# PeixinC/VoiceControlledRobot-VAR

Hardware: AMD Instinct MI355X
Metric: pretext triplets/sec (84x84 RGB + 16 kHz/1 s audio) (higher is better)
Workload: dtype f32; 1 GPU; Kuka+GoogleCommand pretext step, batch 256 per GPU on MI355X, fp32: u8 84x84 image + 2 int16 1 s clips per triplet resident in HBM -> MFCC -> fwd + triplet loss + bwd + Adam (BASELINE.json configs[1]); per_gpu_batch=256, global_batch=256, audio=16 kHz x 1 s int16 x 2, parallelism=dp1, launch=hip-graph replay, head=triplet

## Files before the change

include/var_hip.h:

```cpp
#ifndef VAR_HIP_H
#define VAR_HIP_H

#include <stdint.h>

#ifdef __cplusplus
extern "C" {
#endif

#define VAR_OK 0
#define VAR_ERR_ARG (-1)
#define VAR_ERR_HIP (-2)
#define VAR_ERR_PLAN (-3)
#define VAR_ERR_STATE (-4)

#define VAR_N_PARAMS 213478
#define VAR_EMB_DIM 3
#define VAR_MFCC_FRAMES 100
#define VAR_MFCC_COEFFS 40

typedef struct var_ctx var_ctx;


int var_init(int device_id, var_ctx** out);
int var_destroy(var_ctx* ctx);
const char* var_last_error(var_ctx* ctx);
int var_param_count(void);

int var_plan(var_ctx* ctx, int max_batch, int img_hw);

int var_plan_generation(var_ctx* ctx);
int var_saved_generation(var_ctx* ctx);

typedef struct var_weights var_weights;
int var_weights_create(var_ctx* ctx, var_weights** out);
int var_weights_destroy(var_ctx* ctx, var_weights* w);
int var_weights_bind(var_ctx* ctx, var_weights* w);
int var_pack_weights(var_ctx* ctx, void* stream, const float* params);

int var_arm_encoder_fwd(var_ctx* ctx, void* stream, const float* params,
                        const void* image, int image_is_u8, long image_bstride,
                        const float* mfcc_pos, const float* mfcc_neg, int B, int H,
                        float* image_feat, float* pos_feat, float* neg_feat,
                        float* image_raw, float* pos_raw, int save_for_bwd);

int var_row_dot(var_ctx* ctx, void* stream, const float* a, const float* b, int rows, int dim, float* out);
int var_set_reward_dot(var_ctx* ctx, const float* goal_feat, float* reward_out);

int var_arm_encoder_bwd(var_ctx* ctx, void* stream, const float* params,
                        const float* g_image_feat, const float* g_pos_feat, const float* g_neg_feat,
                        float* grads);

int var_triplet_fwd_bwd(var_ctx* ctx, void* stream, const float* a, const float* p, const float* n,
                        int B, float margin, float inv_count,
                        float* loss_out, float* ga, float* gp, float* gn);

int var_arm_loss_grad(var_ctx* ctx, void* stream, const float* params,
                      const void* image, int image_is_u8, long image_bstride,
                      const float* mfcc_pos, const float* mfcc_neg, int B, int H,
                      float margin, float inv_count,
                      float* grads, float* loss_out, float* feats_out);

int var_arm_loss_grad_pcm(var_ctx* ctx, void* stream, const float* params,
                          const void* image, int image_is_u8, long image_bstride, const int* image_index,
                          const int16_t* pcm, int pcm_stride, const int* clip_index, const int* lens,
                          int B, int H, float margin, float inv_count,
                          float* grads, float* loss_out, float* feats_out);

int var_arm_loss_grad_gather(var_ctx* ctx, void* stream, const float* params,
                             const void* image, int image_is_u8, long image_bstride, const int* image_index,
                             const float* mfcc_pos, const float* mfcc_neg, int B, int H,
                             float margin, float inv_count,
                             float* grads, float* loss_out, float* feats_out);

int var_adam_step(var_ctx* ctx, void* stream, float* params, const float* grads, float* exp_avg,
                  float* exp_avg_sq, long n, float lr, float beta1, float beta2, float eps,
                  float weight_decay, int step);

int var_adam_step_dev(var_ctx* ctx, void* stream, float* params, const float* grads, float* exp_avg,
                      float* exp_avg_sq, long n, const float* lr_dev, float beta1, float beta2, float eps,
                      float weight_decay, int* step_dev);

int var_adam_step_graph(var_ctx* ctx, void* stream, float* params, const float* grads, float* exp_avg,
                        float* exp_avg_sq, long n, const float* lr_dev, float beta1, float beta2, float eps,
                        float weight_decay, int* step_dev, const int* index_table, int row_ints, int n_rows,
                        int* cursor_dev, int* index_row, int ahead);

int var_mfcc(var_ctx* ctx, void* stream, const int16_t* pcm, const int* lens, const int* clip_index,
             int nclips, int pcm_stride, int out_frames, float* out);

int var_mfcc_ex(var_ctx* ctx, void* stream, const int16_t* pcm, const int* lens, const int* clip_index,
                int nclips, int pcm_stride, int out_frames, int n_fft, int win_length, int hop_length, float* out);

int var_ithor_param_count(void);
int var_ithor_plan(var_ctx* ctx, int max_batch, int img_hw);
int var_ithor_set_bf16(var_ctx* ctx, int on);
int var_ithor_set_gru_sequence(var_ctx* ctx, int on);
int var_ithor_gru_status(var_ctx* ctx, unsigned* word);
int var_ithor_guard_loss(var_ctx* ctx, const float* loss_dev);
int var_ithor_encoder_fwd(var_ctx* ctx, void* stream, const float* params,
                          const void* image, int image_is_u8, long image_bstride,
                          const float* snd_pos, const float* snd_neg, int B, int H,
                          float* image_feat, float* pos_feat, float* neg_feat,
                          float* image_raw, float* pos_raw, int save_for_bwd);
int var_ithor_saved_generation(var_ctx* ctx);
int var_ithor_encoder_bwd(var_ctx* ctx, void* stream, const float* params,
                          const float* g_image_feat, const float* g_pos_feat, const float* g_neg_feat,
                          float* grads);
int var_ithor_loss_grad(var_ctx* ctx, void* stream, const float* params,
                        const void* image, int image_is_u8, long image_bstride,
                        const float* snd_pos, const float* snd_neg, int B, int H,
                        float margin, float inv_count,
                        float* grads, float* loss_out, float* feats_out);

int var_inbatch_loss_fwd_bwd(var_ctx* ctx, void* stream, const float* anchor, const float* cand, const int* target,
                             int B, int M, float tau, float inv_count, float* scratch, float* loss_out,
                             float* g_anchor, float* g_cand);

int var_comm_unique_id(var_ctx* ctx, void* id128);
int var_comm_init(var_ctx* ctx, int rank, int nranks, const void* id128);
int var_comm_destroy(var_ctx* ctx);
int var_allreduce_grads(var_ctx* ctx, void* stream, float* flat_grad, long n);
int var_allgather_emb(var_ctx* ctx, void* stream, const float* local, float* global, long n_local);

int var_armnet_param_count(void);
int var_armnet_plan(var_ctx* ctx, int max_batch);
int var_armnet_forward(var_ctx* ctx, void* stream, const float* params, const void* image, int image_is_u8,
                       long image_bstride, const float* image_feat, const float* robot_pose,
                       const float* goal_sound_feat, const float* rnn_hxs, const float* masks, int B,
                       float* value, float* actor_features, float* action_mean, float* rnn_hxs_out);
int var_armnet_status(var_ctx* ctx, unsigned* word);
int var_armnet_clear_status(var_ctx* ctx);

int var_ithor_policy_param_count(int n_actions);
int var_ithor_policy_plan(var_ctx* ctx, int max_batch);
int var_ithor_policy_forward(var_ctx* ctx, void* stream, const float* params, int n_actions, const void* image, int image_is_u8,
                             long image_bstride, const void* occupancy, int occupancy_is_u8, const float* image_feat,
                             const float* goal_sound_feat, const float* rnn_hxs, const float* masks, int B,
                             float* value, float* actor_features, float* logits, float* rnn_hxs_out);
int var_ithor_policy_status(var_ctx* ctx, unsigned* word);
int var_ithor_policy_clear_status(var_ctx* ctx);

int var_ithor_reward_plan(var_ctx* ctx, int max_batch, int img_hw);
int var_ithor_reward_pack(var_ctx* ctx, void* stream, const float* params);
int var_ithor_reward_step(var_ctx* ctx, void* stream, const float* params,
                          const void* image, int image_is_u8, long image_bstride,
                          const float* goal_mfcc, int B,
                          float* image_feat, float* goal_feat, float* reward);

int var_mfcc_psf(var_ctx* ctx, void* stream, const int16_t* pcm, const int* lens, const int* clip_index,
                 int nclips, int pcm_stride, int out_frames, float* out);

int var_profile_tag_count(void);
const char* var_profile_tag_name(int tag);
int var_profile_select(var_ctx* ctx, int tag);
int var_profile_read(var_ctx* ctx, float* total_ms, int* count);
int var_set_streams(var_ctx* ctx, int mask);
int var_join_status(var_ctx* ctx, unsigned* timeouts);
int var_debug_buffer(var_ctx* ctx, const char* name, void** ptr, long* nfloats);
int var_debug_ithor_gru_drop_workgroup(var_ctx* ctx);
int var_debug_armnet_drop_workgroup(var_ctx* ctx);
int var_debug_ithor_dense(var_ctx* ctx, void* stream, int a_kfast, int b_kfast, const float* a, const float* b,
                          float* c, int M, int N, int K, int nsplit, int add);

#ifdef __cplusplus
}
#endif
#endif
```

voicecontrolledrobot-var_amd/_lib.py:

```python
import ctypes
import os
import subprocess
import threading

_HERE = os.path.dirname(os.path.abspath(__file__))
_LIB_PATH = os.environ.get("VAR_HIP_LIB") or os.path.join(_HERE, "libvar_hip.so")
_lib = None
_lock = threading.Lock()


class VarHipError(RuntimeError):
    pass


def library_path():
    return _LIB_PATH


def build_library(force=False):
    args = ["make", "-C", os.path.join(_HERE, "csrc"), "-j8", "-s"]
    if force:
        args.append("-B")
    subprocess.check_call(args)
    return _LIB_PATH


_vp, _i, _l, _f = ctypes.c_void_p, ctypes.c_int, ctypes.c_long, ctypes.c_float

_SIGNATURES = {
    "var_init": (_i, [_i, ctypes.POINTER(_vp)]),
    "var_destroy": (_i, [_vp]),
    "var_last_error": (ctypes.c_char_p, [_vp]),
    "var_param_count": (_i, []),
    "var_plan": (_i, [_vp, _i, _i]),
    "var_plan_generation": (_i, [_vp]),
    "var_saved_generation": (_i, [_vp]),
    "var_weights_create": (_i, [_vp, ctypes.POINTER(_vp)]),
    "var_weights_destroy": (_i, [_vp, _vp]),
    "var_weights_bind": (_i, [_vp, _vp]),
    "var_pack_weights": (_i, [_vp, _vp, _vp]),
    "var_arm_encoder_fwd": (_i, [_vp, _vp, _vp, _vp, _i, _l, _vp, _vp, _i, _i, _vp, _vp, _vp, _vp, _vp, _i]),
    "var_arm_encoder_bwd": (_i, [_vp, _vp, _vp, _vp, _vp, _vp, _vp]),
    "var_row_dot": (_i, [_vp, _vp, _vp, _vp, _i, _i, _vp]),
    "var_triplet_fwd_bwd": (_i, [_vp, _vp, _vp, _vp, _vp, _i, _f, _f, _vp, _vp, _vp, _vp]),
    "var_arm_loss_grad": (_i, [_vp, _vp, _vp, _vp, _i, _l, _vp, _vp, _i, _i, _f, _f, _vp, _vp, _vp]),
    "var_adam_step": (_i, [_vp, _vp, _vp, _vp, _vp, _vp, _l, _f, _f, _f, _f, _f, _i]),
    "var_adam_step_dev": (_i, [_vp, _vp, _vp, _vp, _vp, _vp, _l, _vp, _f, _f, _f, _f, _vp]),
    "var_adam_step_graph": (_i, [_vp, _vp, _vp, _vp, _vp, _vp, _l, _vp, _f, _f, _f, _f, _vp, _vp, _i, _i, _vp, _vp, _i]),
    "var_mfcc": (_i, [_vp, _vp, _vp, _vp, _vp, _i, _i, _i, _vp]),
    "var_mfcc_ex": (_i, [_vp, _vp, _vp, _vp, _vp, _i, _i, _i, _i, _i, _i, _vp]),
    "var_arm_loss_grad_pcm": (_i, [_vp, _vp, _vp, _vp, _i, _l, _vp, _vp, _i, _vp, _vp, _i, _i, _f, _f, _vp, _vp, _vp]),
    "var_arm_loss_grad_gather": (_i, [_vp, _vp, _vp, _vp, _i, _l, _vp, _vp, _vp, _i, _i, _f, _f, _vp, _vp, _vp]),
    "var_inbatch_loss_fwd_bwd": (_i, [_vp, _vp, _vp, _vp, _vp, _i, _i, _f, _f, _vp, _vp, _vp, _vp]),
    "var_comm_unique_id": (_i, [_vp, _vp]),
    "var_comm_init": (_i, [_vp, _i, _i, _vp]),
    "var_comm_destroy": (_i, [_vp]),
    "var_allreduce_grads": (_i, [_vp, _vp, _vp, _l]),
    "var_allgather_emb": (_i, [_vp, _vp, _vp, _vp, _l]),
    "var_armnet_param_count": (_i, []),
    "var_armnet_plan": (_i, [_vp, _i]),
    "var_armnet_forward": (_i, [_vp, _vp, _vp, _vp, _i, _l, _vp, _vp, _vp, _vp, _vp, _i, _vp, _vp, _vp, _vp]),
    "var_armnet_status": (_i, [_vp, _vp]),
    "var_join_status": (_i, [_vp, _vp]),
    "var_set_reward_dot": (_i, [_vp, _vp, _vp]),
    "var_armnet_clear_status": (_i, [_vp]),
    "var_debug_armnet_drop_workgroup": (_i, [_vp]),
    "var_ithor_policy_param_count": (_i, [_i]),
    "var_ithor_policy_plan": (_i, [_vp, _i]),
    "var_ithor_policy_forward": (_i, [_vp, _vp, _vp, _i, _vp, _i, _l, _vp, _i, _vp, _vp, _vp, _vp, _i, _vp, _vp, _vp, _vp]),
    "var_ithor_policy_status": (_i, [_vp, _vp]),
    "var_ithor_policy_clear_status": (_i, [_vp]),
    "var_ithor_reward_plan": (_i, [_vp, _i, _i]),
    "var_ithor_reward_pack": (_i, [_vp, _vp, _vp]),
    "var_ithor_reward_step": (_i, [_vp, _vp, _vp, _vp, _i, _l, _vp, _i, _vp, _vp, _vp]),
    "var_mfcc_psf": (_i, [_vp, _vp, _vp, _vp, _vp, _i, _i, _i, _vp]),
    "var_ithor_param_count": (_i, []),
    "var_ithor_plan": (_i, [_vp, _i, _i]),
    "var_ithor_set_bf16": (_i, [_vp, _i]),
    "var_ithor_set_gru_sequence": (_i, [_vp, _i]),
    "var_ithor_gru_status": (_i, [_vp, _vp]),
    "var_ithor_guard_loss": (_i, [_vp, _vp]),
    "var_debug_ithor_gru_drop_workgroup": (_i, [_vp]),
    "var_ithor_encoder_fwd": (_i, [_vp, _vp, _vp, _vp, _i, _l, _vp, _vp, _i, _i, _vp, _vp, _vp, _vp, _vp, _i]),
    "var_ithor_saved_generation": (_i, [_vp]),
    "var_ithor_encoder_bwd": (_i, [_vp, _vp, _vp, _vp, _vp, _vp, _vp]),
    "var_ithor_loss_grad": (_i, [_vp, _vp, _vp, _vp, _i, _l, _vp, _vp, _i, _i, _f, _f, _vp, _vp, _vp]),
    "var_profile_tag_count": (_i, []),
    "var_profile_tag_name": (ctypes.c_char_p, [_i]),
    "var_profile_select": (_i, [_vp, _i]),
    "var_set_streams": (_i, [_vp, _i]),
    "var_profile_read": (_i, [_vp, ctypes.POINTER(_f), ctypes.POINTER(_i)]),
    "var_debug_buffer": (_i, [_vp, ctypes.c_char_p, ctypes.POINTER(_vp), ctypes.POINTER(_l)]),
    "var_debug_ithor_dense": (_i, [_vp, _vp, _i, _i, _vp, _vp, _vp, _i, _i, _i, _i, _i]),
}

EXPORTED_SYMBOLS = tuple(_SIGNATURES.keys())


def load_library():
    global _lib
    with _lock:
        if _lib is None:
            if not os.path.exists(_LIB_PATH):
                raise VarHipError(
                    f"{_LIB_PATH} is missing: build it with `python __graft_entry__.py` "
                    "(there is no CPU/eager fallback for the VAR hot path)")
            lib = ctypes.CDLL(_LIB_PATH)
            for name, (res, args) in _SIGNATURES.items():
                fn = getattr(lib, name)
                fn.restype = res
                fn.argtypes = args
            _lib = lib
    return _lib


def new_graph():
    import torch
    return torch.cuda.CUDAGraph()


class Context:
    _by_device = {}

    def __init__(self, device_index):
        self.lib = load_library()
        self.device_index = int(device_index)
        h = _vp()
        rc = self.lib.var_init(self.device_index, ctypes.byref(h))
        if rc != 0:
            raise VarHipError(f"var_init({device_index}) failed ({rc}): {self.lib.var_last_error(None).decode()}")
        self.handle = h
        self.plan = (0, 0)

    @classmethod
    def get(cls, device_index):
        ctx = cls._by_device.get(device_index)
        if ctx is None:
            ctx = cls._by_device[device_index] = Context(device_index)
        return ctx

    def check(self, rc, what):
        if rc != 0:
            raise VarHipError(f"{what} failed ({rc}): {self.lib.var_last_error(self.handle).decode()}")

    def stream(self):
        return current_stream_handle()

    def new_weights(self):
        return Weights(self)

    def capture(self, groups):
        import torch
        dev = torch.device("cuda", self.device_index)
        side = torch.cuda.Stream(device=dev)
        side.wait_stream(torch.cuda.current_stream(dev))
        graphs = []
        with torch.cuda.stream(side):
            for bodies in groups:
                g = new_graph()
                with torch.cuda.graph(g, stream=side, capture_error_mode="thread_local"):
                    for body in bodies:
                        body()
                graphs.append(g)
        torch.cuda.current_stream(dev).wait_stream(side)
        return [g.replay for g in graphs]

    def ensure_plan(self, batch, hw):
        if self.plan[1] != hw or self.plan[0] < batch:
            self.check(self.lib.var_plan(self.handle, int(batch), int(hw)), "var_plan")
            self.plan = (int(batch), int(hw))

    def profile_select(self, tag):
        self.check(self.lib.var_profile_select(self.handle, int(tag)), "var_profile_select")

    def set_streams(self, mask):
        return self.lib.var_set_streams(self.handle, int(mask))

    def join_timeouts(self):
        n = ctypes.c_uint(0)
        self.check(self.lib.var_join_status(self.handle, ctypes.byref(n)), "var_join_status")
        return n.value

    def profile_read(self):
        ms, n = _f(), _i()
        self.check(self.lib.var_profile_read(self.handle, ctypes.byref(ms), ctypes.byref(n)), "var_profile_read")
        return ms.value, n.value

    def tag_names(self):
        return [self.lib.var_profile_tag_name(t).decode() for t in range(self.lib.var_profile_tag_count())]

    def debug_buffer(self, name):
        import torch
        p, n = _vp(), _l()
        self.check(self.lib.var_debug_buffer(self.handle, name.encode(), ctypes.byref(p), ctypes.byref(n)),
                   "var_debug_buffer")
        out = torch.empty(n.value, dtype=torch.float32, device=f"cuda:{self.device_index}")
        torch.cuda.synchronize()
        rt = ctypes.CDLL("libamdhip64.so")
        rt.hipMemcpy.argtypes = [_vp, _vp, ctypes.c_size_t, _i]
        rc = rt.hipMemcpy(out.data_ptr(), p, n.value * 4, 3)
        if rc != 0:
            raise VarHipError(f"hipMemcpy failed ({rc})")
        return out


class Weights:

    def __init__(self, ctx):
        self.ctx = ctx
        h = _vp()
        ctx.check(ctx.lib.var_weights_create(ctx.handle, ctypes.byref(h)), "var_weights_create")
        self.handle = h
        self.key = None

    def bind(self):
        c = self.ctx
        c.check(c.lib.var_weights_bind(c.handle, self.handle), "var_weights_bind")

    def pack(self, flat, key=None):
        c = self.ctx
        self.bind()
        c.check(c.lib.var_pack_weights(c.handle, c.stream(), flat.data_ptr()), "var_pack_weights")
        self.key = key

    def __del__(self):
        try:
            if self.handle and self.ctx.handle:
                self.ctx.lib.var_weights_destroy(self.ctx.handle, self.handle)
        except Exception:
            pass
        self.handle = None


def ptr(t):
    return None if t is None else t.data_ptr()


def current_stream_handle():
    import torch
    return torch.cuda.current_stream().cuda_stream
```

voicecontrolledrobot-var_amd/csrc/api.hip:

```cpp
#include <new>
#include <stdlib.h>
#include <string.h>

#include "var_common.h"

static char g_init_err[256] = "";

#define CHECK_CTX(ctx) do { if (!(ctx)) return VAR_ERR_ARG; } while (0)
#define SET_DEVICE(ctx) VAR_HIP_CHECK(ctx, hipSetDevice((ctx)->device))

extern "C" {

int var_param_count(void) { return VAR_N_PARAMS; }

const char* var_last_error(var_ctx* ctx) { return ctx ? ctx->err : g_init_err; }

static int default_streams();

int var_init(int device_id, var_ctx** out) {
    if (!out) return VAR_ERR_ARG;
    *out = nullptr;
    int n = 0;
    hipError_t e = hipGetDeviceCount(&n);
    if (e != hipSuccess || device_id < 0 || device_id >= n) {
        snprintf(g_init_err, sizeof(g_init_err), "var_init: device %d not available (%d HIP devices, %s)",
                 device_id, n, hipGetErrorString(e));
        return VAR_ERR_HIP;
    }
    var_ctx* c = new (std::nothrow) var_ctx();
    if (!c) return VAR_ERR_HIP;
    c->device = device_id;
    c->streams = default_streams();
    c->pl = make_param_layout();
    c->kl = make_pack_layout();
    if (c->pl.total != VAR_N_PARAMS) {
        snprintf(g_init_err, sizeof(g_init_err), "var_init: layout mismatch %d", c->pl.total);
        delete c;
        return VAR_ERR_ARG;
    }
    e = hipSetDevice(device_id);
    if (e == hipSuccess) e = hipMalloc((void**)&c->default_w.data, sizeof(float) * (size_t)c->kl.total);
    c->default_w.owner = c;
    c->bound = &c->default_w;
    c->wpack = c->default_w.data;
    if (e == hipSuccess) e = hipMalloc((void**)&c->loss_buf, sizeof(float) * 64);
    if (e == hipSuccess) e = hipMemset(c->loss_buf, 0, sizeof(float) * 64);
    c->done_ctr = (unsigned*)(c->loss_buf + 32);
    c->jsig = (unsigned*)(c->loss_buf + 40);
    if (e != hipSuccess) {
        snprintf(g_init_err, sizeof(g_init_err), "var_init: %s", hipGetErrorString(e));
        delete c;
        return VAR_ERR_HIP;
    }
    if (e == hipSuccess) e = hipStreamCreateWithFlags(&c->side, hipStreamNonBlocking);
    for (int i = 0; i < 2 && e == hipSuccess; i++) {
        e = hipEventCreateWithFlags(&c->ev_fork[i], hipEventDisableTiming);
        if (e == hipSuccess) e = hipEventCreateWithFlags(&c->ev_join[i], hipEventDisableTiming);
    }
    if (e != hipSuccess) {
        snprintf(g_init_err, sizeof(g_init_err), "var_init: %s", hipGetErrorString(e));
        delete c;
        return VAR_ERR_HIP;
    }
    if (mfcc_build_tables(c) != VAR_OK || pack_table_upload(c) != VAR_OK) {
        snprintf(g_init_err, sizeof(g_init_err), "var_init: %s", c->err);
        delete c;
        return VAR_ERR_HIP;
    }
    *out = c;
    return VAR_OK;
}

int var_destroy(var_ctx* c) {
    CHECK_CTX(c);
    (void)hipSetDevice(c->device);
    comm_free(c);
    mfcc_any_forget(c);
    ithor_free(c);
    armnet_free(c);
    ithor_policy_free(c);
    ithor_reward_free(c);
    for (auto& sl : c->ws_slot) if (sl.base) (void)hipFree(sl.base);
    for (int i = 0; i < c->n_retired; i++) (void)hipFree(c->retired[i]);
    free(c->retired);
    if (c->default_w.data) (void)hipFree(c->default_w.data);
    if (c->loss_buf) (void)hipFree(c->loss_buf);
    if (c->mfcc_tab) (void)hipFree(c->mfcc_tab);
    if (c->mfcc_psf_tab) (void)hipFree(c->mfcc_psf_tab);
    if (c->pack_segs_dev) (void)hipFree(c->pack_segs_dev);
    for (int i = 0; i < 2; i++) {
        if (c->ev_fork[i]) (void)hipEventDestroy(c->ev_fork[i]);
        if (c->ev_join[i]) (void)hipEventDestroy(c->ev_join[i]);
    }
    if (c->side) (void)hipStreamDestroy(c->side);
    if (c->prof_ev) {
        for (int i = 0; i < 2 * kProfMaxPairs; i++) (void)hipEventDestroy(c->prof_ev[i]);
        delete[] c->prof_ev;
    }
    delete c;
    return VAR_OK;
}

int retire_block(var_ctx* c, void* p) {
    if (c->n_retired == c->cap_retired) {
        const int cap = c->cap_retired ? 2 * c->cap_retired : 8;
        void** q = (void**)realloc(c->retired, sizeof(void*) * cap);
        if (!q) { VAR_SET_ERR(c, "var_plan: out of host memory"); return VAR_ERR_HIP; }
        c->retired = q; c->cap_retired = cap;
    }
    c->retired[c->n_retired++] = p;
    return VAR_OK;
}

int var_plan_generation(var_ctx* c) { return c ? c->plan_gen : VAR_ERR_ARG; }
int var_saved_generation(var_ctx* c) { return c ? (c->saved_B > 0 ? c->saved_gen : 0) : VAR_ERR_ARG; }

int var_weights_create(var_ctx* c, var_weights** out) {
    CHECK_CTX(c);
    if (!out) return VAR_ERR_ARG;
    *out = nullptr;
    SET_DEVICE(c);
    var_weights* w = new (std::nothrow) var_weights();
    if (!w) return VAR_ERR_HIP;
    w->owner = c;
    hipError_t e = hipMalloc((void**)&w->data, sizeof(float) * (size_t)c->kl.total);
    if (e != hipSuccess) { VAR_SET_ERR(c, "var_weights_create: %s", hipGetErrorString(e)); delete w; return VAR_ERR_HIP; }
    *out = w;
    return VAR_OK;
}

int var_weights_destroy(var_ctx* c, var_weights* w) {
    CHECK_CTX(c);
    if (!w || w->owner != c || w == &c->default_w) { VAR_SET_ERR(c, "var_weights_destroy: not a handle of this context"); return VAR_ERR_ARG; }
    SET_DEVICE(c);
    if (c->bound == w) { c->bound = &c->default_w; c->wpack = c->default_w.data; }
    int rc = retire_block(c, w->data);
    delete w;
    return rc;
}

int var_weights_bind(var_ctx* c, var_weights* w) {
    CHECK_CTX(c);
    if (!w) w = &c->default_w;
    if (w->owner != c) { VAR_SET_ERR(c, "var_weights_bind: handle belongs to another context"); return VAR_ERR_ARG; }
    c->bound = w;
    c->wpack = w->data;
    return VAR_OK;
}

static int check_weights(var_ctx* c, const float* params, const char* who) {
    if (c->bound->params != params) {
        VAR_SET_ERR(c, "%s: the bound weight image was %s -- var_weights_bind + var_pack_weights first", who,
                    c->bound->params ? "packed from another parameter arena" : "never packed");
        return VAR_ERR_STATE;
    }
    return VAR_OK;
}

static size_t plan_layout(var_ctx* c, char* base, int max_batch, int img_hw) {
    const size_t B = (size_t)max_batch;
    int hs[6];
    hs[0] = img_hw;
    for (int i = 0; i < 5; i++) hs[i + 1] = conv_out(hs[i]);
    size_t off = 0;
    auto carve = [&](size_t nfloats) { size_t o = off; off += (nfloats * 4 + 255) & ~(size_t)255; return o; };
    size_t o_act[6], o_gact[6], o_sact[5], o_gsact[5];
    for (int l = 1; l <= 5; l++) {
        size_t n = B * kImgCh[l] * hs[l] * hs[l];
        if (l == 1 && img_hw == 84) n = B * kAct1TiledFloats;
        o_act[l] = carve(n);
        o_gact[l] = carve(n);
    }
    for (int l = 1; l <= 4; l++) {
        const size_t n = 2 * B * 32 * kSndT[l];
        o_sact[l] = carve(n);
        o_gsact[l] = carve(n);
    }
    const size_t o_hid_i = carve(B * kHid), o_hid_s = carve(2 * B * kHid);
    const size_t o_emb = carve(9 * B), o_emb_raw = carve(9 * B), o_gemb = carve(24 * B), o_hpart = carve(48 * B);
    const size_t o_ghid = carve(6 * B * kHid);
    const size_t n_img_slab = img_slab_floats(), n_snd_slab = snd_slab_floats();
    const size_t o_slab = carve(n_img_slab + n_snd_slab);
    const size_t o_mfcc = carve(2 * B * VAR_MFCC_FRAMES * VAR_MFCC_COEFFS);
    if (!base) return off;
    c->ws = base;
    c->ws_bytes = off;
    auto P = [&](size_t o) { return (float*)(c->ws + o); };
    for (int l = 1; l <= 5; l++) { c->act[l] = P(o_act[l]); c->gact[l] = P(o_gact[l]); }
    for (int l = 1; l <= 4; l++) { c->sact[l] = P(o_sact[l]); c->gsact[l] = P(o_gsact[l]); }
    c->hid_i = P(o_hid_i); c->hid_s = P(o_hid_s);
    c->head_part = P(o_hpart);
    c->emb = P(o_emb); c->emb_raw = P(o_emb_raw); c->gemb = P(o_gemb); c->ghid = P(o_ghid);
    c->slabs = P(o_slab);
    c->mfcc_buf = P(o_mfcc);
    c->slab_floats = n_img_slab + n_snd_slab;
    c->snd_slab_off = n_img_slab;
    c->maxB = max_batch;
    c->H = img_hw;
    for (int i = 0; i < 6; i++) c->hs[i] = hs[i];
    c->saved_B = 0;
    return off;
}

int var_plan(var_ctx* c, int max_batch, int img_hw) {
    CHECK_CTX(c);
    if (max_batch <= 0 || (img_hw != 84 && img_hw != 96)) {
        VAR_SET_ERR(c, "var_plan: batch %d / image size %d unsupported (size must be 84 or 96)", max_batch, img_hw);
        return VAR_ERR_ARG;
    }
    SET_DEVICE(c);
    if (c->ws && c->maxB >= max_batch && c->H == img_hw) return VAR_OK;
    var_ctx::WsSlot& slot = c->ws_slot[img_hw == 84 ? 0 : 1];
    if (!slot.base || slot.maxB < max_batch) {
        if (slot.base) { int rc = retire_block(c, slot.base); if (rc != VAR_OK) return rc; slot.base = nullptr; }
        if (c->ws && c->H == img_hw) c->ws = nullptr;
        const int Bn = slot.maxB > max_batch ? slot.maxB : max_batch;
        const size_t bytes = plan_layout(c, nullptr, Bn, img_hw);
        char* blk = nullptr;
        VAR_HIP_CHECK(c, hipMalloc((void**)&blk, bytes));
        VAR_HIP_CHECK(c, hipMemset(blk, 0, bytes));
        slot.base = blk; slot.maxB = Bn;
    }
    c->plan_gen++;
    plan_layout(c, slot.base, slot.maxB, img_hw);
    return VAR_OK;
}

int var_pack_weights(var_ctx* c, void* stream, const float* params) {
    CHECK_CTX(c);
    if (!params) { VAR_SET_ERR(c, "var_pack_weights: null params"); return VAR_ERR_ARG; }
    SET_DEVICE(c);
    c->bound->params = params;
    return launch_pack_weights(c, (hipStream_t)stream, params);
}

static int check_plan(var_ctx* c, int B, int H, const char* who) {
    if (!c->ws) { VAR_SET_ERR(c, "%s: var_plan() has not been called", who); return VAR_ERR_PLAN; }
    if (B <= 0) { VAR_SET_ERR(c, "%s: batch %d", who, B); return VAR_ERR_ARG; }
    if (B > c->maxB || H != c->H) {
        VAR_SET_ERR(c, "%s: batch %d / size %d exceeds the plan (%d / %d)", who, B, H, c->maxB, c->H);
        return VAR_ERR_PLAN;
    }
    return VAR_OK;
}


struct AudioIn {
    const int16_t* pcm = nullptr; const int* lens = nullptr; const int* clip_index = nullptr; int pcm_stride = 0;
};

static int fork_side(var_ctx* c, hipStream_t s, int i) {
    if (!(c->streams & (1 << i))) return VAR_OK;
    VAR_HIP_CHECK(c, hipEventRecord(c->ev_fork[i], s));
    VAR_HIP_CHECK(c, hipStreamWaitEvent(c->side, c->ev_fork[i], 0));
    return VAR_OK;
}
static int join_side(var_ctx* c, hipStream_t s, int i) {
    if (!(c->streams & (1 << i))) return VAR_OK;
    VAR_HIP_CHECK(c, hipEventRecord(c->ev_join[i], c->side));
    VAR_HIP_CHECK(c, hipStreamWaitEvent(s, c->ev_join[i], 0));
    return VAR_OK;
}

struct CopySegs { float* dst[5]; const float* src[5]; int n[5]; int count; };
__global__ void __launch_bounds__(256) copy_out_kernel(CopySegs S) {
    for (int k = 0; k < S.count; ++k)
        for (int e = blockIdx.x * 256 + threadIdx.x; e < S.n[k]; e += gridDim.x * 256) S.dst[k][e] = S.src[k][e];
}

__global__ void __launch_bounds__(256) gemb_in_kernel(const float* __restrict__ g0, const float* __restrict__ g1, const float* __restrict__ g2,
                                                      float* __restrict__ gemb, int n) {
    const int e = blockIdx.x * 256 + threadIdx.x;
    if (e >= n) return;
    gemb[e] = g0 ? g0[e] : 0.f;
    gemb[n + e] = g1 ? g1[e] : 0.f;
    gemb[2 * n + e] = g2 ? g2[e] : 0.f;
}

__global__ void __launch_bounds__(256) row_dot_kernel(const float* __restrict__ a, const float* __restrict__ b, int rows, int dim,
                                                      float* __restrict__ out) {
    const int r = blockIdx.x * 256 + threadIdx.x;
    if (r >= rows) return;
    float s = 0.f;
    for (int k = 0; k < dim; ++k) s += a[(size_t)r * dim + k] * b[(size_t)r * dim + k];
    out[r] = s;
}

static constexpr int kHead1MaxB = 64;
static constexpr int kSmallMidB = 16;

static FwdPlan plan_encoder_fwd(int H, int B, int save_for_bwd, bool image, bool pos, bool neg, bool finish, bool join_requested,
                                bool capturing, int streams, bool dot_armed) {
    FwdPlan p;
    const bool fwd_only = save_for_bwd == 2;
    const bool snd = pos || neg;
    const bool head2 = !(fwd_only && B <= kHead1MaxB);
    if (head2 && H == 84 && B <= kHead2G && !snd) p.img = ImgPath::All;
    else if (fwd_only && B <= kSmallMidB && H == 84) p.img = ImgPath::Head1Small;
    else p.img = head2 ? ImgPath::Head2Mid3 : ImgPath::Head1Mid3;
    p.act1_tiled = head2 && H == 84;
    p.head_in_conv = p.img != ImgPath::Head1Small;
    p.conv_finish = p.head_in_conv && finish;
    p.fork_ok = (streams & 1) && B > 32;
    p.mfcc_main = !p.fork_ok;
    p.dev_join = join_requested && capturing && p.fork_ok && (streams & 2) && !(streams & 64) && image && pos && neg;
    if (dot_armed && image && finish) p.dot = p.img == ImgPath::Head1Small ? RewardDot::InHead : RewardDot::RowDot;
    return p;
}

static int encoder_fwd(var_ctx* c, hipStream_t s, const float* params, const void* image, int is_u8,
                       long bstride, const int* image_index, const float* pos, const float* neg,
                       const AudioIn* audio, int B, int save_for_bwd, bool finish, bool join_requested, bool dot_armed) {
    int rc;
    if (audio && audio->pcm) {
        pos = c->mfcc_buf;
        neg = c->mfcc_buf + (size_t)B * VAR_MFCC_FRAMES * VAR_MFCC_COEFFS;
    }
    const bool snd = pos || neg;
    hipStreamCaptureStatus cap = hipStreamCaptureStatusNone;
    if (join_requested && hipStreamIsCapturing(s, &cap) != hipSuccess) cap = hipStreamCaptureStatusNone;
    const FwdPlan p = plan_encoder_fwd(c->H, B, save_for_bwd, image, pos, neg, finish, join_requested,
                                       cap == hipStreamCaptureStatusActive, c->streams, dot_armed);
    c->fwd_plan = p;
    hipStream_t ss = p.fork_ok ? c->side : s;
    bool forked = false;
    if (snd && audio && audio->pcm) {
        if (!p.mfcc_main) { if ((rc = fork_side(c, s, 0)) != VAR_OK) return rc; forked = true; }
        if ((rc = launch_mfcc(c, p.mfcc_main ? s : ss, audio->pcm, audio->lens, audio->clip_index, 2 * B, audio->pcm_stride,
                              VAR_MFCC_FRAMES, c->mfcc_buf)) != VAR_OK) return rc;
    }
    if (snd && p.fork_ok && !forked && (rc = fork_side(c, s, 0)) != VAR_OK) return rc;
    if (image) {
        if ((rc = launch_img_fwd(c, s, p, params, image, is_u8, bstride, image_index, B)) != VAR_OK) return rc;
        if ((rc = launch_heads_fwd(c, s, s, p, params, B, true, false, false, finish)) != VAR_OK) return rc;
        if (p.dot == RewardDot::RowDot) {
            hipLaunchKernelGGL(row_dot_kernel, dim3((B + 255) / 256), dim3(256), 0, s, (const float*)c->emb, c->dot_with, B, kEmb, c->dot_out);
            VAR_HIP_CHECK(c, hipGetLastError());
        }
    }
    if (snd) {
        if ((rc = launch_snd_fwd(c, ss, params, pos, neg, B)) != VAR_OK) return rc;
        if ((rc = launch_heads_fwd(c, ss, ss, p, params, B, false, pos != nullptr, neg != nullptr, finish)) != VAR_OK) return rc;
        if (p.fork_ok && !p.dev_join && (rc = join_side(c, s, 0)) != VAR_OK) return rc;
    }
    c->saved_B = B;
    c->saved_gen = ++c->fwd_gen;
    c->saved_image = image;
    c->saved_u8 = is_u8;
    c->saved_bstride = bstride;
    c->saved_index = image_index;
    c->saved_pos = pos;
    c->saved_neg = neg;
    return VAR_OK;
}

int var_arm_encoder_fwd(var_ctx* c, void* stream, const float* params, const void* image, int image_is_u8,
                        long image_bstride, const float* mfcc_pos, const float* mfcc_neg, int B, int H,
                        float* image_feat, float* pos_feat, float* neg_feat, float* image_raw, float* pos_raw,
                        int save_for_bwd) {
    CHECK_CTX(c);
    if (!params) { VAR_SET_ERR(c, "var_arm_encoder_fwd: null params"); return VAR_ERR_ARG; }
    if (image && image_bstride < 3L * H * H) { VAR_SET_ERR(c, "var_arm_encoder_fwd: image stride %ld < 3*H*H", image_bstride); return VAR_ERR_ARG; }
    int rc = check_plan(c, B, H, "var_arm_encoder_fwd");
    if (rc != VAR_OK) return rc;
    if ((rc = check_weights(c, params, "var_arm_encoder_fwd")) != VAR_OK) return rc;
    SET_DEVICE(c);
    hipStream_t s = (hipStream_t)stream;
    c->out_img = image ? image_feat : nullptr; c->out_pos = mfcc_pos ? pos_feat : nullptr; c->out_neg = mfcc_neg ? neg_feat : nullptr;
    rc = encoder_fwd(c, s, params, image, image_is_u8, image_bstride, nullptr, mfcc_pos, mfcc_neg, nullptr, B, save_for_bwd, true,
                     false, c->dot_out != nullptr);
    c->out_img = c->out_pos = c->out_neg = nullptr;
    c->dot_with = nullptr; c->dot_out = nullptr;
    if (rc != VAR_OK) return rc;
    if (save_for_bwd != 1) c->saved_B = 0;
    CopySegs S{};
    auto seg = [&](float* dst, const float* src, int n) { S.dst[S.count] = dst; S.src[S.count] = src; S.n[S.count] = n; S.count++; };
    if (image && image_raw) seg(image_raw, c->act[5], kImgFeat * B);
    if (mfcc_pos && pos_raw) seg(pos_raw, c->sact[4], kSndFeat * B);
    if (S.count) {
        const int grid = (kImgFeat * B + 255) / 256;
        hipLaunchKernelGGL(copy_out_kernel, dim3(grid < 1024 ? grid : 1024), dim3(256), 0, s, S);
        VAR_HIP_CHECK(c, hipGetLastError());
    }
    return VAR_OK;
}

int var_row_dot(var_ctx* c, void* stream, const float* a, const float* b, int rows, int dim, float* out) {
    CHECK_CTX(c);
    if (!a || !b || !out || rows < 1 || dim < 1 || dim > 64) { VAR_SET_ERR(c, "var_row_dot: bad argument (rows %d, dim %d)", rows, dim); return VAR_ERR_ARG; }
    SET_DEVICE(c);
    hipLaunchKernelGGL(row_dot_kernel, dim3((rows + 255) / 256), dim3(256), 0, (hipStream_t)stream, a, b, rows, dim, out);
    VAR_HIP_CHECK(c, hipGetLastError());
    return VAR_OK;
}

int var_set_reward_dot(var_ctx* c, const float* goal_feat, float* reward_out) {
    CHECK_CTX(c);
    if ((goal_feat == nullptr) != (reward_out == nullptr)) { VAR_SET_ERR(c, "var_set_reward_dot: both pointers or neither"); return VAR_ERR_ARG; }
    c->dot_with = goal_feat;
    c->dot_out = reward_out;
    return VAR_OK;
}

static int encoder_bwd(var_ctx* c, hipStream_t s, const float* params, float* grads, bool fused = false,
                       float margin = 0.f, float inv_count = 0.f, float* loss_out = nullptr) {
    const int B = c->saved_B;
    int rc;
    if (!c->saved_image || !c->saved_pos || !c->saved_neg) {
        if ((rc = var_zero_async(c, s, grads, sizeof(float) * VAR_N_PARAMS)) != VAR_OK) return rc;
    }
    const int snd_lo = c->saved_pos ? 0 : B, snd_hi = c->saved_neg ? 2 * B : B;
    hipStream_t ss = (c->streams & 2) ? c->side : s;
    const bool dev_join = c->fwd_plan.dev_join;
    if (!dev_join && (rc = fork_side(c, s, 1)) != VAR_OK) return rc;
    if (c->saved_image) {
        if ((rc = launch_heads_bwd(c, s, s, params, grads, B, true, 0, 0, dev_join, fused, margin, inv_count, fused ? loss_out : nullptr)) != VAR_OK) return rc;
        if ((rc = launch_img_bwd(c, s, params, grads, B)) != VAR_OK) return rc;
    }
    if ((rc = launch_heads_bwd(c, ss, ss, params, grads, B, false, snd_lo, snd_hi, dev_join, fused, margin, inv_count)) != VAR_OK) return rc;
    if ((rc = launch_snd_bwd(c, ss, params, grads, B)) != VAR_OK) return rc;
    return join_side(c, s, 1);
}

int var_arm_encoder_bwd(var_ctx* c, void* stream, const float* params, const float* g_image_feat,
                        const float* g_pos_feat, const float* g_neg_feat, float* grads) {
    CHECK_CTX(c);
    if (!params || !grads) { VAR_SET_ERR(c, "var_arm_encoder_bwd: null params/grads"); return VAR_ERR_ARG; }
    if (c->saved_B <= 0) { VAR_SET_ERR(c, "var_arm_encoder_bwd: no forward saved (save_for_bwd=1 required)"); return VAR_ERR_STATE; }
    { int rc = check_weights(c, params, "var_arm_encoder_bwd"); if (rc != VAR_OK) return rc; }
    SET_DEVICE(c);
    hipStream_t s = (hipStream_t)stream;
    const int B = c->saved_B;
    hipLaunchKernelGGL(gemb_in_kernel, dim3((3 * B + 255) / 256), dim3(256), 0, s, g_image_feat, g_pos_feat, g_neg_feat, c->gemb, 3 * B);
    VAR_HIP_CHECK(c, hipGetLastError());
    return encoder_bwd(c, s, params, grads);
}

int var_triplet_fwd_bwd(var_ctx* c, void* stream, const float* a, const float* p, const float* n, int B,
                        float margin, float inv_count, float* loss_out, float* ga, float* gp, float* gn) {
    CHECK_CTX(c);
    if (!a || !p || !n || !loss_out || B <= 0) { VAR_SET_ERR(c, "var_triplet_fwd_bwd: bad argument"); return VAR_ERR_ARG; }
    SET_DEVICE(c);
    return launch_triplet(c, (hipStream_t)stream, a, p, n, B, margin, inv_count, loss_out, ga, gp, gn);
}

static int loss_grad_impl(var_ctx* c, hipStream_t s, const float* params, const void* image, int image_is_u8,
                          long image_bstride, const int* image_index, const float* mfcc_pos, const float* mfcc_neg,
                          const AudioIn* audio, int B, int H, float margin, float inv_count, float* grads,
                          float* loss_out, float* feats_out, const char* who) {
    if (image_bstride < 3L * H * H) { VAR_SET_ERR(c, "%s: image stride %ld < 3*H*H", who, image_bstride); return VAR_ERR_ARG; }
    int rc = check_plan(c, B, H, who);
    if (rc != VAR_OK) return rc;
    if ((rc = check_weights(c, params, who)) != VAR_OK) return rc;
    SET_DEVICE(c);
    const bool fused = !feats_out && image && (mfcc_pos || (audio && audio->pcm)) && (mfcc_neg || (audio && audio->pcm));
    if ((rc = encoder_fwd(c, s, params, image, image_is_u8, image_bstride, image_index, mfcc_pos, mfcc_neg, audio, B, 1,
                          !fused, fused, false)) != VAR_OK) return rc;
    if (fused) {
        rc = encoder_bwd(c, s, params, grads, true, margin, inv_count, loss_out);
        c->fwd_plan.dev_join = false;
        return rc;
    }
    if ((rc = launch_triplet(c, s, c->emb, c->emb + 3 * B, c->emb + 6 * B, B, margin, inv_count, loss_out,
                             c->gemb, c->gemb + 3 * B, c->gemb + 6 * B)) != VAR_OK) return rc;
    if (feats_out)
        if ((rc = var_copy_async(c, s, feats_out, c->emb, sizeof(float) * 9 * (size_t)B)) != VAR_OK) return rc;
    return encoder_bwd(c, s, params, grads);
}

int var_arm_loss_grad(var_ctx* c, void* stream, const float* params, const void* image, int image_is_u8,
                      long image_bstride, const float* mfcc_pos, const float* mfcc_neg, int B, int H,
                      float margin, float inv_count, float* grads, float* loss_out, float* feats_out) {
    CHECK_CTX(c);
    if (!params || !image || !mfcc_pos || !mfcc_neg || !grads || !loss_out) {
        VAR_SET_ERR(c, "var_arm_loss_grad: null argument");
        return VAR_ERR_ARG;
    }
    return loss_grad_impl(c, (hipStream_t)stream, params, image, image_is_u8, image_bstride, nullptr, mfcc_pos,
                          mfcc_neg, nullptr, B, H, margin, inv_count, grads, loss_out, feats_out, "var_arm_loss_grad");
}

int var_arm_loss_grad_gather(var_ctx* c, void* stream, const float* params, const void* image, int image_is_u8,
                             long image_bstride, const int* image_index, const float* mfcc_pos, const float* mfcc_neg,
                             int B, int H, float margin, float inv_count, float* grads, float* loss_out,
                             float* feats_out) {
    CHECK_CTX(c);
    if (!params || !image || !mfcc_pos || !mfcc_neg || !grads || !loss_out) {
        VAR_SET_ERR(c, "var_arm_loss_grad_gather: null argument");
        return VAR_ERR_ARG;
    }
    return loss_grad_impl(c, (hipStream_t)stream, params, image, image_is_u8, image_bstride, image_index, mfcc_pos,
                          mfcc_neg, nullptr, B, H, margin, inv_count, grads, loss_out, feats_out,
                          "var_arm_loss_grad_gather");
}

int var_arm_loss_grad_pcm(var_ctx* c, void* stream, const float* params, const void* image, int image_is_u8,
                          long image_bstride, const int* image_index, const int16_t* pcm, int pcm_stride,
                          const int* clip_index, const int* lens, int B, int H, float margin, float inv_count,
                          float* grads, float* loss_out, float* feats_out) {
    CHECK_CTX(c);
    if (!params || !image || !pcm || !lens || !grads || !loss_out || pcm_stride <= 0) {
        VAR_SET_ERR(c, "var_arm_loss_grad_pcm: null argument");
        return VAR_ERR_ARG;
    }
    AudioIn a;
    a.pcm = pcm; a.lens = lens; a.clip_index = clip_index; a.pcm_stride = pcm_stride;
    return loss_grad_impl(c, (hipStream_t)stream, params, image, image_is_u8, image_bstride, image_index, nullptr,
                          nullptr, &a, B, H, margin, inv_count, grads, loss_out, feats_out, "var_arm_loss_grad_pcm");
}

int var_adam_step(var_ctx* c, void* stream, float* params, const float* grads, float* exp_avg, float* exp_avg_sq,
                  long n, float lr, float beta1, float beta2, float eps, float weight_decay, int step) {
    CHECK_CTX(c);
    if (!params || !grads || !exp_avg || !exp_avg_sq || n <= 0 || step < 1) {
        VAR_SET_ERR(c, "var_adam_step: bad argument");
        return VAR_ERR_ARG;
    }
    SET_DEVICE(c);
    hipStream_t s = (hipStream_t)stream;
    int rc = launch_adam(c, s, params, grads, exp_avg, exp_avg_sq, n, lr, beta1, beta2, eps, weight_decay, step);
    if (rc != VAR_OK) return rc;
    if (n == VAR_N_PARAMS && c->bound->params == params) return launch_pack_weights(c, s, params);
    return VAR_OK;
}

int var_adam_step_dev(var_ctx* c, void* stream, float* params, const float* grads, float* exp_avg, float* exp_avg_sq,
                      long n, const float* lr_dev, float beta1, float beta2, float eps, float weight_decay,
                      int* step_dev) {
    return var_adam_step_graph(c, stream, params, grads, exp_avg, exp_avg_sq, n, lr_dev, beta1, beta2, eps,
                               weight_decay, step_dev, nullptr, 0, 0, nullptr, nullptr, 0);
}

int var_adam_step_graph(var_ctx* c, void* stream, float* params, const float* grads, float* exp_avg,
                        float* exp_avg_sq, long n, const float* lr_dev, float beta1, float beta2, float eps,
                        float weight_decay, int* step_dev, const int* index_table, int row_ints, int n_rows,
                        int* cursor_dev, int* index_row, int ahead_from) {
    CHECK_CTX(c);
    if (!params || !grads || !exp_avg || !exp_avg_sq || !lr_dev || !step_dev || n <= 0) {
        VAR_SET_ERR(c, "var_adam_step_dev: bad argument");
        return VAR_ERR_ARG;
    }
    if (index_table && (!cursor_dev || !index_row || row_ints <= 0 || n_rows <= 0)) {
        VAR_SET_ERR(c, "var_adam_step_graph: index table without cursor / row buffer / sizes");
        return VAR_ERR_ARG;
    }
    SET_DEVICE(c);
    return launch_adam_dev(c, (hipStream_t)stream, params, grads, exp_avg, exp_avg_sq, n, lr_dev, beta1, beta2, eps,
                           weight_decay, step_dev, n == VAR_N_PARAMS && c->bound->params == params, index_table, row_ints, n_rows, cursor_dev, index_row,
                           ahead_from);
}

int var_mfcc(var_ctx* c, void* stream, const int16_t* pcm, const int* lens, const int* clip_index, int nclips,
             int pcm_stride, int out_frames, float* out) {
    CHECK_CTX(c);
    if (!pcm || !lens || !out || nclips <= 0 || pcm_stride <= 0 || out_frames <= 0) {
        VAR_SET_ERR(c, "var_mfcc: bad argument");
        return VAR_ERR_ARG;
    }
    SET_DEVICE(c);
    return launch_mfcc(c, (hipStream_t)stream, pcm, lens, clip_index, nclips, pcm_stride, out_frames, out);
}

int var_mfcc_ex(var_ctx* c, void* stream, const int16_t* pcm, const int* lens, const int* clip_index, int nclips,
                int pcm_stride, int out_frames, int n_fft, int win_length, int hop_length, float* out) {
    CHECK_CTX(c);
    if (!pcm || !lens || !out || nclips <= 0 || pcm_stride <= 0 || out_frames <= 0) {
        VAR_SET_ERR(c, "var_mfcc_ex: bad argument");
        return VAR_ERR_ARG;
    }
    SET_DEVICE(c);
    if (n_fft == 512 && win_length == 400 && hop_length == 160)
        return launch_mfcc(c, (hipStream_t)stream, pcm, lens, clip_index, nclips, pcm_stride, out_frames, out);
    return launch_mfcc_any(c, (hipStream_t)stream, pcm, lens, clip_index, nclips, pcm_stride, out_frames, n_fft, win_length,
                           hop_length, out);
}

static const char* kTagNames[TAG_COUNT] = {
    "(unused)", "img conv1+conv2 forward", "img conv3+4+5 forward + image head", "(unused)",
    "(unused)", "(unused)", "(unused)", "img conv3+4+5 weight gradients",
    "(unused)", "(unused)", "(unused)",
    "img conv2 data gradient + conv2, conv1 weight gradients",
    "img conv5-4-3 data gradient chain", "(unused)", "(unused)", "img weight-gradient slab fold",
    "snd_fwd_kernel", "snd_dgrad_kernel", "snd_wgrad_kernel", "snd_reduce_kernel", "heads_fwd_kernel",
    "heads_bwd_rows_kernel", "heads_bwd_gemm_kernel", "triplet_kernel", "adam_kernel", "pack_weights_kernel",
    "mfcc_kernel", "ithor conv 11x5 s2 forward", "ithor conv 11x5 s2 data gradient", "ithor conv 11x5 s2 weight gradient"};

int var_profile_tag_count(void) { return TAG_COUNT; }
const char* var_profile_tag_name(int tag) { return (tag >= 0 && tag < TAG_COUNT) ? kTagNames[tag] : ""; }

static int default_streams() { return kDefaultStreams; }

int var_set_streams(var_ctx* c, int mask) {
    if (!c) return -1;
    const int old = c->streams;
    c->streams = mask < 0 ? default_streams() : (mask & (3 | 64));
    return old;
}

int var_join_status(var_ctx* c, unsigned* timeouts) {
    CHECK_CTX(c);
    if (!timeouts) { VAR_SET_ERR(c, "var_join_status: null argument"); return VAR_ERR_ARG; }
    SET_DEVICE(c);
    unsigned w[8];
    VAR_HIP_CHECK(c, hipMemcpy(w, c->jsig, sizeof(w), hipMemcpyDeviceToHost));
    *timeouts = w[3] + w[7];
    return VAR_OK;
}

int var_profile_select(var_ctx* c, int tag) {
    CHECK_CTX(c);
    SET_DEVICE(c);
    if (tag >= TAG_COUNT) { VAR_SET_ERR(c, "var_profile_select: bad tag %d", tag); return VAR_ERR_ARG; }
    if (tag >= 0 && !c->prof_ev) {
        c->prof_ev = new hipEvent_t[2 * kProfMaxPairs];
        for (int i = 0; i < 2 * kProfMaxPairs; i++) VAR_HIP_CHECK(c, hipEventCreate(&c->prof_ev[i]));
    }
    c->prof_tag = tag;
    c->prof_n = 0;
    return VAR_OK;
}

int var_profile_read(var_ctx* c, float* total_ms, int* count) {
    CHECK_CTX(c);
    if (!total_ms || !count) return VAR_ERR_ARG;
    SET_DEVICE(c);
    float tot = 0.f;
    for (int i = 0; i < c->prof_n; i++) {
        float ms = 0.f;
        VAR_HIP_CHECK(c, hipEventSynchronize(c->prof_ev[2 * i + 1]));
        VAR_HIP_CHECK(c, hipEventElapsedTime(&ms, c->prof_ev[2 * i], c->prof_ev[2 * i + 1]));
        tot += ms;
    }
    *total_ms = tot;
    *count = c->prof_n;
    return VAR_OK;
}

int var_debug_buffer(var_ctx* c, const char* name, void** ptr, long* nfloats) {
    CHECK_CTX(c);
    if (!name || !ptr || !nfloats) return VAR_ERR_ARG;
    const size_t B = c->maxB;
    *ptr = nullptr; *nfloats = 0;
    if (!strcmp(name, "wpack")) { *ptr = c->wpack; *nfloats = c->kl.total; return VAR_OK; }
    if (!strncmp(name, "ithor_", 6)) return ithor_debug_buffer(c, name + 6, ptr, nfloats);
    if (!c->ws) { VAR_SET_ERR(c, "var_debug_buffer: no plan"); return VAR_ERR_PLAN; }
    for (int l = 1; l <= 5; l++) {
        char a[16], g[16];
        snprintf(a, sizeof a, "act%d", l); snprintf(g, sizeof g, "gact%d", l);
        const long n = (long)(B * kImgCh[l] * c->hs[l] * c->hs[l]);
        if (!strcmp(name, a)) {
            *ptr = c->act[l]; *nfloats = n;
            if (l == 1 && c->fwd_plan.act1_tiled) {
                int rc = launch_act1_untile(c, nullptr, (int)B);
                if (rc != VAR_OK) return rc;
                VAR_HIP_CHECK(c, hipStreamSynchronize(nullptr));
                *ptr = c->gact[1];
            }
            return VAR_OK;
        }
        if (!strcmp(name, g)) { *ptr = c->gact[l]; *nfloats = n; return VAR_OK; }
    }
    for (int l = 1; l <= 4; l++) {
        char a[16], g[16];
        snprintf(a, sizeof a, "sact%d", l); snprintf(g, sizeof g, "gsact%d", l);
        const long n = (long)(2 * B * 32 * kSndT[l]);
        if (!strcmp(name, a)) { *ptr = c->sact[l]; *nfloats = n; return VAR_OK; }
        if (!strcmp(name, g)) { *ptr = c->gsact[l]; *nfloats = n; return VAR_OK; }
    }
    if (!strcmp(name, "hid_i")) { *ptr = c->hid_i; *nfloats = (long)B * kHid; return VAR_OK; }
    if (!strcmp(name, "hid_s")) { *ptr = c->hid_s; *nfloats = 2 * (long)B * kHid; return VAR_OK; }
    if (!strcmp(name, "emb")) { *ptr = c->emb; *nfloats = 9 * (long)B; return VAR_OK; }
    if (!strcmp(name, "mfcc")) { *ptr = c->mfcc_buf; *nfloats = 2 * (long)B * VAR_MFCC_FRAMES * VAR_MFCC_COEFFS; return VAR_OK; }
    if (!strcmp(name, "slabs")) { *ptr = c->slabs; *nfloats = (long)c->slab_floats; return VAR_OK; }
    if (!strcmp(name, "gemb")) { *ptr = c->gemb; *nfloats = 9 * (long)B; return VAR_OK; }
    VAR_SET_ERR(c, "var_debug_buffer: unknown buffer '%s'", name);
    return VAR_ERR_ARG;
}

}
```

voicecontrolledrobot-var_amd/csrc/img_conv_bwd.hip:

```cpp
#include <stdio.h>
#include <stdlib.h>

#include "img_stage.h"
#define VAR_WGRAD_DEVICE_ONLY
#include "img_wgrad.hip"
#undef VAR_WGRAD_DEVICE_ONLY

template <class W2, class W3, class W4>
__global__ void __launch_bounds__(768)
img_wgrad345_kernel(const float* __restrict__ x2, const float* __restrict__ x3, const float* __restrict__ x4,
                    const float* __restrict__ gy3, const float* __restrict__ gy4, const float* __restrict__ gy5,
                    float* __restrict__ slabs2, float* __restrict__ slabs3, float* __restrict__ slabs4, int G2, int G3, int G4, int B) {
    static_assert(W2::NW * 64 == 768 && W3::NW * 64 == 768 && W4::NW * 64 == 768, "12 waves each");
    int id = blockIdx.x;
    const int n2 = G2 * W2::NCOMBO, n3 = G3 * W3::NCOMBO;
    if (id < n2) { img_wgrad_body<W2>(x2, (long)W2::CIN * W2::H * W2::W, nullptr, gy3, slabs2, B, id % G2, id / G2, G2); return; }
    id -= n2;
    if (id < n3) { img_wgrad_body<W3>(x3, (long)W3::CIN * W3::H * W3::W, nullptr, gy4, slabs3, B, id % G3, id / G3, G3); return; }
    id -= n3;
    img_wgrad_body<W4>(x4, (long)W4::CIN * W4::H * W4::W, nullptr, gy5, slabs4, B, id % G4, id / G4, G4);
}

template <class W2, class W3, class W4>
static int launch_wgrad345(var_ctx* c, hipStream_t s, int B) {
    ProfScope prof(c, s, TAG_IMG_WGRAD0 + 2);
    constexpr int LDS_BYTES = W2::LDS_BYTES > W3::LDS_BYTES ? (W2::LDS_BYTES > W4::LDS_BYTES ? W2::LDS_BYTES : W4::LDS_BYTES)
                                                           : (W3::LDS_BYTES > W4::LDS_BYTES ? W3::LDS_BYTES : W4::LDS_BYTES);
    static unsigned attr_set = 0;
    if (!(attr_set & var_dev_bit(c))) {
        VAR_HIP_CHECK(c, hipFuncSetAttribute((const void*)img_wgrad345_kernel<W2, W3, W4>,
                                             hipFuncAttributeMaxDynamicSharedMemorySize, LDS_BYTES));
        attr_set |= var_dev_bit(c);
    }
    auto groups = [&](int layer, int nb, int nu) {
        const int need = (B * nb + nu - 1) / nu, gmax = img_wgrad_groups(layer);
        return need < gmax ? need : gmax;
    };
    const int G2 = groups(2, W2::NB, W2::NU), G3 = groups(3, W3::NB, W3::NU), G4 = groups(4, W4::NB, W4::NU);
    c->wg_groups[2] = G2; c->wg_groups[3] = G3; c->wg_groups[4] = G4;
    hipLaunchKernelGGL((img_wgrad345_kernel<W2, W3, W4>), dim3(G2 * W2::NCOMBO + G3 * W3::NCOMBO + G4 * W4::NCOMBO), dim3(768),
                       LDS_BYTES, s, c->act[2], c->act[3], c->act[4], c->gact[3], c->gact[4], c->gact[5],
                       c->slabs + img_slab_offset(2), c->slabs + img_slab_offset(3), c->slabs + img_slab_offset(4), G2, G3, G4, B);
    VAR_HIP_CHECK(c, hipGetLastError());
    return VAR_OK;
}

int launch_img_bwd(var_ctx* c, hipStream_t s, const float* params, float* grads, int B) {
    int rc;
    const int H = c->H;
    if (H != 84 && H != 96) { VAR_SET_ERR(c, "unsupported image size %d (84 or 96)", H); return VAR_ERR_ARG; }
    if ((rc = launch_img_bwd_chain(c, s, B)) != VAR_OK) return rc;
    rc = H == 84 ? launch_wgrad345<W84_2, W84_3, W84_4>(c, s, B) : launch_wgrad345<W96_2, W96_3, W96_4>(c, s, B);
    if (rc != VAR_OK) return rc;
    rc = launch_img_bwd_tail2(c, s, B);
    if (rc != VAR_OK) return rc;
    (void)params;
    return launch_img_wgrad_reduce(c, s, grads, 0, 4);
}
```

voicecontrolledrobot-var_amd/csrc/img_wgrad.hip:

```cpp
#include <stdlib.h>

#include <type_traits>

#include "img_stage.h"

template <int CIN_, int COUT_, int H_, bool U8_, int R_, int NU_, int KS_, bool DB_ = false>
struct WgCfg {
    static constexpr bool DB = DB_;
    static constexpr int CIN = CIN_, COUT = COUT_, H = H_, W = H_, R = R_, NU = NU_;
    static constexpr bool U8 = U8_;
    static constexpr bool SMALLC = (CIN < 32);
    static constexpr int HO = (H - 1) / 2 + 1, WO = HO;
    static constexpr int IR = 2 * R + 1;
    static constexpr int PW = 2 * WO + 3;
    static constexpr int XC = SMALLC ? CIN : 32;
    static constexpr int PLANE_X = (IR * PW) | 1;
    static constexpr int UNIT_X = XC * PLANE_X;
    static constexpr int POW = WO + 1;
    static constexpr int PLANE_Y = (R * POW) | 1;
    static constexpr int UNIT_Y = 32 * PLANE_Y;
    static constexpr int NB = (HO + R - 1) / R;
    static constexpr int NBLK = COUT / 32;
    static constexpr int CBLK = SMALLC ? 1 : CIN / 32;
    static constexpr int NCOMBO = NBLK * CBLK;
    static constexpr int KS = KS_;
    static constexpr int NW = SMALLC ? KS : 3 * KS;
    static constexpr int NT = NW * 64;
    static constexpr int XS = (NU * UNIT_X + 3) & ~3, YS = NU * UNIT_Y;
    static constexpr int ZPAD = (XS + YS + 3) & ~3;
    static constexpr int STAGE = ZPAD + 4;
    static constexpr int FOLD = SMALLC ? NW * 1024 : NW * 3 * 1024;
    static constexpr int LDS_FLOATS = ((DB ? 2 : 1) * STAGE > FOLD ? (DB ? 2 : 1) * STAGE : FOLD);
    static_assert(LDS_FLOATS * 4 <= 160 * 1024, "LDS");
    static constexpr int LDS_BYTES = LDS_FLOATS * 4;
    static constexpr int SLAB = SMALLC ? (32 * 32 + 32) : (32 * 9 * 32 + 32);
    static constexpr int HSTEPS = (WO + 1) / 2;
    static constexpr int TS = NU * R * HSTEPS;
    static constexpr int NSTEP = (TS + KS - 1) / KS;
};

#ifndef VAR_WG_PH
#define VAR_WG_PH
namespace { PH_DECL(); }
#if defined(VAR_PHASES) && defined(VAR_WGRAD_DEVICE_ONLY)
extern "C" int var_debug_phases_wgrad(unsigned long long* out) {
    unsigned long long z[32] = {0};
    if (hipMemcpyFromSymbol(out, HIP_SYMBOL(g_phase), sizeof(z)) != hipSuccess) return -1;
    return hipMemcpyToSymbol(HIP_SYMBOL(g_phase), z, sizeof(z)) == hipSuccess ? 0 : -1;
}
#endif
#endif
#ifndef VAR_WG_PH_BLOCK
#define VAR_WG_PH_BLOCK 0
#endif
template <class C>
__device__ __forceinline__ void img_wgrad_body(const void* __restrict__ xin, long bstride, const int* __restrict__ bidx,
                                               const float* __restrict__ gy, float* __restrict__ slabs, int B,
                                               int bx, int by, int G) {
    extern __shared__ __attribute__((aligned(16))) float lds[];
    float* xs = lds;
    float* ys = lds + C::XS;
    constexpr int NT = C::NT;
    using XT = typename std::conditional<C::U8, uint8_t, float>::type;
    const int tid = threadIdx.x, lane = tid & 63, wave = tid >> 6;
    const int half = lane >> 5, l31 = lane & 31;
    const int total_units = B * C::NB;
    const int combo = by;
    const int nb = combo / C::CBLK, cb = combo - nb * C::CBLK;
    const int ky = C::SMALLC ? 0 : wave % 3, ks = C::SMALLC ? wave : wave / 3;

    constexpr bool FLATX = !C::U8 && !C::SMALLC && C::NB == 1 && (C::W & 1) && C::R == C::HO;
    constexpr bool FLATY = !C::SMALLC && C::NB == 1 && (C::WO & 1) && C::R == C::HO;
    typename std::conditional<FLATX, FlatStager<C::XC, C::H, C::W, C::PW, C::PLANE_X, 1, 1, NT, C::NU>,
                              ColStager<C::XC, C::H, C::W, C::IR, C::PW, C::PLANE_X, 1, C::U8, NT, C::NU>>::type sx;
    typename std::conditional<FLATY, FlatStager<32, C::HO, C::WO, C::POW, C::PLANE_Y, 0, 0, NT, C::NU>,
                              ColStager<32, C::HO, C::WO, C::R, C::POW, C::PLANE_Y, 0, false, NT, C::NU>>::type sy;
    sx.init(tid);
    sy.init(tid);

    static_assert(C::NU == 1 || C::NB == 1, "multi-unit stages need whole-image units (consecutive images)");
    struct Stage { const XT* bx; const float* by; int row0x, row0y, nvalid; };
    auto make_stage = [&](int unit0) {
        Stage st;
        const int bo = unit0 / C::NB, band = unit0 - bo * C::NB;
        const int b = bidx ? bidx[bo] : bo;
        st.bx = (const XT*)xin + (size_t)b * bstride + (size_t)(cb * C::XC) * C::H * C::W;
        st.by = gy + ((size_t)bo * C::COUT + nb * 32) * C::HO * C::WO;
        st.row0x = 2 * band * C::R - 1;
        st.row0y = band * C::R;
        st.nvalid = total_units - unit0 < C::NU ? total_units - unit0 : C::NU;
        return st;
    };
    constexpr long YSTRIDE = (long)C::COUT * C::HO * C::WO;

    const int aoff = l31 * C::PLANE_Y + half;
    int boff;
    if constexpr (C::SMALLC) {
        const int col = l31 < C::CIN * 9 ? l31 : 0;
        const int tap = col / C::CIN, c = col - tap * C::CIN;
        boff = c * C::PLANE_X + (tap / 3) * C::PW + (tap % 3) + 2 * half;
    } else {
        boff = l31 * C::PLANE_X + ky * C::PW + 2 * half;
    }
    const int t0 = (ks * C::TS) / C::KS, t1 = ((ks + 1) * C::TS) / C::KS;
    int aos[C::NSTEP], bos[C::NSTEP];
#pragma unroll
    for (int i = 0; i < C::NSTEP; ++i) {
        const int t = t0 + i;
        const bool live = t < t1;
        const int tt = live ? t : t0;
        const int u = tt / (C::R * C::HSTEPS), rem = tt - u * (C::R * C::HSTEPS);
        const int oyl = rem / C::HSTEPS, sstep = rem - oyl * C::HSTEPS;
        aos[i] = live ? C::XS + aoff + u * C::UNIT_Y + oyl * C::POW + 2 * sstep : C::ZPAD;
        bos[i] = boff + u * C::UNIT_X + 2 * oyl * C::PW + 4 * sstep;
    }
    f32x16 acc[3];
#pragma unroll
    for (int t = 0; t < 3; ++t)
#pragma unroll
        for (int r = 0; r < 16; ++r) acc[t][r] = 0.f;
    float bsum = 0.f;

    PHR_INIT(VAR_WG_PH_BLOCK, VAR_PH_THREAD);
    lds_zero<NT>(lds, C::LDS_FLOATS, tid);
    const int first = bx * C::NU;
    if (first < total_units) {
        const Stage st = make_stage(first);
        sx.issue(st.bx, bstride, st.row0x, st.nvalid);
        sy.issue(st.by, YSTRIDE, st.row0y, st.nvalid);
    }
    auto multiply = [&](const float* stage) {
#pragma unroll
        for (int i = 0; i < C::NSTEP; ++i) {
            const float a = stage[aos[i]];
            bsum += a;
            if constexpr (C::SMALLC) {
                acc[0] = __builtin_amdgcn_mfma_f32_32x32x2f32(a, stage[bos[i]], acc[0], 0, 0, 0);
            } else {
                const float b0 = stage[bos[i]], b1 = stage[bos[i] + 1], b2 = stage[bos[i] + 2];
                acc[0] = __builtin_amdgcn_mfma_f32_32x32x2f32(a, b0, acc[0], 0, 0, 0);
                acc[1] = __builtin_amdgcn_mfma_f32_32x32x2f32(a, b1, acc[1], 0, 0, 0);
                acc[2] = __builtin_amdgcn_mfma_f32_32x32x2f32(a, b2, acc[2], 0, 0, 0);
            }
        }
    };
    if constexpr (C::DB) {
        __syncthreads();
        if (first < total_units) {
            const Stage st = make_stage(first);
            sx.store(lds, st.row0x, st.nvalid);
            sy.store(lds + C::XS, st.row0y, st.nvalid);
        }
        __syncthreads();
        int it = 0;
#pragma unroll 1
        for (int unit0 = first; unit0 < total_units; unit0 += G * C::NU, ++it) {
            const int next = unit0 + G * C::NU;
            const bool more = next < total_units;
            const Stage sn = make_stage(more ? next : unit0);
            if (more) {
                sx.issue(sn.bx, bstride, sn.row0x, sn.nvalid);
                sy.issue(sn.by, YSTRIDE, sn.row0y, sn.nvalid);
            }
            __builtin_amdgcn_sched_barrier(0);
            multiply(lds + (it & 1) * C::STAGE);
            __builtin_amdgcn_sched_barrier(0);
            if (more) {
                float* nst = lds + ((it + 1) & 1) * C::STAGE;
                sx.store(nst, sn.row0x, sn.nvalid);
                sy.store(nst + C::XS, sn.row0y, sn.nvalid);
            }
            __syncthreads();
        }
    } else {
        PHR(0);
#pragma unroll 1
        for (int unit0 = first; unit0 < total_units; unit0 += G * C::NU) {
            __syncthreads();
            PHR(1);
            {
                const Stage st = make_stage(unit0);
                sx.store(xs, st.row0x, st.nvalid);
                sy.store(ys, st.row0y, st.nvalid);
            }
            PHR(2);
            __syncthreads();
            PHR(3);
            if (unit0 + G * C::NU < total_units) {
                const Stage st = make_stage(unit0 + G * C::NU);
                sx.issue(st.bx, bstride, st.row0x, st.nvalid);
                sy.issue(st.by, YSTRIDE, st.row0y, st.nvalid);
            }
            PHR(4);
            __builtin_amdgcn_sched_barrier(0);
            multiply(lds);
            __builtin_amdgcn_sched_barrier(0);
            PHR(5);
        }
    }

    float* slab = slabs + ((size_t)bx * C::NCOMBO + combo) * C::SLAB;
    bsum += __shfl_down(bsum, 32, 64);
    if constexpr (C::SMALLC) {
        __syncthreads();
#pragma unroll
        for (int r = 0; r < 16; ++r) {
            const int n = (r & 3) + 8 * (r >> 2) + 4 * half;
            lds[wave * 1024 + n * 32 + l31] = acc[0][r];
        }
        __syncthreads();
        for (int e = tid; e < 1024; e += NT) {
            float sum = 0.f;
#pragma unroll
            for (int q = 0; q < C::KS; ++q) sum += lds[q * 1024 + e];
            slab[e] = sum;
        }
    } else {
        __syncthreads();
#pragma unroll
        for (int kx = 0; kx < 3; ++kx)
#pragma unroll
            for (int r = 0; r < 16; ++r) {
                const int n = (r & 3) + 8 * (r >> 2) + 4 * half;
                lds[(wave * 3 + kx) * 1024 + n * 32 + l31] = acc[kx][r];
            }
        __syncthreads();
        for (int e = tid; e < 9 * 256; e += NT) {
            const int tap = e >> 8, kyy = tap / 3, kx = tap - 3 * kyy, i = (e & 255) * 4;
            f32x4 sum = {0.f, 0.f, 0.f, 0.f};
#pragma unroll
            for (int q = 0; q < C::KS; ++q) sum += *(const f32x4*)(lds + ((q * 3 + kyy) * 3 + kx) * 1024 + i);
            *(f32x4*)(slab + ((i >> 5) * 9 + tap) * 32 + (i & 31)) = sum;
        }
    }
    __syncthreads();
    if (ky == 0 && half == 0) lds[ks * 32 + l31] = bsum;
    __syncthreads();
    if (tid < 32) {
        float sum = 0.f;
#pragma unroll
        for (int q = 0; q < C::KS; ++q) sum += lds[q * 32 + tid];
        slab[(C::SMALLC ? 1024 : 9216) + tid] = sum;
    }
    PHR(6);
    PHR_FLUSH();
}

using W84_2 = WgCfg<32, 64, 21, false, 11, 1, 4>;
using W84_3 = WgCfg<64, 64, 11, false, 6, 4, 4>;
using W84_4 = WgCfg<64, 64, 6, false, 3, 4, 4>;
using W96_2 = WgCfg<32, 64, 24, false, 6, 1, 4>;
using W96_3 = WgCfg<64, 64, 12, false, 6, 1, 4>;
using W96_4 = WgCfg<64, 64, 6, false, 3, 4, 4>;

#ifndef VAR_WGRAD_DEVICE_ONLY
struct RedSeg { int slab_off; int slab_sz; int G; int ncombo; int cblk; int cin; int smallc; int gw; int gb; };
struct RedTable { RedSeg seg[5]; int start[6]; };

__global__ void __launch_bounds__(256)
img_wgrad_reduce_kernel(RedTable T, const float* __restrict__ slabs, float* __restrict__ grads) {
    __shared__ float part[8][33];
    const int lane32 = threadIdx.x & 31, gs = threadIdx.x >> 5;
    const int j = blockIdx.x * 32 + lane32;
    const bool live = j < T.start[5];
    int l = 0;
#pragma unroll
    for (int i = 1; i < 5; ++i) if (j >= T.start[i] && T.start[i + 1] > T.start[i]) l = i;
    const RedSeg S = T.seg[l];
    const int e = live ? j - T.start[l] : 0;
    const float* p = slabs + S.slab_off + e;
    const size_t gstride = (size_t)S.ncombo * S.slab_sz;
    float s = 0.f;
    if (live) {
#pragma unroll 8
        for (int g = gs; g < S.G; g += 8) s += p[(size_t)g * gstride];
    }
    part[gs][lane32] = s;
    __syncthreads();
    if (gs != 0 || !live) return;
    s = ((part[0][lane32] + part[1][lane32]) + (part[2][lane32] + part[3][lane32])) +
        ((part[4][lane32] + part[5][lane32]) + (part[6][lane32] + part[7][lane32]));
    const int combo = e / S.slab_sz, i = e - combo * S.slab_sz;
    if (S.smallc) {
        if (i >= 1024) { grads[S.gb + (i - 1024)] = s; return; }
        const int n = i / 32, col = i % 32;
        if (col < S.cin * 9) {
            const int tap = col / S.cin, c = col - tap * S.cin;
            grads[S.gw + (n * S.cin + c) * 9 + tap] = s;
        }
        return;
    }
    const int nb = combo / S.cblk, cb = combo - nb * S.cblk;
    if (i >= 9216) {
        if (cb == 0) grads[S.gb + nb * 32 + (i - 9216)] = s;
        return;
    }
    const int c = i % 32, tap = (i / 32) % 9, n = i / 288;
    grads[S.gw + ((nb * 32 + n) * S.cin + cb * 32 + c) * 9 + tap] = s;
}

static const int kWgG[5] = {512, 256, 64, 32, 32};
static const int kCombo[5] = {1, 1, 2, 4, 4};
static const int kSlabSz[5] = {32 * 32 + 32, 9248, 9248, 9248, 9248};

size_t img_slab_floats() {
    size_t t = 0;
    for (int i = 0; i < 5; i++) t += (size_t)kWgG[i] * kCombo[i] * kSlabSz[i];
    return t;
}

static size_t slab_offset(int layer) {
    size_t o = 0;
    for (int i = 0; i < layer; i++) o += (size_t)kWgG[i] * kCombo[i] * kSlabSz[i];
    return o;
}

int launch_img_wgrad_reduce(var_ctx* c, hipStream_t s, float* grads, int lo, int hi) {
    const ParamLayout& L = c->pl;
    RedTable T{};
    int st = 0;
    for (int i = 0; i < 5; i++) {
        T.seg[i] = RedSeg{(int)slab_offset(i), kSlabSz[i], c->wg_groups[i], kCombo[i], i < 3 ? 1 : 2, kImgCh[i],
                          i == 0 ? 1 : 0, L.img_w[i], L.img_b[i]};
        T.start[i] = st;
        if (i >= lo && i <= hi) st += kCombo[i] * kSlabSz[i];
    }
    T.start[5] = st;
    ProfScope prof(c, s, TAG_IMG_WREDUCE);
    hipLaunchKernelGGL(img_wgrad_reduce_kernel, dim3((st + 31) / 32), dim3(256), 0, s, T, c->slabs, grads);
    VAR_HIP_CHECK(c, hipGetLastError());
    return VAR_OK;
}

int img_wgrad_groups(int layer) { return kWgG[layer]; }
size_t img_slab_offset(int layer) { return slab_offset(layer); }
#endif
```

voicecontrolledrobot-var_amd/csrc/pack_adam.hip:

```cpp
#include <stdlib.h>

#include "var_common.h"

__global__ void __launch_bounds__(256) zero_words_kernel(unsigned* __restrict__ p, size_t n) {
    for (size_t i = (size_t)blockIdx.x * 256 + threadIdx.x; i < n; i += (size_t)gridDim.x * 256) p[i] = 0u;
}
__global__ void __launch_bounds__(256) copy_words_kernel(unsigned* __restrict__ d, const unsigned* __restrict__ s, size_t n) {
    for (size_t i = (size_t)blockIdx.x * 256 + threadIdx.x; i < n; i += (size_t)gridDim.x * 256) d[i] = s[i];
}
static inline int words_grid(size_t n) { const size_t g = (n + 255) / 256; return (int)(g < 1 ? 1 : (g > 2048 ? 2048 : g)); }
int var_zero_async(var_ctx* c, hipStream_t s, void* p, size_t bytes) {
    if (!bytes) return VAR_OK;
    if ((bytes & 3) || ((uintptr_t)p & 3)) { VAR_SET_ERR(c, "var_zero_async: %zu bytes at %p are not whole aligned words", bytes, p); return VAR_ERR_ARG; }
    hipLaunchKernelGGL(zero_words_kernel, dim3(words_grid(bytes / 4)), dim3(256), 0, s, (unsigned*)p, bytes / 4);
    VAR_HIP_CHECK(c, hipGetLastError());
    return VAR_OK;
}
int var_copy_async(var_ctx* c, hipStream_t s, void* dst, const void* src, size_t bytes) {
    if (!bytes) return VAR_OK;
    if ((bytes & 3) || ((uintptr_t)dst & 3) || ((uintptr_t)src & 3)) { VAR_SET_ERR(c, "var_copy_async: not whole aligned words"); return VAR_ERR_ARG; }
    hipLaunchKernelGGL(copy_words_kernel, dim3(words_grid(bytes / 4)), dim3(256), 0, s, (unsigned*)dst, (const unsigned*)src, bytes / 4);
    VAR_HIP_CHECK(c, hipGetLastError());
    return VAR_OK;
}

struct PackSeg {
    int dst;
    int count;
    int src;
    int cin, cout, taps;
    int kvalid;
    int type;
};
struct PackTable { PackSeg seg[24]; int nseg; };

__global__ void __launch_bounds__(256) pack_weights_kernel(PackTable T, const float* __restrict__ params,
                                                            float* __restrict__ wpack, int total) {
    for (int j = blockIdx.x * 256 + threadIdx.x; j < total; j += gridDim.x * 256) {
        int si = 0;
#pragma unroll
        for (int i = 1; i < 24; ++i) if (i < T.nseg && j >= T.seg[i].dst) si = i;
        const PackSeg S = T.seg[si];
        const int e = j - S.dst;
        float v = 0.f;
        if (S.type == 1) {
            const int c = e % S.cin, n = (e / S.cin) % S.cout, tap = e / (S.cin * S.cout);
            v = params[S.src + (n * S.cin + c) * S.taps + tap];
        } else if (S.type == 3) {
            const int jj = e & 3, ln = (e >> 2) & 63, grp = e >> 8;
            const int nsg = S.cout / 16, nct = S.cin / 16;
            const int sg = grp % nsg, ct = (grp / nsg) % nct, tap = grp / (nsg * nct);
            const int n = 16 * sg + 4 * jj + (ln >> 4), c = 16 * ct + (ln & 15);
            v = params[S.src + (n * S.cin + c) * S.taps + tap];
        } else if (S.type >= 4) {
            const int jj = e & 3, ln = (e >> 2) & 63, grp = e >> 8;
            const int nnt = S.cout / 16, ncg = S.cin / 16;
            const int nt = grp % nnt, G = grp / nnt;
            const int cg = S.type == 4 ? G % ncg : G / 9, tap = S.type == 4 ? G / ncg : G % 9;
            const int n = 16 * nt + (ln & 15), c = 16 * cg + 4 * jj + (ln >> 4);
            v = params[S.src + (n * S.cin + c) * S.taps + tap];
        } else {
            const int n = e % S.cout, k = e / S.cout;
            if (k < S.kvalid) {
                const int tap = k / S.cin, c = k - tap * S.cin;
                v = (S.type == 0) ? params[S.src + (n * S.cin + c) * S.taps + tap]
                                  : params[S.src + (n * S.taps + tap) * S.cin + c];
            }
        }
        wpack[j] = v;
    }
}

static PackTable make_pack_table(var_ctx* c) {
    const ParamLayout& L = c->pl;
    const PackLayout& K = c->kl;
    PackTable T{};
    int n = 0;
    auto add = [&](int dst, int count, int src, int cin, int cout, int taps, int type) {
        T.seg[n++] = PackSeg{dst, count, src, cin, cout, taps, cin * taps, type};
    };
    for (int i = 0; i < 5; i++) {
        int Kp = kImgCh[i] * 9; if (Kp & 1) Kp++;
        add(K.img_f[i], Kp * kImgCh[i + 1], L.img_w[i], kImgCh[i], kImgCh[i + 1], 9, i < 2 ? 0 : (i == 2 ? 5 : 4));
    }
    add(K.img_d[1], 9 * kImgCh[2] * kImgCh[1], L.img_w[1], kImgCh[1], kImgCh[2], 9, 1);
    add(K.snd_f[0], 200 * 32, L.snd_w[0], 40, 32, 5, 2);
    for (int i = 1; i < 4; i++) add(K.snd_f[i], 96 * 32, L.snd_w[i], 32, 32, 3, 0);
    for (int i = 1; i < 4; i++) add(K.snd_d[i], 96 * 32, L.snd_w[i], 32, 32, 3, 1);
    for (int i = 2; i < 5; i++) add(K.img_a[i], 9 * kImgCh[i + 1] * kImgCh[i], L.img_w[i], kImgCh[i], kImgCh[i + 1], 9, 3);
    add(K.ih_w0t, kImgFeat * kHid, L.ih_w0, kImgFeat, kHid, 1, 0);
    add(K.sh_w0t, kSndFeat * kHid, L.sh_w0, kSndFeat, kHid, 1, 0);
    T.nseg = n;
    return T;
}

int launch_pack_weights(var_ctx* c, hipStream_t s, const float* params) {
    const PackLayout& K = c->kl;
    const PackTable T = make_pack_table(c);
    ProfScope prof(c, s, TAG_PACK);
    hipLaunchKernelGGL(pack_weights_kernel, dim3(256), dim3(256), 0, s, T, params, c->wpack, K.total);
    VAR_HIP_CHECK(c, hipGetLastError());
    return VAR_OK;
}

__global__ void __launch_bounds__(256) adam_kernel(float* __restrict__ p, const float* __restrict__ g,
                                                    float* __restrict__ m, float* __restrict__ v, long n,
                                                    float b1, float b2, float eps, float wd,
                                                    float step_size, float bc2_sqrt, const unsigned* __restrict__ guard,
                                                    const float* __restrict__ gloss) {
    if (guard && *guard) return;
    if (gloss && !(fabsf(*gloss) <= 3.4e38f)) return;
    for (long i = (long)blockIdx.x * 256 + threadIdx.x; i < n; i += (long)gridDim.x * 256) {
        const float pi = p[i];
        const float gi = g[i] + wd * pi;
        const float mi = m[i] + (gi - m[i]) * (1.f - b1);
        const float vi = v[i] * b2 + (1.f - b2) * gi * gi;
        m[i] = mi;
        v[i] = vi;
        const float denom = sqrtf(vi) / bc2_sqrt + eps;
        p[i] = pi - step_size * (mi / denom);
    }
}

constexpr int kAdamT = 1024;
__global__ void __launch_bounds__(kAdamT)
adam_pack_dev_kernel(const PackSeg* __restrict__ segs, int nseg, float* __restrict__ p, const float* __restrict__ g, float* __restrict__ m,
                     float* __restrict__ v, long n, const float* __restrict__ lr_dev, float b1, float b2, float eps,
                     float wd, int* __restrict__ step_dev, unsigned* __restrict__ done_ctr, float* __restrict__ wpack,
                     const int* __restrict__ idx_table, int row_ints, int n_rows, int* __restrict__ cursor,
                     int* __restrict__ idx_row, int ahead_from, const unsigned* __restrict__ guard, const float* __restrict__ gloss) {
    if (guard && *guard) return;
    if (gloss && !(fabsf(*gloss) <= 3.4e38f)) return;
    __shared__ float sh_step[2];
    const int t = step_dev[0] + 1;
    if (threadIdx.x == 0) {
        auto ipow = [](double b, int e) { double r = 1.0; while (e > 0) { if (e & 1) r *= b; b *= b; e >>= 1; } return r; };
        const double bc1 = 1.0 - ipow((double)b1, t);
        const double bc2 = 1.0 - ipow((double)b2, t);
        sh_step[0] = (float)((double)lr_dev[0] / bc1);
        sh_step[1] = (float)sqrt(bc2);
    }
    __syncthreads();
    const float step_size = sh_step[0], bc2_sqrt = sh_step[1];
    if (blockIdx.x == 0 && idx_table) {
        int next = cursor[0] + 1;
        if (next >= n_rows) next = 0;
        int next2 = next + 1;
        if (next2 >= n_rows) next2 = 0;
        for (int e = threadIdx.x; e < row_ints; e += kAdamT) {
            idx_row[e] = idx_table[(size_t)next * row_ints + e];
            if (ahead_from > 0) idx_row[row_ints + e] = idx_table[(size_t)next2 * row_ints + e];
        }
        __syncthreads();
        if (threadIdx.x == 0) cursor[0] = next;
    }
    __shared__ PackSeg ssegs[24];
    if (wpack) {
        for (int e = threadIdx.x; e < nseg * (int)(sizeof(PackSeg) / 4); e += kAdamT) ((int*)ssegs)[e] = ((const int*)segs)[e];
        __syncthreads();
    }
    const int lane = threadIdx.x & 63;
    for (long w0 = (long)blockIdx.x * kAdamT + (threadIdx.x - lane); w0 < n; w0 += (long)gridDim.x * kAdamT) {
        const long i = w0 + lane;
        float pn = 0.f;
        if (i < n) {
            const float pi = p[i];
            const float gi = g[i] + wd * pi;
            const float mi = m[i] + (gi - m[i]) * (1.f - b1);
            const float vi = v[i] * b2 + (1.f - b2) * gi * gi;
            m[i] = mi;
            v[i] = vi;
            const float denom = sqrtf(vi) / bc2_sqrt + eps;
            pn = pi - step_size * (mi / denom);
            p[i] = pn;
        }
        if (wpack) {
            bool hit = false;
            if (lane < nseg) {
                const int src = ssegs[lane].src, cnt = ssegs[lane].cin * ssegs[lane].cout * ssegs[lane].taps;
                hit = src < w0 + 64 && src + cnt > w0;
            }
            unsigned long long mask = __ballot(hit);
            while (mask) {
                const int q = __ffsll((long long)mask) - 1;
                mask &= mask - 1;
                const PackSeg S = ssegs[q];
                const int e = (int)i - S.src;
                if (i >= n || e < 0 || e >= S.cin * S.cout * S.taps) continue;
                auto divmod = [](int a, int d, int& qq, int& r) {
                    qq = (int)((float)a * __frcp_rn((float)d));
                    r = a - qq * d;
                    if (r < 0) { --qq; r += d; } else if (r >= d) { ++qq; r -= d; }
                };
                int c, tap, nn, rest;
                if (S.type == 2) { divmod(e, S.cin, rest, c); divmod(rest, S.taps, nn, tap); }
                else { divmod(e, S.taps, rest, tap); divmod(rest, S.cin, nn, c); }
                int d;
                if (S.type == 3)
                    d = ((((tap * (S.cin / 16) + (c >> 4)) * (S.cout / 16) + (nn >> 4)) * 64 + 16 * (nn & 3) + (c & 15)) << 2) + ((nn >> 2) & 3);
                else if (S.type >= 4) {
                    const int G = S.type == 4 ? tap * (S.cin / 16) + (c >> 4) : (c >> 4) * 9 + tap;
                    d = (((G * (S.cout / 16) + (nn >> 4)) * 64 + 16 * (c & 3) + (nn & 15)) << 2) + ((c >> 2) & 3);
                } else d = S.type == 1 ? (tap * S.cout + nn) * S.cin + c : (tap * S.cin + c) * S.cout + nn;
                wpack[S.dst + d] = pn;
            }
        }
    }
    if (threadIdx.x == 0) {
        if (atomicAdd(done_ctr, (unsigned)(t != (int)0x80000000)) == gridDim.x - 1) { step_dev[0] = t; done_ctr[0] = 0; }
    }
}

int pack_table_upload(var_ctx* c) {
    const PackTable T = make_pack_table(c);
    VAR_HIP_CHECK(c, hipMalloc((void**)&c->pack_segs_dev, sizeof(T.seg)));
    VAR_HIP_CHECK(c, hipMemcpy(c->pack_segs_dev, T.seg, sizeof(T.seg), hipMemcpyHostToDevice));
    c->pack_nseg = T.nseg;
    return VAR_OK;
}

int launch_adam_dev(var_ctx* c, hipStream_t s, float* p, const float* g, float* m, float* v, long n,
                    const float* lr_dev, float b1, float b2, float eps, float wd, int* step_dev, bool repack,
                    const int* idx_table, int row_ints, int n_rows, int* cursor, int* idx_row, int ahead_from) {
    ProfScope prof(c, s, TAG_ADAM);
    int grid = (int)((n + kAdamT - 1) / kAdamT);
    if (grid > 256) grid = 256;
    hipLaunchKernelGGL(adam_pack_dev_kernel, dim3(grid), dim3(kAdamT), 0, s, (const PackSeg*)c->pack_segs_dev, c->pack_nseg, p, g, m, v, n, lr_dev,
                       b1, b2, eps, wd, step_dev, c->done_ctr, repack ? c->wpack : nullptr, idx_table, row_ints, n_rows,
                       cursor, idx_row, ahead_from, (c->adam_guard && n == c->adam_guard_n) ? c->adam_guard : nullptr,
                       n == c->adam_guard_n ? c->adam_guard_loss : nullptr);
    VAR_HIP_CHECK(c, hipGetLastError());
    return VAR_OK;
}

int launch_adam(var_ctx* c, hipStream_t s, float* p, const float* g, float* m, float* v, long n,
                float lr, float b1, float b2, float eps, float wd, int step) {
    const double bc1 = 1.0 - pow((double)b1, (double)step);
    const double bc2 = 1.0 - pow((double)b2, (double)step);
    const float step_size = (float)((double)lr / bc1);
    const float bc2_sqrt = (float)sqrt(bc2);
    int grid = (int)((n + 255) / 256);
    if (grid > 2048) grid = 2048;
    ProfScope prof(c, s, TAG_ADAM);
    hipLaunchKernelGGL(adam_kernel, dim3(grid), dim3(256), 0, s, p, g, m, v, n, b1, b2, eps, wd, step_size, bc2_sqrt,
                       (c->adam_guard && n == c->adam_guard_n) ? c->adam_guard : nullptr, n == c->adam_guard_n ? c->adam_guard_loss : nullptr);
    VAR_HIP_CHECK(c, hipGetLastError());
    return VAR_OK;
}
```

voicecontrolledrobot-var_amd/csrc/snd_mfma.hip:

```cpp
#include "var_common.h"

namespace {
constexpr int T0 = 100, F = 40, T1 = 48, T2 = 23, T3 = 11, T4 = 5;
constexpr int XROW = 41;
constexpr int XCLIP = T0 * XROW;
constexpr int SND_SLICE = 32 * 200 + 32 + 3 * (32 * 96 + 32);

template <int NT>
__device__ __forceinline__ void zero_lds(float* p, int n, int tid) {
    for (int e = tid; e < n; e += NT) p[e] = 0.f;
}

template <int NT>
__device__ __forceinline__ void stage_clip(float* dst, const float* __restrict__ src, bool valid, int tid) {
    constexpr int TOT = T0 * F / 4;
#pragma unroll 1
    for (int e0 = tid; e0 < TOT; e0 += NT * 4) {
        float4 v[4];
#pragma unroll
        for (int u = 0; u < 4; ++u) {
            const int e = e0 + u * NT;
            v[u] = (valid && e < TOT) ? ((const float4*)src)[e] : float4{0.f, 0.f, 0.f, 0.f};
        }
#pragma unroll
        for (int u = 0; u < 4; ++u) {
            const int e = e0 + u * NT;
            if (e < TOT) {
                const int r = e / 10, f4 = e - r * 10;
                float* d = dst + r * XROW + f4 * 4;
                d[0] = v[u].x; d[1] = v[u].y; d[2] = v[u].z; d[3] = v[u].w;
            }
        }
    }
}

constexpr int FNC = 4, FNW = 6, FNT = FNW * 64;
static_assert(FNC * 48 == FNW * 32, "layer 0: one 32-pixel block of the FNC x 48 (clip, t) pixels per wave");
constexpr int P1 = 49, P2 = 23, P3 = 11;
constexpr int F_XS = 0, F_Y1 = FNC * XCLIP, F_Y2 = F_Y1 + FNC * 32 * P1, F_Y3 = F_Y2 + FNC * 32 * P2,
              F_END = F_Y3 + FNC * 32 * P3;

template <int TIN, int TOUT, int PIN, int POUT, bool LAST>
__device__ __forceinline__ void snd_layer(const float* __restrict__ in, float* __restrict__ out,
                                          const float* __restrict__ w , const float* __restrict__ bias,
                                          float* __restrict__ gout, int clip0, int nclips, int wave, int lane) {
    constexpr int NPIX = FNC * TOUT, NPB = (NPIX + 31) / 32;
    if (wave >= NPB) return;
    const int half = lane >> 5, l31 = lane & 31;
    int p = wave * 32 + l31;
    const bool pv = p < NPIX;
    if (!pv) p = 0;
    const int cl = p / TOUT, t = p - cl * TOUT;
    const float* bp = in + cl * 32 * PIN + half * PIN + 2 * t;
    const float* wl = w + half * 32 + l31;
    f32x16 acc;
#pragma unroll
    for (int r = 0; r < 16; ++r) acc[r] = 0.f;
    float wb[3][16];
#pragma unroll
    for (int kt = 0; kt < 3; ++kt)
#pragma unroll
        for (int u = 0; u < 16; ++u) wb[kt][u] = wl[(kt * 32 + 2 * u) * 32];
    __builtin_amdgcn_sched_barrier(0);
#pragma unroll
    for (int kt = 0; kt < 3; ++kt)
#pragma unroll
        for (int u = 0; u < 16; ++u)
            acc = __builtin_amdgcn_mfma_f32_32x32x2f32(wb[kt][u], bp[2 * u * PIN + kt], acc, 0, 0, 0);
    if (pv && cl < nclips) {
#pragma unroll
        for (int r = 0; r < 16; ++r) {
            const int n = (r & 3) + 8 * (r >> 2) + 4 * half;
            float v = acc[r] + bias[n];
            v = v > 0.f ? v : 0.f;
            if constexpr (!LAST) out[cl * 32 * POUT + n * POUT + t] = v;
            gout[(size_t)(clip0 + cl) * 32 * TOUT + n * TOUT + t] = v;
        }
    }
}

__global__ void __launch_bounds__(FNT)
snd_fwd_kernel(const float* __restrict__ pos, const float* __restrict__ neg, int B, int clip_lo, int clip_hi,
               const float* __restrict__ w0, const float* __restrict__ w1, const float* __restrict__ w2,
               const float* __restrict__ w3, const float* __restrict__ b0, const float* __restrict__ b1,
               const float* __restrict__ b2, const float* __restrict__ b3,
               float* __restrict__ a1, float* __restrict__ a2, float* __restrict__ a3, float* __restrict__ a4) {
    extern __shared__ __attribute__((aligned(16))) float lds[];
    const int tid = threadIdx.x, lane = tid & 63, wave = tid >> 6;
    const int half = lane >> 5, l31 = lane & 31;
    const int clip0 = clip_lo + blockIdx.x * FNC;
    const int nclips = (clip_hi - clip0) < FNC ? (clip_hi - clip0) : FNC;
#pragma unroll 1
    for (int c = 0; c < FNC; ++c) {
        const int clip = clip0 + c;
        const bool valid = c < nclips;
        const float* src = clip < B ? pos + (size_t)clip * T0 * F : neg + (size_t)(clip - B) * T0 * F;
        stage_clip<FNT>(lds + F_XS + c * XCLIP, valid ? src : pos, valid, tid);
    }
    __syncthreads();
    {
        const int p = wave * 32 + l31;
        const int cl = p / T1, t = p - cl * T1;
        const float* bp = lds + F_XS + cl * XCLIP + 2 * t * XROW + half;
        const float* wl = w0 + half * 32 + l31;
        f32x16 acc;
#pragma unroll
        for (int r = 0; r < 16; ++r) acc[r] = 0.f;
        float wb[2][20];
#pragma unroll
        for (int u = 0; u < 20; ++u) wb[0][u] = wl[(2 * u) * 32];
#pragma unroll
        for (int kt = 0; kt < 5; ++kt) {
            if (kt + 1 < 5) {
#pragma unroll
                for (int u = 0; u < 20; ++u) wb[(kt + 1) & 1][u] = wl[((kt + 1) * 40 + 2 * u) * 32];
            }
            __builtin_amdgcn_sched_barrier(0);
#pragma unroll
            for (int u = 0; u < 20; ++u)
                acc = __builtin_amdgcn_mfma_f32_32x32x2f32(wb[kt & 1][u], bp[kt * XROW + 2 * u], acc, 0, 0, 0);
            __builtin_amdgcn_sched_barrier(0);
        }
        if (cl < nclips) {
#pragma unroll
            for (int r = 0; r < 16; ++r) {
                const int n = (r & 3) + 8 * (r >> 2) + 4 * half;
                float v = acc[r] + b0[n];
                v = v > 0.f ? v : 0.f;
                lds[F_Y1 + cl * 32 * P1 + n * P1 + t] = v;
                a1[(size_t)(clip0 + cl) * 32 * T1 + n * T1 + t] = v;
            }
        }
    }
    __syncthreads();
    snd_layer<T1, T2, P1, P2, false>(lds + F_Y1, lds + F_Y2, w1, b1, a2, clip0, nclips, wave, lane);
    __syncthreads();
    snd_layer<T2, T3, P2, P3, false>(lds + F_Y2, lds + F_Y3, w2, b2, a3, clip0, nclips, wave, lane);
    __syncthreads();
    snd_layer<T3, T4, P3, 1, true>(lds + F_Y3, nullptr, w3, b3, a4, clip0, nclips, wave, lane);
}

constexpr int DNC = 4, DNW = 4, DNT = DNW * 64;
constexpr int G4S = T4 + 2, G3S = T3 + 2, G2S = T2 + 2;
constexpr int D_G4 = 0, D_G3 = D_G4 + DNC * 32 * G4S, D_G2 = D_G3 + DNC * 32 * G3S, D_END = D_G2 + DNC * 32 * G2S;

template <int TIN, int TOUT, int GS, int GXS, bool TO_LDS>
__device__ __forceinline__ void snd_dgrad_layer(const float* __restrict__ g , float* __restrict__ gx_lds,
                                                const float* __restrict__ wd ,
                                                const float* __restrict__ yin, float* __restrict__ gout,
                                                int clip0, int nclips, int wave, int lane) {
    const int half = lane >> 5, l31 = lane & 31;
    constexpr int NE = (TIN + 1) / 2, NO = TIN / 2;
    constexpr int PBE = (DNC * NE + 31) / 32, PBO = (DNC * NO + 31) / 32;
#pragma unroll 1
    for (int it = wave; it < PBE + PBO; it += DNW) {
        const bool odd = it >= PBE;
        const int pb = odd ? it - PBE : it;
        const int per = odd ? NO : NE;
        int p = pb * 32 + l31;
        const bool pv = p < DNC * per;
        if (!pv) p = 0;
        const int cl = p / per, j = p - cl * per;
        const int tin = 2 * j + (odd ? 1 : 0);
        const float* gp = g + cl * 32 * GS + half * GS + j + 1;
        const float* wl = wd + half * 32 + l31;
        f32x16 acc;
#pragma unroll
        for (int r = 0; r < 16; ++r) acc[r] = 0.f;
        if (odd) {
            float wb[16];
#pragma unroll
            for (int u = 0; u < 16; ++u) wb[u] = wl[(1 * 32 + 2 * u) * 32];
#pragma unroll
            for (int u = 0; u < 16; ++u)
                acc = __builtin_amdgcn_mfma_f32_32x32x2f32(wb[u], gp[2 * u * GS], acc, 0, 0, 0);
        } else {
            float wa[16], wc[16];
#pragma unroll
            for (int u = 0; u < 16; ++u) { wa[u] = wl[(0 * 32 + 2 * u) * 32]; wc[u] = wl[(2 * 32 + 2 * u) * 32]; }
#pragma unroll
            for (int u = 0; u < 16; ++u) {
                acc = __builtin_amdgcn_mfma_f32_32x32x2f32(wa[u], gp[2 * u * GS], acc, 0, 0, 0);
                acc = __builtin_amdgcn_mfma_f32_32x32x2f32(wc[u], gp[2 * u * GS - 1], acc, 0, 0, 0);
            }
        }
        if (pv && cl < nclips) {
            const size_t go = (size_t)(clip0 + cl) * 32 * TIN + tin;
#pragma unroll
            for (int r = 0; r < 16; ++r) {
                const int c = (r & 3) + 8 * (r >> 2) + 4 * half;
                const float v = yin[go + c * TIN] > 0.f ? acc[r] : 0.f;
                gout[go + c * TIN] = v;
                if constexpr (TO_LDS) gx_lds[cl * 32 * GXS + c * GXS + tin + 1] = v;
            }
        }
    }
}

__global__ void __launch_bounds__(DNT)
snd_dgrad_kernel(int clip_lo, int clip_hi, const float* __restrict__ wd1, const float* __restrict__ wd2,
                 const float* __restrict__ wd3, const float* __restrict__ a1, const float* __restrict__ a2,
                 const float* __restrict__ a3, const float* __restrict__ g4, float* __restrict__ g3,
                 float* __restrict__ g2, float* __restrict__ g1) {
    __shared__ float lds[D_END];
    const int tid = threadIdx.x, lane = tid & 63, wave = tid >> 6;
    const int clip0 = clip_lo + blockIdx.x * DNC;
    const int nclips = (clip_hi - clip0) < DNC ? (clip_hi - clip0) : DNC;
    zero_lds<DNT>(lds, D_END, tid);
    __syncthreads();
    for (int e = tid; e < DNC * 32 * T4; e += DNT) {
        const int cl = e / (32 * T4), rem = e - cl * 32 * T4, n = rem / T4, t = rem - n * T4;
        if (cl < nclips) lds[D_G4 + cl * 32 * G4S + n * G4S + t + 1] = g4[(size_t)(clip0 + cl) * 32 * T4 + rem];
    }
    __syncthreads();
    snd_dgrad_layer<T3, T4, G4S, G3S, true>(lds + D_G4, lds + D_G3, wd3, a3, g3, clip0, nclips, wave, lane);
    __syncthreads();
    snd_dgrad_layer<T2, T3, G3S, G2S, true>(lds + D_G3, lds + D_G2, wd2, a2, g2, clip0, nclips, wave, lane);
    __syncthreads();
    snd_dgrad_layer<T1, T2, G2S, 1, false>(lds + D_G2, nullptr, wd1, a1, g1, clip0, nclips, wave, lane);
}

constexpr int WNW = 9, WNT = WNW * 64;
constexpr int WY1S = 49, WY2S = 23, WY3S = 11;
constexpr int WG1S = 49, WG2S = 25, WG3S = 13, WG4S = 7;
constexpr int W_X = 0, W_Y1 = W_X + XCLIP, W_Y2 = W_Y1 + 32 * WY1S, W_Y3 = W_Y2 + 32 * WY2S,
              W_G1 = W_Y3 + 32 * WY3S, W_G2 = W_G1 + 32 * WG1S, W_G3 = W_G2 + 32 * WG2S, W_G4 = W_G3 + 32 * WG3S,
              W_END = W_G4 + 32 * WG4S;

template <int TT, int NT>
struct RowRegs {
    static constexpr int N = (32 * TT + NT - 1) / NT;
    float v[N];
    __device__ __forceinline__ void load(const float* __restrict__ src, int tid) {
#pragma unroll
        for (int i = 0; i < N; ++i) {
            const int e = tid + i * NT;
            v[i] = e < 32 * TT ? src[e] : 0.f;
        }
    }
    template <int S>
    __device__ __forceinline__ void store(float* dst, int tid) const {
#pragma unroll
        for (int i = 0; i < N; ++i) {
            const int e = tid + i * NT;
            if (e < 32 * TT) dst[(e / TT) * S + (e % TT)] = v[i];
        }
    }
};

template <int NT>
struct ClipRegs {
    static constexpr int N = (T0 * F / 4 + NT - 1) / NT;
    float4 v[N];
    __device__ __forceinline__ void load(const float* __restrict__ src, int tid) {
#pragma unroll
        for (int i = 0; i < N; ++i) {
            const int e = tid + i * NT;
            v[i] = e < T0 * F / 4 ? ((const float4*)src)[e] : float4{0.f, 0.f, 0.f, 0.f};
        }
    }
    __device__ __forceinline__ void store(float* dst, int tid) const {
#pragma unroll
        for (int i = 0; i < N; ++i) {
            const int e = tid + i * NT;
            if (e < T0 * F / 4) {
                const int r = e / 10, f4 = e - r * 10;
                float* d = dst + r * XROW + f4 * 4;
                d[0] = v[i].x; d[1] = v[i].y; d[2] = v[i].z; d[3] = v[i].w;
            }
        }
    }
};

template <int TOUT, int GS, int YS>
__device__ __forceinline__ void wgrad_taps(f32x16 (&acc)[3], float& bsum, const float* __restrict__ g,
                                           const float* __restrict__ yin, int lane) {
    const int half = lane >> 5, l31 = lane & 31;
    const float* ap = g + l31 * GS + half;
    const float* bp = yin + l31 * YS + 2 * half;
#pragma unroll
    for (int s = 0; s < (TOUT + 1) / 2; ++s) {
        const float a = ap[2 * s];
        bsum += a;
#pragma unroll
        for (int kt = 0; kt < 3; ++kt)
            acc[kt] = __builtin_amdgcn_mfma_f32_32x32x2f32(a, bp[4 * s + kt], acc[kt], 0, 0, 0);
    }
}

__global__ void __launch_bounds__(WNT)
snd_wgrad_kernel(int clip_lo, int clip_hi, int B, const float* __restrict__ pos, const float* __restrict__ neg,
                 const float* __restrict__ a1, const float* __restrict__ a2, const float* __restrict__ a3,
                 const float* __restrict__ g1, const float* __restrict__ g2, const float* __restrict__ g3,
                 const float* __restrict__ g4, float* __restrict__ slabs) {
    __shared__ float lds[W_END];
    const int tid = threadIdx.x, lane = tid & 63, wave = tid >> 6;
    const int half = lane >> 5, l31 = lane & 31;
    f32x16 acc[3], acc2[3];
#pragma unroll
    for (int i = 0; i < 3; ++i)
#pragma unroll
        for (int r = 0; r < 16; ++r) { acc[i][r] = 0.f; acc2[i][r] = 0.f; }
    float bsum = 0.f, bsum2 = 0.f;
    int k0 = wave * 32 + l31;
    if (k0 >= 200) k0 = 0;
    const int xoff = (k0 / 40) * XROW + (k0 % 40) + 2 * half * XROW;
    zero_lds<WNT>(lds, W_END, tid);
    ClipRegs<WNT> rx;
    RowRegs<T1, WNT> ry1, rg1;
    RowRegs<T2, WNT> ry2, rg2;
    RowRegs<T3, WNT> ry3, rg3;
    RowRegs<T4, WNT> rg4;
    auto load_clip = [&](int clip) {
        const float* src = clip < B ? pos + (size_t)clip * T0 * F : neg + (size_t)(clip - B) * T0 * F;
        rx.load(src, tid);
        ry1.load(a1 + (size_t)clip * 32 * T1, tid);
        ry2.load(a2 + (size_t)clip * 32 * T2, tid);
        ry3.load(a3 + (size_t)clip * 32 * T3, tid);
        rg1.load(g1 + (size_t)clip * 32 * T1, tid);
        rg2.load(g2 + (size_t)clip * 32 * T2, tid);
        rg3.load(g3 + (size_t)clip * 32 * T3, tid);
        rg4.load(g4 + (size_t)clip * 32 * T4, tid);
    };
    if (clip_lo + (int)blockIdx.x < clip_hi) load_clip(clip_lo + blockIdx.x);
#pragma unroll 1
    for (int clip = clip_lo + blockIdx.x; clip < clip_hi; clip += gridDim.x) {
        __syncthreads();
        rx.store(lds + W_X, tid);
        ry1.store<WY1S>(lds + W_Y1, tid);
        ry2.store<WY2S>(lds + W_Y2, tid);
        ry3.store<WY3S>(lds + W_Y3, tid);
        rg1.store<WG1S>(lds + W_G1, tid);
        rg2.store<WG2S>(lds + W_G2, tid);
        rg3.store<WG3S>(lds + W_G3, tid);
        rg4.store<WG4S>(lds + W_G4, tid);
        __syncthreads();
        if (clip + (int)gridDim.x < clip_hi) load_clip(clip + gridDim.x);
        __builtin_amdgcn_sched_barrier(0);
        if (wave < 7) {
            const float* ap = lds + W_G1 + l31 * WG1S + half;
            const float* bp = lds + W_X + xoff;
#pragma unroll 8
            for (int s = 0; s < T1 / 2; ++s) {
                const float a = ap[2 * s];
                bsum += a;
                acc[0] = __builtin_amdgcn_mfma_f32_32x32x2f32(a, bp[4 * s * XROW], acc[0], 0, 0, 0);
            }
        } else if (wave == 7) {
            wgrad_taps<T2, WG2S, WY1S>(acc, bsum, lds + W_G2, lds + W_Y1, lane);
        } else {
            wgrad_taps<T3, WG3S, WY2S>(acc, bsum, lds + W_G3, lds + W_Y2, lane);
            wgrad_taps<T4, WG4S, WY3S>(acc2, bsum2, lds + W_G4, lds + W_Y3, lane);
        }
    }
    float* slab = slabs + (size_t)blockIdx.x * SND_SLICE;
    bsum += __shfl_down(bsum, 32, 64);
    bsum2 += __shfl_down(bsum2, 32, 64);
    if (wave < 7) {
        const int k = wave * 32 + l31;
        if (k < 200) {
#pragma unroll
            for (int r = 0; r < 16; ++r) {
                const int n = (r & 3) + 8 * (r >> 2) + 4 * half;
                slab[n * 200 + k] = acc[0][r];
            }
        }
        if (wave == 0 && half == 0) slab[6400 + l31] = bsum;
    } else {
        float* sl = slab + 6432 + (wave == 7 ? 0 : 3104);
#pragma unroll
        for (int kt = 0; kt < 3; ++kt)
#pragma unroll
            for (int r = 0; r < 16; ++r) {
                const int n = (r & 3) + 8 * (r >> 2) + 4 * half;
                sl[(n * 32 + l31) * 3 + kt] = acc[kt][r];
                if (wave == 8) sl[3104 + (n * 32 + l31) * 3 + kt] = acc2[kt][r];
            }
        if (half == 0) {
            sl[3072 + l31] = bsum;
            if (wave == 8) sl[3104 + 3072 + l31] = bsum2;
        }
    }
}

__global__ void __launch_bounds__(256)
snd_reduce_kernel(const float* __restrict__ slabs, int G, float* __restrict__ out) {
    __shared__ float part[8][33];
    const int l32 = threadIdx.x & 31, gs = threadIdx.x >> 5;
    const int e = blockIdx.x * 32 + l32;
    const bool live = e < SND_SLICE;
    float s = 0.f;
    if (live) {
#pragma unroll 16
        for (int g = gs; g < G; g += 8) s += slabs[(size_t)g * SND_SLICE + e];
    }
    part[gs][l32] = s;
    __syncthreads();
    if (gs == 0 && live)
        out[e] = ((part[0][l32] + part[1][l32]) + (part[2][l32] + part[3][l32])) +
                 ((part[4][l32] + part[5][l32]) + (part[6][l32] + part[7][l32]));
}
}

static const int kSndG = 128;
size_t snd_slab_floats() { return (size_t)kSndG * SND_SLICE; }

int launch_snd_fwd(var_ctx* c, hipStream_t s, const float* params, const float* pos, const float* neg, int B) {
    const ParamLayout& L = c->pl;
    const PackLayout& K = c->kl;
    const int lo = pos ? 0 : B, hi = neg ? 2 * B : B;
    if (hi <= lo) return VAR_OK;
    static unsigned attr_set = 0;
    if (!(attr_set & var_dev_bit(c))) {
        VAR_HIP_CHECK(c, hipFuncSetAttribute((const void*)snd_fwd_kernel, hipFuncAttributeMaxDynamicSharedMemorySize,
                                             F_END * 4));
        attr_set |= var_dev_bit(c);
    }
    ProfScope prof(c, s, TAG_SND_FWD);
    hipLaunchKernelGGL(snd_fwd_kernel, dim3((hi - lo + FNC - 1) / FNC), dim3(FNT), F_END * 4, s, pos, neg, B, lo, hi,
                       c->wpack + K.snd_f[0], c->wpack + K.snd_f[1], c->wpack + K.snd_f[2], c->wpack + K.snd_f[3],
                       params + L.snd_b[0], params + L.snd_b[1], params + L.snd_b[2], params + L.snd_b[3],
                       c->sact[1], c->sact[2], c->sact[3], c->sact[4]);
    VAR_HIP_CHECK(c, hipGetLastError());
    return VAR_OK;
}

int launch_snd_bwd(var_ctx* c, hipStream_t s, const float* params, float* grads, int B) {
    const ParamLayout& L = c->pl;
    const PackLayout& K = c->kl;
    const int lo = c->saved_pos ? 0 : B, hi = c->saved_neg ? 2 * B : B;
    if (hi <= lo) {
        { const int rz = var_zero_async(c, s, grads + L.snd_w[0], sizeof(float) * SND_SLICE); if (rz != VAR_OK) return rz; }
        return VAR_OK;
    }
    {
        ProfScope prof(c, s, TAG_SND_DGRAD);
        hipLaunchKernelGGL(snd_dgrad_kernel, dim3((hi - lo + DNC - 1) / DNC), dim3(DNT), 0, s, lo, hi,
                           c->wpack + K.snd_d[1], c->wpack + K.snd_d[2], c->wpack + K.snd_d[3],
                           c->sact[1], c->sact[2], c->sact[3], c->gsact[4], c->gsact[3], c->gsact[2], c->gsact[1]);
    }
    const int G = hi - lo < kSndG ? hi - lo : kSndG;
    float* slabs = c->slabs + c->snd_slab_off;
    {
        ProfScope prof(c, s, TAG_SND_WGRAD);
        hipLaunchKernelGGL(snd_wgrad_kernel, dim3(G), dim3(WNT), 0, s, lo, hi, B, c->saved_pos, c->saved_neg,
                           c->sact[1], c->sact[2], c->sact[3], c->gsact[1], c->gsact[2], c->gsact[3], c->gsact[4], slabs);
    }
    ProfScope prof(c, s, TAG_SND_REDUCE);
    hipLaunchKernelGGL(snd_reduce_kernel, dim3((SND_SLICE + 31) / 32), dim3(256), 0, s, slabs, G,
                       grads + L.snd_w[0]);
    VAR_HIP_CHECK(c, hipGetLastError());
    (void)params;
    return VAR_OK;
}
```

voicecontrolledrobot-var_amd/csrc/var_common.h:

```cpp
#pragma once
#include <hip/hip_runtime.h>
#include <stdint.h>
#include <stdio.h>

#include "../../include/var_hip.h"

typedef float f32x16 __attribute__((ext_vector_type(16)));
typedef float f32x4 __attribute__((ext_vector_type(4)));

static constexpr int kImgCh[6] = {3, 32, 32, 64, 64, 64};
static constexpr int kHid = 128;
static constexpr int kEmb = 3;
static constexpr int kImgFeat = 576;
static constexpr int kSndFeat = 160;
static constexpr int kSndT[5] = {100, 48, 23, 11, 5};

struct ParamLayout {
    int img_w[5], img_b[5];
    int snd_w[4], snd_b[4];
    int ih_w0, ih_b0, ih_w1, ih_b1;
    int sh_w0, sh_b0, sh_w1, sh_b1;
    int total;
};

inline ParamLayout make_param_layout() {
    ParamLayout L{};
    int o = 0;
    for (int i = 0; i < 5; i++) {
        L.img_w[i] = o; o += kImgCh[i + 1] * kImgCh[i] * 9;
        L.img_b[i] = o; o += kImgCh[i + 1];
    }
    const int snd_k[4] = {200, 96, 96, 96};
    for (int i = 0; i < 4; i++) {
        L.snd_w[i] = o; o += 32 * snd_k[i];
        L.snd_b[i] = o; o += 32;
    }
    L.ih_w0 = o; o += kHid * kImgFeat; L.ih_b0 = o; o += kHid;
    L.ih_w1 = o; o += kEmb * kHid;     L.ih_b1 = o; o += kEmb;
    L.sh_w0 = o; o += kHid * kSndFeat; L.sh_b0 = o; o += kHid;
    L.sh_w1 = o; o += kEmb * kHid;     L.sh_b1 = o; o += kEmb;
    L.total = o;
    return L;
}

struct PackLayout {
    int img_f[5];
    int img_d[5];
    int img_a[5];
    int snd_f[4];
    int snd_d[4];
    int ih_w0t;
    int sh_w0t;
    int total;
};

inline PackLayout make_pack_layout() {
    PackLayout P{};
    int o = 0;
    for (int i = 0; i < 5; i++) {
        int K = kImgCh[i] * 9; if (K & 1) K++;
        P.img_f[i] = o; o += K * kImgCh[i + 1];
    }
    P.img_d[0] = P.img_d[2] = P.img_d[3] = P.img_d[4] = -1;
    P.img_d[1] = o; o += 9 * kImgCh[2] * kImgCh[1];
    const int snd_k[4] = {200, 96, 96, 96};
    for (int i = 0; i < 4; i++) { P.snd_f[i] = o; o += snd_k[i] * 32; }
    P.snd_d[0] = -1;
    for (int i = 1; i < 4; i++) { P.snd_d[i] = o; o += 96 * 32; }
    P.img_a[0] = P.img_a[1] = -1;
    for (int i = 2; i < 5; i++) { P.img_a[i] = o; o += 9 * kImgCh[i + 1] * kImgCh[i]; }
    P.ih_w0t = o; o += kImgFeat * kHid;
    P.sh_w0t = o; o += kSndFeat * kHid;
    P.total = o;
    return P;
}

enum VarTag {
    TAG_IMG_FWD0 = 0,
    TAG_IMG_WGRAD0 = 5,
    TAG_IMG_DGRAD0 = 10,
    TAG_IMG_WREDUCE = 15,
    TAG_SND_FWD = 16, TAG_SND_DGRAD = 17, TAG_SND_WGRAD = 18, TAG_SND_REDUCE = 19,
    TAG_HEADS_FWD = 20, TAG_HEADS_BWD_ROWS = 21, TAG_HEADS_BWD_W = 22, TAG_TRIPLET = 23,
    TAG_ADAM = 24, TAG_PACK = 25, TAG_MFCC = 26,
    TAG_ITHOR_S2_FWD = 27, TAG_ITHOR_S2_DGRAD = 28, TAG_ITHOR_S2_WGRAD = 29,
    TAG_COUNT = 30
};
constexpr int kProfMaxPairs = 4096;

struct var_weights {
    float* data = nullptr;
    const float* params = nullptr;
    var_ctx* owner = nullptr;
};

enum class ImgPath {
    All,
    Head2Mid3,
    Head1Mid3,
    Head1Small,
};
enum class RewardDot {
    None,
    InHead,
    RowDot,
};
struct FwdPlan {
    ImgPath img = ImgPath::Head2Mid3;
    bool act1_tiled = false;
    bool head_in_conv = false;
    bool conv_finish = false;
    bool fork_ok = false;
    bool mfcc_main = true;
    bool dev_join = false;
    RewardDot dot = RewardDot::None;
};

struct var_ctx {
    int device = 0;
    char err[512] = {0};
    ParamLayout pl;
    PackLayout kl;
    int maxB = 0, H = 0;
    int hs[6] = {0};
    char* ws = nullptr;
    struct WsSlot { char* base = nullptr; int maxB = 0; } ws_slot[2];
    size_t ws_bytes = 0;
    float* wpack = nullptr;
    var_weights default_w;
    var_weights* bound = nullptr;
    void** retired = nullptr; int n_retired = 0, cap_retired = 0;
    int plan_gen = 0;
    int fwd_gen = 0, saved_gen = 0;
    float* act[6] = {nullptr};
    float* gact[6] = {nullptr};
    float* sact[5] = {nullptr};
    float* gsact[5] = {nullptr};
    float* hid_i = nullptr;
    float* hid_s = nullptr;
    float* emb = nullptr;
    float* emb_raw = nullptr;
    float* head_part = nullptr;
    float* gemb = nullptr;
    float* ghid = nullptr;
    void* pack_segs_dev = nullptr; int pack_nseg = 0;
    unsigned* done_ctr = nullptr;
    unsigned* jsig = nullptr;
    const float* dot_with = nullptr;
    float* dot_out = nullptr;
    FwdPlan fwd_plan;
    float* slabs = nullptr;
    size_t slab_floats = 0;
    size_t snd_slab_off = 0;
    int wg_groups[5] = {0};
    float* loss_buf = nullptr;
    float* mfcc_tab = nullptr;
    int prof_tag = -1;
    int prof_n = 0;
    hipEvent_t* prof_ev = nullptr;
    float *out_img = nullptr, *out_pos = nullptr, *out_neg = nullptr;
    int saved_B = 0;
    const void* saved_image = nullptr;
    int saved_u8 = 0;
    long saved_bstride = 0;
    const float* saved_pos = nullptr;
    const float* saved_neg = nullptr;
    const int* saved_index = nullptr;
    int streams = 0;
    hipStream_t side = nullptr;
    hipEvent_t ev_fork[2] = {nullptr, nullptr}, ev_join[2] = {nullptr, nullptr};
    float* mfcc_buf = nullptr;
    float* mfcc_psf_tab = nullptr;
    void* comm = nullptr; int comm_rank = 0, comm_size = 1;
    void* arm = nullptr;
    void* ith = nullptr;
    void* ipol = nullptr;
    void* irew = nullptr;
    const unsigned* adam_guard = nullptr;
    long adam_guard_n = 0;
    const float* adam_guard_loss = nullptr;
};

static inline unsigned var_dev_bit(const var_ctx* c) { return 1u << (c->device & 31); }

#define VAR_SET_ERR(ctx, ...) do { if (ctx) snprintf((ctx)->err, sizeof((ctx)->err), __VA_ARGS__); } while (0)

#define VAR_HIP_CHECK(ctx, expr)                                                              \
    do {                                                                                      \
        hipError_t e_ = (expr);                                                               \
        if (e_ != hipSuccess) {                                                               \
            VAR_SET_ERR(ctx, "%s failed: %s (%s:%d)", #expr, hipGetErrorString(e_), __FILE__, __LINE__); \
            return VAR_ERR_HIP;                                                               \
        }                                                                                     \
    } while (0)

struct ProfScope {
    var_ctx* c; hipStream_t s; bool on;
    ProfScope(var_ctx* c_, hipStream_t s_, int tag) : c(c_), s(s_), on(false) {
        if (c->prof_tag == tag && c->prof_ev && c->prof_n < kProfMaxPairs) {
            on = hipEventRecord(c->prof_ev[2 * c->prof_n], s) == hipSuccess;
        }
    }
    ~ProfScope() {
        if (on) { (void)hipEventRecord(c->prof_ev[2 * c->prof_n + 1], s); c->prof_n++; }
    }
};

#ifndef VAR_PH_THREAD
#define VAR_PH_THREAD 0
#endif
#ifdef VAR_PHASES
#define PH_DECL() static __device__ unsigned long long g_phase[32]
#define PH_INIT2(blk, thr) unsigned long long ph_t = clock64(); const bool ph_on = (int)blockIdx.x == (blk) && (int)threadIdx.x == (thr)
#define PH_INIT(blk) PH_INIT2(blk, 0)
#define PH(i) do { if (ph_on) { const unsigned long long t_ = clock64(); g_phase[i] += t_ - ph_t; ph_t = t_; } } while (0)
#define PHR_INIT(blk, thr) unsigned long long ph_t = clock64(), ph_a[16] = {0}; const unsigned long long ph_c0 = ph_t, ph_r0 = wall_clock64(); const bool ph_on = (int)blockIdx.x == (blk) && (int)threadIdx.x == (thr)
#define PHR(i) do { const unsigned long long t_ = clock64(); ph_a[i] += t_ - ph_t; ph_t = t_; } while (0)
#define PHR_FLUSH() do { if (ph_on) { for (int i_ = 0; i_ < 16; ++i_) g_phase[i_] += ph_a[i_]; g_phase[16] += wall_clock64() - ph_r0; g_phase[17] += clock64() - ph_c0; } } while (0)
#else
#define PH_DECL()
#define PH_INIT(blk)
#define PH_INIT2(blk, thr)
#define PH(i)
#define PHR_INIT(blk, thr)
#define PHR(i)
#define PHR_FLUSH()
#endif


typedef __attribute__((address_space(1))) unsigned gu32h;
__device__ __forceinline__ void join_store(float* p, float v) {
    __hip_atomic_store((gu32h*)p, __builtin_bit_cast(unsigned, v), __ATOMIC_RELAXED, __HIP_MEMORY_SCOPE_AGENT);
}
__device__ __forceinline__ float join_load(const float* p) {
    return __builtin_bit_cast(float, __hip_atomic_load((gu32h*)p, __ATOMIC_RELAXED, __HIP_MEMORY_SCOPE_AGENT));
}
__device__ __forceinline__ void join_signal(unsigned* sig, unsigned n_wg, unsigned* other) {
    __syncthreads();
    if (threadIdx.x == 0 && atomicAdd(sig, 1u) == n_wg - 1) {
        atomicExch(sig, 0u);
        atomicAdd(sig + 1, 1u);
        const unsigned want = __hip_atomic_load((gu32h*)(other + 2), __ATOMIC_RELAXED, __HIP_MEMORY_SCOPE_AGENT) + 1u;
        const unsigned long long t0 = wall_clock64();
        while ((int)(__hip_atomic_load((gu32h*)(other + 1), __ATOMIC_RELAXED, __HIP_MEMORY_SCOPE_AGENT) - want) < 0) {
            if (wall_clock64() - t0 > 500000ull) { atomicAdd(other + 3, 1u); break; }
            __builtin_amdgcn_s_sleep(8);
        }
        __hip_atomic_store((gu32h*)(other + 2), want, __ATOMIC_RELAXED, __HIP_MEMORY_SCOPE_AGENT);
    }
}

static inline int conv_out(int h) { return (h - 1) / 2 + 1; }

extern "C" int retire_block(var_ctx* c, void* p);
int mfcc_build_tables(var_ctx* c);
int launch_mfcc_any(var_ctx* c, hipStream_t s, const int16_t* pcm, const int* lens, const int* clip_index, int nclips,
                    int pcm_stride, int out_frames, int n_fft, int win, int hop, float* out);
int launch_mfcc_psf(var_ctx* c, hipStream_t s, const int16_t* pcm, const int* lens, const int* clip_index, int nclips,
                    int pcm_stride, int out_frames, float* out);
void mfcc_any_forget(var_ctx* c);
void ithor_free(var_ctx* c);
void armnet_free(var_ctx* c);
void ithor_policy_free(var_ctx* c);
void ithor_reward_free(var_ctx* c);
void comm_free(var_ctx* c);
int pack_table_upload(var_ctx* c);
size_t img_slab_floats();
int img_wgrad_groups(int layer);
size_t img_slab_offset(int layer);
int launch_img_wgrad_reduce(var_ctx* c, hipStream_t s, float* grads, int lo, int hi);
size_t snd_slab_floats();

int launch_pack_weights(var_ctx* c, hipStream_t s, const float* params);
int launch_img_fwd(var_ctx* c, hipStream_t s, const FwdPlan& p, const float* params, const void* image, int is_u8,
                   long bstride, const int* image_index, int B);
int launch_img_fwd_head(var_ctx* c, hipStream_t s, const float* params, const void* image, int is_u8, long bstride,
                        const int* image_index, int B);
int var_zero_async(var_ctx* c, hipStream_t s, void* p, size_t bytes);
int var_copy_async(var_ctx* c, hipStream_t s, void* dst, const void* src, size_t bytes);
int launch_img_fwd_head2(var_ctx* c, hipStream_t s, const float* params, const void* image, int is_u8, long bstride,
                         const int* image_index, int B);
#ifndef VAR_HEAD2_G
#define VAR_HEAD2_G 256
#endif
static constexpr int kHead2G = VAR_HEAD2_G;
int launch_img_fwd_mid(var_ctx* c, hipStream_t s, const float* params, int B, unsigned* sig, const float* fin_b1);
int launch_img_fwd_all(var_ctx* c, hipStream_t s, const float* params, const void* image, int is_u8, long bstride,
                       const int* image_index, int B, unsigned* sig,
                       const float* fin_b1);
static constexpr int kDefaultStreams = 3;
static constexpr int kTailG = 256;
static constexpr long kAct1TiledFloats = 7L * 32 * 300 + 128;
int launch_act1_untile(var_ctx* c, hipStream_t s, int B);
int launch_img_bwd_chain(var_ctx* c, hipStream_t s, int B);
static constexpr int kTail2G = 256;
int launch_img_bwd_tail2(var_ctx* c, hipStream_t s, int B);
int launch_img_bwd(var_ctx* c, hipStream_t s, const float* params, float* grads, int B);
int launch_snd_fwd(var_ctx* c, hipStream_t s, const float* params, const float* pos, const float* neg, int B);
int launch_snd_bwd(var_ctx* c, hipStream_t s, const float* params, float* grads, int B);
int launch_heads_fwd(var_ctx* c, hipStream_t s, hipStream_t ss, const FwdPlan& p, const float* params, int B, bool has_img,
                     bool has_pos, bool has_neg, bool finish);
int launch_heads_bwd(var_ctx* c, hipStream_t s, hipStream_t ss, const float* params, float* grads, int B, bool has_img,
                     int snd_lo, int snd_hi, bool dev_join, bool fused = false, float margin = 0.f, float inv_count = 0.f,
                     float* loss_out = nullptr);
int launch_triplet_loss(var_ctx* c, hipStream_t s, const float* params, int B, float margin, float inv_count,
                        float* loss_out);
int launch_triplet(var_ctx* c, hipStream_t s, const float* a, const float* p, const float* n, int B,
                   float margin, float inv_count, float* loss_out, float* ga, float* gp, float* gn);
int launch_adam(var_ctx* c, hipStream_t s, float* p, const float* g, float* m, float* v, long n,
                float lr, float b1, float b2, float eps, float wd, int step);
int launch_adam_dev(var_ctx* c, hipStream_t s, float* p, const float* g, float* m, float* v, long n,
                    const float* lr_dev, float b1, float b2, float eps, float wd, int* step_dev, bool repack,
                    const int* idx_table, int row_ints, int n_rows, int* cursor, int* idx_row, int ahead_from);
int launch_mfcc(var_ctx* c, hipStream_t s, const int16_t* pcm, const int* lens, const int* clip_index, int nclips,
                int pcm_stride, int out_frames, float* out);

long snd_bf16_workspace_bytes(int nclips);
int snd2_bf16_fwd(var_ctx* c, hipStream_t s, const float* x, const float* w, const float* bias, float* y, int nclips,
                  int maxclips, void* ws);
int snd1_bf16_fwd(var_ctx* c, hipStream_t s, const float* x0, int n0, const float* x1, int n1, const float* w, const float* bias,
                  float* y, int maxclips, void* ws);
int snd1_bf16_wgrad(var_ctx* c, hipStream_t s, const float* x0, int n0, const float* x1, int n1, float* dw, float* slab, int maxclips,
                    void* ws);
int snd3_bf16_fwd(var_ctx* c, hipStream_t s, const float* w, const float* bias, float* y, int nclips, int maxclips, void* ws);
int snd3_bf16_dgrad(var_ctx* c, hipStream_t s, const float* gy_seq, const float* w, float* dx, float* bias_part, int* nparts,
                    int nclips, int maxclips, void* ws);
int snd2_bf16_prepare_gy(var_ctx* c, hipStream_t s, const float* gy, int nclips, int maxclips, void* ws);
int snd2_bf16_dgrad(var_ctx* c, hipStream_t s, const float* w, float* dx, float* bias_part, int* nparts, int nclips, int maxclips,
                    void* ws);
int snd2_bf16_wgrad(var_ctx* c, hipStream_t s, float* dw, float* slab, int nclips, int maxclips, void* ws);
int snd3_bf16_wgrad(var_ctx* c, hipStream_t s, float* dw, float* slab, int nclips, int maxclips, void* ws);
int ithor_debug_buffer(var_ctx* c, const char* name, void** ptr, long* nfloats);

long gru_bf16_workspace_bytes(int maxclips);
void* gru_bf16_h16(void* ws);
void* gru_bf16_dgh16(void* ws, int maxclips);
void* gru_bf16_dgi16(void* ws, int maxclips);
void* gru_bf16_x16(void* ws, int maxclips);
int gru_bf16_to_bf16(var_ctx* c, hipStream_t s, const float* x, void* y, long n);
int gru_bf16_convert_x(var_ctx* c, hipStream_t s, const float* x, long n, int maxclips, void* ws);
void* gru_bf16_wih16(void* ws, int maxclips);
float* gru_bf16_bias_part(void* ws, int maxclips);
int gru_bf16_pack(var_ctx* c, hipStream_t s, const float* w_hh, const float* w_ih, long dirP, int nclips, int maxclips, float* Hb,
                  long dirH, void* ws);
int gru_bf16_step_fwd(var_ctx* c, hipStream_t s, const float* GI, float* Hb, const float* b_hh, long dirP, float* R, float* Z,
                      float* Nn, float* GHN, int nclips, int maxclips, int step, long dirGI, long dirH, long dirS, int save, void* ws);
int gru_bf16_step_bwd(var_ctx* c, hipStream_t s, float* DH, const float* Hb, const float* R, const float* Z, const float* Nn,
                      const float* GHN, float* DGI, float* DGH, int nclips, int maxclips, int step, int has_next, long dirGI,
                      long dirH, long dirS, long dirDGH, void* ws);
int gru_bf16_seq_fwd(var_ctx* c, hipStream_t s, const float* GI, float* Hb, const float* b_hh, long dirP, float* R, float* Z, float* Nn,
                     float* GHN, int nclips, int maxclips, long dirGI, long dirH, long dirS, int save, void* ws, int drop_one);
int gru_bf16_seq_bwd(var_ctx* c, hipStream_t s, float* DH, const float* Hb, const float* R, const float* Z, const float* Nn,
                     const float* GHN, float* DGI, float* DGH, int nclips, int maxclips, long dirGI, long dirH, long dirS, long dirDGH,
                     void* ws, int store32);
int gru_bf16_reset_timeout(var_ctx* c, hipStream_t s, int maxclips, void* ws);
int gru_bf16_step_begin(var_ctx* c, hipStream_t s, int maxclips, void* ws);
const unsigned* gru_bf16_timeout_ptr(int maxclips, void* ws);
int gru_bf16_poison_on_timeout(var_ctx* c, hipStream_t s, float* grads, int n, int maxclips, void* ws);
int gru_bf16_timeout_word(var_ctx* c, int maxclips, void* ws, unsigned* out);

long img_bf16_workspace_bytes();
int img_bf16_conv(var_ctx* c, hipStream_t s, int layer, int side, int dgrad, const float* x, const float* w, const float* bias,
                  const float* mask, float* y, float* csum, int* nparts, int B, void* ws, int prepacked);
int img_bf16_pack_all(var_ctx* c, hipStream_t s, const float* w2, const float* w3, const float* w4, const float* w5, void* ws);
int img_bf16_wgrad(var_ctx* c, hipStream_t s, int layer, int side, const float* x, const float* gy, float* dw, float* slab, int B);
int img_bf16_wgrad1(var_ctx* c, hipStream_t s, int side, const void* image, long bstride, const float* gy, float* dw, float* slab, int B);
```

voicecontrolledrobot-var_amd/trainer.py:

```python
import csv
import os

import torch

from ._lib import Context, VarHipError, ptr
from .layout import N_PARAMS
from .ops import mfcc as mfcc_op


def multistep_lr(base_lr, milestones, gamma, epoch):
    lr = base_lr
    for ms in sorted(milestones):
        if epoch >= ms:
            lr *= gamma
    return lr


def _dist_on(pg):
    return pg is not None or (torch.distributed.is_available() and torch.distributed.is_initialized())


class VARTrainer:

    def __init__(self, model, lr=1e-4, weight_decay=1e-6, betas=(0.9, 0.999), eps=1e-8, margin=1.0,
                 process_group=None, _ctx=None):
        flat = model.flat_parameters()
        if _ctx is None:
            if not flat.is_cuda:
                raise VarHipError("VARTrainer needs the model on a GPU (no CPU fallback)")
            _ctx = Context.get(flat.device.index)
        self.model = model
        self.dev = flat.device
        self.ctx = _ctx
        self.lr, self.wd, self.betas, self.eps, self.margin = lr, weight_decay, betas, eps, margin
        self.hw = model.config.img_dim[1]
        self.gbuf = torch.zeros(N_PARAMS + 1, dtype=torch.float32, device=self.dev)
        self.exp_avg = torch.zeros(N_PARAMS, dtype=torch.float32, device=self.dev)
        self.exp_avg_sq = torch.zeros(N_PARAMS, dtype=torch.float32, device=self.dev)
        self.step_count = 0
        self.pg = process_group
        self.world, self.rank = 1, 0
        self.rccl = None
        self.force_collective = os.environ.get("VAR_FORCE_ALLREDUCE") == "1"
        if _dist_on(process_group):
            self.world = torch.distributed.get_world_size(process_group)
            self.rank = torch.distributed.get_rank(process_group)
            if self.world > 1:
                src = torch.distributed.get_global_rank(process_group, 0) if process_group is not None else 0
                torch.distributed.broadcast(flat, src=src, group=process_group)
        self.pack()

    def pack(self):
        self.weights = self.model.hip_weights(self.ctx, force=True)

    def _bind(self):
        self.weights = self.model.hip_weights(self.ctx)

    @property
    def grads(self):
        return self.gbuf[:N_PARAMS]

    @property
    def loss(self):
        return self.gbuf[N_PARAMS:]

    def _loss_ptr(self):
        return self.gbuf.data_ptr() + 4 * N_PARAMS

    def sync_global_batch(self, local_batch):
        if self.rccl is not None and self.world > 1:
            t = torch.tensor([float(local_batch)], dtype=torch.float32, device=self.dev)
            self.rccl.allreduce(t)
            return int(round(float(t.item())))
        if self.world > 1:
            t = torch.tensor([int(local_batch)], dtype=torch.int64, device=self.dev)
            torch.distributed.all_reduce(t, op=torch.distributed.ReduceOp.SUM, group=self.pg)
            return int(t.item())
        return int(local_batch)

    def _gb(self, B, global_batch):
        return B * self.world if global_batch is None else int(global_batch)

    def loss_and_grads(self, image, pos, neg, global_batch=None):
        flat = self.model.flat_parameters()
        B = image.shape[0]
        c = self.ctx
        c.ensure_plan(B, self.hw)
        self._bind()
        c.check(c.lib.var_arm_loss_grad(c.handle, c.stream(), ptr(flat), ptr(image),
                                        int(image.dtype == torch.uint8), image.stride(0), ptr(pos), ptr(neg),
                                        B, self.hw, float(self.margin), 1.0 / self._gb(B, global_batch), ptr(self.gbuf),
                                        self._loss_ptr(), None), "var_arm_loss_grad")

    def use_rccl(self, comm):
        self.rccl = comm
        self.world, self.rank = comm.size, comm.rank
        return self

    def _collective(self):
        return self.rccl is not None or self.world > 1 or (self.force_collective and torch.distributed.is_initialized())

    def allreduce(self, async_op=False):
        if self.rccl is not None:
            self.rccl.allreduce(self.gbuf)
        elif self.world > 1 or (self.force_collective and torch.distributed.is_initialized()):
            return torch.distributed.all_reduce(self.gbuf, op=torch.distributed.ReduceOp.SUM, group=self.pg,
                                                async_op=async_op)
        return None

    def adam(self):
        self.step_count += 1
        flat = self.model.flat_parameters()
        c = self.ctx
        self._bind()
        c.check(c.lib.var_adam_step(c.handle, c.stream(), ptr(flat), ptr(self.gbuf),
                                    ptr(self.exp_avg), ptr(self.exp_avg_sq), N_PARAMS, float(self.lr),
                                    float(self.betas[0]), float(self.betas[1]), float(self.eps), float(self.wd),
                                    int(self.step_count)), "var_adam_step")

    def _device_scalars(self, B):
        dev = self.dev
        self._g_lr = torch.full((1,), float(self.lr), dtype=torch.float32, device=dev)
        self._g_step = torch.full((1,), int(self.step_count), dtype=torch.int32, device=dev)

    def sync_device_scalars(self):
        if getattr(self, "_g_step", None) is not None:
            self._g_step.fill_(int(self.step_count))
            self._g_lr.fill_(float(self.lr))

    def _body_grad_pcm(self, images, pcm, idx, Bs, gb):
        c, flat = self.ctx, self.model.flat_parameters()
        img_idx, clip_idx, lens = idx[:Bs], idx[Bs:3 * Bs], idx[3 * Bs:5 * Bs]

        def body():
            self._bind()
            c.check(c.lib.var_arm_loss_grad_pcm(c.handle, c.stream(), ptr(flat), ptr(images),
                                                int(images.dtype == torch.uint8), images.stride(0), ptr(img_idx),
                                                ptr(pcm), pcm.stride(0), ptr(clip_idx), ptr(lens), Bs, self.hw,
                                                float(self.margin), 1.0 / gb, ptr(self.gbuf),
                                                self._loss_ptr(), None), "var_arm_loss_grad_pcm")
        return body

    def _body_adam(self, table=None, rows=0, row_ints=0, ahead=0):
        c, flat = self.ctx, self.model.flat_parameters()

        def body():
            self._bind()
            c.check(c.lib.var_adam_step_graph(c.handle, c.stream(), ptr(flat), ptr(self.gbuf),
                                              ptr(self.exp_avg), ptr(self.exp_avg_sq), N_PARAMS, ptr(self._g_lr),
                                              float(self.betas[0]), float(self.betas[1]), float(self.eps),
                                              float(self.wd), ptr(self._g_step),
                                              ptr(table) if table is not None else None, row_ints, rows,
                                              ptr(self._g_cursor) if table is not None else None,
                                              ptr(self._g_idx) if table is not None else None, int(ahead)),
                    "var_adam_step_graph")
        return body

    def capture_dataset_step(self, images, pcm, batch, global_batch=None):
        B = batch
        self._g_idx = torch.zeros(5 * B, dtype=torch.int32, device=self.dev)
        self._device_scalars(B)
        self.ctx.ensure_plan(B, self.hw)
        grad = self._body_grad_pcm(images, pcm, self._g_idx, B, self._gb(B, global_batch))
        adam = self._body_adam()
        if self._collective():
            g_grad, g_adam = self.ctx.capture([[grad], [adam]])
        else:
            (g_grad,), g_adam = self.ctx.capture([[grad, adam]]), None

        def replay(idx_row):
            self._bind()
            self._g_idx.copy_(idx_row, non_blocking=True)
            g_grad()
            if g_adam is not None:
                self.allreduce()
                g_adam()
            self.step_count += 1
            return self.loss
        return replay

    def capture_epoch_steps(self, images, pcm, batch, table, global_batch=None, steps_per_epoch=None, tail_batch=0,
                            tail_global_batch=None):
        B = batch
        rows, row_ints = int(table.shape[0]), int(table.shape[1])
        if row_ints != 5 * B or table.dtype != torch.int32 or table.device != self.dev or not table.is_contiguous():
            raise VarHipError("index table must be a contiguous int32 (rows, 5*batch) tensor on the trainer's device")
        tail_batch = int(tail_batch)
        if tail_batch:
            if not (0 < tail_batch < B) or not steps_per_epoch or rows % steps_per_epoch:
                raise VarHipError("ragged table: need 0 < tail_batch < batch and rows a multiple of steps_per_epoch")
        self._g_table = torch.empty_like(table)
        self._g_cursor = torch.zeros(1, dtype=torch.int32, device=self.dev)
        self._device_scalars(B)
        c = self.ctx
        c.ensure_plan(B, self.hw)
        dp = self._collective()
        ahead = 1 if dp else 0
        self._g_idx = torch.zeros((2 if dp else 1) * row_ints, dtype=torch.int32, device=self.dev)
        adam = self._body_adam(self._g_table, rows, row_ints, ahead)
        sizes = [(B, self._gb(B, global_batch))]
        if tail_batch:
            sizes.append((tail_batch, self._gb(tail_batch, tail_global_batch)))
        state = {"row": 0}

        def is_tail(row):
            return bool(tail_batch) and row % steps_per_epoch == steps_per_epoch - 1

        if not dp:
            graphs = [c.capture([[self._body_grad_pcm(images, pcm, self._g_idx, Bs, gb), adam]])[0] for Bs, gb in sizes]

            def load_table(t):
                assert t.shape == self._g_table.shape
                self._g_table.copy_(t, non_blocking=True)
                self._g_idx.copy_(t[0], non_blocking=True)
                self._g_cursor.zero_()
                state["row"] = 0

            def replay():
                self._bind()
                graphs[1 if is_tail(state["row"]) else 0]()
                state["row"] = (state["row"] + 1) % rows
                self.step_count += 1
                return self.loss
            load_table(table)
            return replay, load_table

        flat = self.model.flat_parameters()
        self._g_mfcc = torch.zeros(2 * B, 1, 100, 40, dtype=torch.float32, device=self.dev)
        cur, nxt = self._g_idx[:row_ints], self._g_idx[row_ints:]

        def body_grad(Bs, gb):
            img_idx = cur[:Bs]

            def body():
                self._bind()
                c.check(c.lib.var_arm_loss_grad_gather(c.handle, c.stream(), ptr(flat), ptr(images),
                                                       int(images.dtype == torch.uint8), images.stride(0), ptr(img_idx),
                                                       ptr(self._g_mfcc), ptr(self._g_mfcc[Bs:]), Bs, self.hw,
                                                       float(self.margin), 1.0 / gb, ptr(self.gbuf),
                                                       self._loss_ptr(), None), "var_arm_loss_grad_gather")
            return body

        def body_front(Bs):
            clip_idx, lens = nxt[Bs:3 * Bs], nxt[3 * Bs:5 * Bs]

            def body():
                c.check(c.lib.var_mfcc(c.handle, c.stream(), ptr(pcm), ptr(lens), ptr(clip_idx), 2 * Bs,
                                       pcm.stride(0), 100, ptr(self._g_mfcc)), "var_mfcc")
            return body

        body_front(B)()
        g_front = [c.capture([[body_front(Bs)]])[0] for Bs, _ in sizes]

        def body_step(Bs, gb, Bn):
            grad, front = body_grad(Bs, gb), body_front(Bn)

            def body():
                grad()
                if self.dev.type == "cuda":
                    main = torch.cuda.current_stream(self.dev)
                    aux = self._aux_stream()
                    aux.wait_stream(main)
                    with torch.cuda.stream(aux):
                        front()
                    self.allreduce()
                    main.wait_stream(aux)
                else:
                    self.allreduce()
                    front()
                adam()
            return body

        def pairs():
            out = {(0, 0)}
            if tail_batch:
                out |= {(0, 1), (1, 0)} if steps_per_epoch > 1 else {(1, 1)}
            return sorted(out)
        one_graph = getattr(self, "dp_one_graph", True) and (
            self.dev.type != "cuda" or self.rccl is not None or
            (torch.distributed.is_initialized() and torch.distributed.get_backend(self.pg) == "nccl"))
        g_step = {}
        if one_graph:
            for a, b in pairs():
                (Bs, gb), (Bn, _) = sizes[a], sizes[b]
                g_step[(a, b)] = c.capture([[body_step(Bs, gb, Bn)]])[0]
        g_grad = g_adam = None
        if not one_graph:
            g_grad = [c.capture([[body_grad(Bs, gb)]])[0] for Bs, gb in sizes]
            g_adam = c.capture([[adam]])[0]
        self.dp_graphs_per_step = 1 if one_graph else 3

        def load_table(t):
            assert t.shape == self._g_table.shape
            self._g_table.copy_(t, non_blocking=True)
            nxt.copy_(t[0], non_blocking=True)
            g_front[1 if is_tail(0) else 0]()
            cur.copy_(t[0], non_blocking=True)
            nxt.copy_(t[1 % rows], non_blocking=True)
            self._g_cursor.zero_()
            state["row"] = 0

        def replay():
            row = state["row"]
            self._bind()
            a, b = (1 if is_tail(row) else 0), (1 if is_tail((row + 1) % rows) else 0)
            if one_graph:
                g_step[(a, b)]()
            else:
                g_grad[a]()
                work = self.allreduce(async_op=True)
                g_front[b]()
                if work is not None:
                    work.wait()
                g_adam()
            state["row"] = (row + 1) % rows
            self.step_count += 1
            return self.loss
        load_table(table)
        return replay, load_table

    def _aux_stream(self):
        if getattr(self, "_aux", None) is None:
            self._aux = torch.cuda.Stream(device=self.dev)
        return self._aux

    def set_lr(self, lr):
        self.lr = lr
        if getattr(self, "_g_lr", None) is not None:
            self._g_lr.fill_(float(lr))

    def step(self, image, pos, neg, global_batch=None):
        self._check(image, pos, neg)
        self.loss_and_grads(image, pos, neg, global_batch)
        self.allreduce()
        self.adam()
        return self.loss

    def step_from_dataset(self, images, image_index, pcm, clip_index, lens, global_batch=None):
        flat = self.model.flat_parameters()
        B = image_index.numel()
        for t in (image_index, clip_index, lens):
            if t.dtype != torch.int32 or t.device != self.dev or not t.is_contiguous():
                raise VarHipError("index / length tensors must be contiguous int32 tensors on the trainer's device")
        if pcm.dtype != torch.int16 or clip_index.numel() != 2 * B or lens.numel() != 2 * B:
            raise VarHipError("pcm must be int16 and clip_index / lens must hold 2*B entries")
        if pcm.stride(0) % 2 or (pcm.dim() == 2 and pcm.stride(1) != 1):
            raise VarHipError("pcm rows must be contiguous with an even stride (the front-end loads sample pairs)")
        c = self.ctx
        c.ensure_plan(B, self.hw)
        self._bind()
        c.check(c.lib.var_arm_loss_grad_pcm(c.handle, c.stream(), ptr(flat), ptr(images),
                                            int(images.dtype == torch.uint8), images.stride(0), ptr(image_index),
                                            ptr(pcm), pcm.stride(0), ptr(clip_index), ptr(lens), B, self.hw,
                                            float(self.margin), 1.0 / self._gb(B, global_batch), ptr(self.gbuf),
                                            self._loss_ptr(), None), "var_arm_loss_grad_pcm")
        self.allreduce()
        self.adam()
        return self.loss

    def _inbatch_head(self, anchor, cand, target, tau, inv_count):
        c = self.ctx
        B, M = anchor.shape[0], cand.shape[0]
        loss = torch.empty(1, dtype=torch.float32, device=self.dev)
        ga, gc = torch.empty_like(anchor), torch.empty_like(cand)
        scratch = torch.empty(2 * B, dtype=torch.float32, device=self.dev)
        c.check(c.lib.var_inbatch_loss_fwd_bwd(c.handle, c.stream(), ptr(anchor), ptr(cand), ptr(target), B, M, float(tau),
                                               float(inv_count), ptr(scratch), ptr(loss), ptr(ga), ptr(gc)),
                "var_inbatch_loss_fwd_bwd")
        return loss, ga, gc

    def step_inbatch(self, image, pos, neg, tau=0.1):
        self._check(image, pos, neg)
        c, m = self.ctx, self.model
        flat = m.flat_parameters()
        B = image.shape[0]
        c.ensure_plan(B, self.hw)
        dev = self.dev
        rccl, rank, world = self.rccl, self.rank, self.world
        stream = c.stream()
        self._bind()
        emb = torch.empty((3, B, 3), dtype=torch.float32, device=dev)
        c.check(c.lib.var_arm_encoder_fwd(c.handle, stream, ptr(flat), ptr(image), int(image.dtype == torch.uint8),
                                          image.stride(0), ptr(pos), ptr(neg), B, self.hw, ptr(emb[0]), ptr(emb[1]), ptr(emb[2]),
                                          None, None, 1), "var_arm_encoder_fwd")
        local = emb[1:].reshape(2 * B, 3)
        if rccl is not None and world > 1:
            cand = rccl.allgather(local.reshape(-1)).view(-1, 3)
        elif world > 1:
            cand = torch.empty((world * 2 * B, 3), dtype=torch.float32, device=dev)
            torch.distributed.all_gather_into_tensor(cand, local.contiguous(), group=self.pg)
        else:
            cand = local
        target = torch.arange(B, dtype=torch.int32, device=dev) + rank * 2 * B
        loss, ga, gc = self._inbatch_head(emb[0], cand.contiguous(), target, tau, 1.0 / (B * world))
        if rccl is not None and world > 1:
            rccl.allreduce(gc.view(-1))
        elif world > 1:
            torch.distributed.all_reduce(gc, op=torch.distributed.ReduceOp.SUM, group=self.pg)
        mine = gc[rank * 2 * B:(rank + 1) * 2 * B]
        c.check(c.lib.var_arm_encoder_bwd(c.handle, stream, ptr(flat), ptr(ga), ptr(mine[:B].contiguous()),
                                          ptr(mine[B:].contiguous()), ptr(self.gbuf)), "var_arm_encoder_bwd")
        self.gbuf[N_PARAMS:].copy_(loss)
        self.allreduce()
        self.adam()
        return self.loss

    def capture_inbatch_epoch_steps(self, images, pcm, batch, table, tau=0.1):
        B = batch
        rows, row_ints = int(table.shape[0]), int(table.shape[1])
        if row_ints != 5 * B or table.dtype != torch.int32 or table.device != self.dev or not table.is_contiguous():
            raise VarHipError("index table must be a contiguous int32 (rows, 5*batch) tensor on the trainer's device")
        c, dev, world, rank, rccl = self.ctx, self.dev, self.world, self.rank, self.rccl
        flat = self.model.flat_parameters()
        c.ensure_plan(B, self.hw)
        self._g_table = torch.empty_like(table)
        self._g_cursor = torch.zeros(1, dtype=torch.int32, device=dev)
        self._g_idx = torch.zeros(row_ints, dtype=torch.int32, device=dev)
        self._device_scalars(B)
        img = torch.zeros((B,) + tuple(images.shape[1:]), dtype=images.dtype, device=dev)
        feats = torch.zeros((2 * B, 1, 100, 40), dtype=torch.float32, device=dev)
        emb = torch.zeros((3, B, 3), dtype=torch.float32, device=dev)
        cand = torch.zeros((world * 2 * B, 3), dtype=torch.float32, device=dev) if world > 1 else emb[1:].reshape(2 * B, 3)
        target = (torch.arange(B, dtype=torch.int32, device=dev) + rank * 2 * B).contiguous()
        loss1 = torch.zeros(1, dtype=torch.float32, device=dev)
        ga, gc = torch.zeros((B, 3), dtype=torch.float32, device=dev), torch.zeros_like(cand)
        scratch = torch.zeros(2 * B, dtype=torch.float32, device=dev)
        mine = gc[rank * 2 * B:(rank + 1) * 2 * B]
        clip_idx, lens = self._g_idx[B:3 * B], self._g_idx[3 * B:5 * B]
        self._keep_inbatch = (img, feats, emb, cand, target, loss1, ga, gc, scratch)

        def body_fwd():
            self._bind()
            torch.index_select(images, 0, self._g_idx[:B], out=img)
            c.check(c.lib.var_mfcc(c.handle, c.stream(), ptr(pcm), ptr(lens), ptr(clip_idx), 2 * B, pcm.stride(0), 100,
                                   ptr(feats)), "var_mfcc")
            c.check(c.lib.var_arm_encoder_fwd(c.handle, c.stream(), ptr(flat), ptr(img), int(img.dtype == torch.uint8),
                                              img.stride(0), ptr(feats), ptr(feats[B:]), B, self.hw, ptr(emb[0]), ptr(emb[1]),
                                              ptr(emb[2]), None, None, 1), "var_arm_encoder_fwd")

        def body_loss():
            c.check(c.lib.var_inbatch_loss_fwd_bwd(c.handle, c.stream(), ptr(emb[0]), ptr(cand), ptr(target), B, cand.shape[0],
                                                   float(tau), 1.0 / (B * world), ptr(scratch), ptr(loss1), ptr(ga), ptr(gc)),
                    "var_inbatch_loss_fwd_bwd")

        def body_bwd():
            self._bind()
            c.check(c.lib.var_arm_encoder_bwd(c.handle, c.stream(), ptr(flat), ptr(ga), ptr(mine[:B]), ptr(mine[B:]),
                                              ptr(self.gbuf)), "var_arm_encoder_bwd")
            torch.mul(loss1, 1.0, out=self.gbuf[N_PARAMS:])

        adam = self._body_adam(self._g_table, rows, row_ints, 0)
        body_fwd()
        if world > 1:
            g_fwd, g_loss, g_bwd, g_adam = c.capture([[body_fwd], [body_loss], [body_bwd], [adam]])
        else:
            (g_all,) = c.capture([[body_fwd, body_loss, body_bwd, adam]])

        def load_table(t):
            assert t.shape == self._g_table.shape
            self._g_table.copy_(t, non_blocking=True)
            self._g_idx.copy_(t[0], non_blocking=True)
            self._g_cursor.zero_()

        def replay():
            self._bind()
            if world == 1:
                g_all()
            else:
                g_fwd()
                local = emb[1:].reshape(2 * B, 3)
                if rccl is not None:
                    cand.copy_(rccl.allgather(local.reshape(-1)).view(-1, 3))
                else:
                    torch.distributed.all_gather_into_tensor(cand, local, group=self.pg)
                g_loss()
                if rccl is not None:
                    rccl.allreduce(gc.view(-1))
                else:
                    torch.distributed.all_reduce(gc, op=torch.distributed.ReduceOp.SUM, group=self.pg)
                g_bwd()
                self.allreduce()
                g_adam()
            self.step_count += 1
            return self.loss
        load_table(table)
        return replay, load_table

    def step_from_pcm(self, image, pcm, lens, global_batch=None):
        B = image.shape[0]
        idx = torch.arange(B, dtype=torch.int32, device=image.device)
        cidx = torch.arange(2 * B, dtype=torch.int32, device=image.device)
        return self.step_from_dataset(image, idx, pcm, cidx, lens, global_batch)

    def _check(self, image, pos, neg):
        for t in (image, pos, neg):
            if t is None or t.device != self.dev or not t.is_contiguous():
                raise VarHipError("VARTrainer.step needs contiguous tensors (image, pos, neg) on the trainer's device")
        if pos.dtype != torch.float32 or neg.dtype != torch.float32 or image.dtype not in (torch.uint8, torch.float32):
            raise VarHipError("image must be u8/f32 and MFCC f32")


def _save_outputs(tr, model, save_dir, fname, log):
    rank = getattr(tr, "rank", 0)
    dist = getattr(tr, "world", 1) > 1 and torch.distributed.is_available() and torch.distributed.is_initialized()
    if rank == 0:
        os.makedirs(save_dir, exist_ok=True)
        torch.save(model.state_dict(), fname, _use_new_zipfile_serialization=False)
        log('Model saved to ' + fname)
    if dist:
        torch.distributed.barrier(group=getattr(tr, "pg", None))


def _save_progress(tr, save_dir, loss_list):
    if getattr(tr, "rank", 0) != 0:
        return
    os.makedirs(save_dir, exist_ok=True)
    with open(os.path.join(save_dir, 'progress.csv'), 'w', newline='') as f:
        w = csv.writer(f)
        w.writerow(['avg_loss'])
        for v in loss_list:
            w.writerow([v])


def train_representation(model, batches, epochs, lr=1e-4, weight_decay=1e-6, milestones=None, gamma=0.2,
                         margin=1.0, save_dir=None, save_interval=10, start_ep=0, log=print):
    from .ithor import IthorTrainer, IthorVARPretextNet
    is_ithor = isinstance(model, IthorVARPretextNet)
    if milestones is None:
        milestones = (20, 30) if is_ithor else (10, 30, 50)
    trainer_cls = IthorTrainer if is_ithor else VARTrainer
    tr = trainer_cls(model, lr=lr, weight_decay=weight_decay, margin=margin)
    model.train()
    loss_list = []
    for ep in range(epochs):
        tr.lr = multistep_lr(lr, milestones, gamma, ep)
        losses = []
        for image, sp, sn, _gt in batches():
            tr.step(image.contiguous(), sp.float().contiguous(), sn.float().contiguous())
            losses.append(tr.loss.clone())
        stack = torch.stack(losses).reshape(-1)
        if is_ithor and model.gru_status():
            bad = int((~torch.isfinite(stack)).sum().item())
            log(f'persistent GRU launch timed out in {bad} step(s) of epoch {start_ep + ep} (status '
                f'{model.gru_status():#x}): skipped by the optimiser; switching to per-step GRU launches')
            model.set_gru_sequence(False)
            model._ensure_plan(tr.ctx, int(image.shape[0]))
            stack = stack[torch.isfinite(stack)]
            if stack.numel() == 0:
                raise VarHipError("every step of the epoch timed out in the persistent GRU launches")
        avg = float(stack.sum().item() / stack.numel())
        loss_list.append(avg)
        log('average loss', avg)
        if save_dir and ((ep + 1) % save_interval == 0 or ep + 1 == epochs):
            _save_outputs(tr, model, save_dir, os.path.join(save_dir, str(start_ep + ep) + '.pt'), log)
    if save_dir:
        _save_progress(tr, save_dir, loss_list)
    model.eval()
    return loss_list


def train_representation_from_pool(model, pool, epochs, batch, lr=1e-4, weight_decay=1e-6, milestones=None,
                                   gamma=0.2, margin=1.0, save_dir=None, save_interval=10, start_ep=0, log=print,
                                   drop_last=False, _ctx=None):
    from .ithor import IthorTrainer, IthorVARPretextNet
    is_ithor = isinstance(model, IthorVARPretextNet)
    if milestones is None:
        milestones = (20, 30) if is_ithor else (10, 30, 50)
    if is_ithor:
        tr = IthorTrainer(model, lr=lr, weight_decay=weight_decay, margin=margin)
    else:
        tr = VARTrainer(model, lr=lr, weight_decay=weight_decay, margin=margin, _ctx=_ctx)
    if getattr(pool, "clip_tab", None) is None:
        pool.freeze_pairs()
    model.train()
    spe, bt = pool.steps_per_epoch(batch, drop_last), pool.tail_batch(batch, drop_last)
    if spe < 1:
        raise VarHipError(f"the pool holds {pool.n_items} triplets: no step of batch {batch} with drop_last={drop_last}")
    replay = load_table = None
    loss_list = []
    acc = torch.zeros(1, dtype=torch.float32, device=tr.dev)
    ran = torch.zeros(1, dtype=torch.float32, device=tr.dev)
    join_timeouts0 = 0 if is_ithor else tr.ctx.join_timeouts()
    for ep in range(epochs):
        tr.set_lr(multistep_lr(lr, milestones, gamma, ep))
        table = pool.epoch_index_table(batch, drop_last)
        if replay is None:
            replay, load_table = tr.capture_epoch_steps(pool.images, pool.clips, batch, table, steps_per_epoch=spe,
                                                        tail_batch=bt)
        else:
            load_table(table)
        acc.zero_()
        ran.zero_()
        for _ in range(spe):
            l = replay()
            ok = torch.isfinite(l)
            acc += torch.where(ok, l, torch.zeros_like(l)).reshape(-1)[:1]
            ran += ok.reshape(-1)[:1].float()
        n_ran = int(ran.item())
        if not is_ithor and tr.ctx.join_timeouts() > join_timeouts0:
            raise VarHipError(f"a device-side stream hand-over timed out in epoch {start_ep + ep} (var_join_status: "
                              f"{tr.ctx.join_timeouts() - join_timeouts0}); var_set_streams(ctx, 3 | 64) restores the stream edges")
        if is_ithor and n_ran < spe:
            log(f'persistent GRU launch timed out in {spe - n_ran} step(s) of epoch {start_ep + ep} (status '
                f'{model.gru_status():#x}): skipped by the optimiser; switching to per-step GRU launches')
            model.set_gru_sequence(False)
            model._ensure_plan(tr.ctx, int(batch))
            replay = None
            if n_ran == 0:
                raise VarHipError("every step of the epoch timed out in the persistent GRU launches")
        avg = float(acc.item()) / max(n_ran, 1)
        loss_list.append(avg)
        log('average loss', avg)
        if save_dir and ((ep + 1) % save_interval == 0 or ep + 1 == epochs):
            _save_outputs(tr, model, save_dir, os.path.join(save_dir, str(start_ep + ep) + '.pt'), log)
    if save_dir:
        _save_progress(tr, save_dir, loss_list)
    model.eval()
    return loss_list
```

Before: 916,200 triplets/s.

## Fold weight-gradient slab reductions into the fused Adam/pack kernel

Adds a single-GPU train-step entry that skips the separate image and sound weight-gradient reduce kernels and instead reduces the per-workgroup slabs inside the Adam update kernel, driven by a precomputed fold schedule uploaded at init. The goal is to remove several kernel launches and a write-then-read round trip of the gradient buffer for those layers. The trainer's graph capture now uses this fused step when not running data-parallel. The cost is a more complex Adam kernel that has to handle uneven work, and it depends on the slab group counts staying consistent with the schedule.

```diff
diff --git a/include/var_hip.h b/include/var_hip.h
--- a/include/var_hip.h
+++ b/include/var_hip.h
@@ -85,6 +85,15 @@
                         float weight_decay, int* step_dev, const int* index_table, int row_ints, int n_rows,
                         int* cursor_dev, int* index_row, int ahead);
 
+int var_arm_train_step_pcm(var_ctx* ctx, void* stream, float* params,
+                           const void* image, int image_is_u8, long image_bstride, const int* image_index,
+                           const int16_t* pcm, int pcm_stride, const int* clip_index, const int* lens,
+                           int B, int H, float margin, float inv_count,
+                           float* grads, float* loss_out, float* exp_avg, float* exp_avg_sq, long n,
+                           const float* lr_dev, float beta1, float beta2, float eps, float weight_decay,
+                           int* step_dev, const int* index_table, int row_ints, int n_rows,
+                           int* cursor_dev, int* index_row, int ahead);
+
 int var_mfcc(var_ctx* ctx, void* stream, const int16_t* pcm, const int* lens, const int* clip_index,
              int nclips, int pcm_stride, int out_frames, float* out);
 
@@ -159,6 +168,7 @@
 int var_debug_buffer(var_ctx* ctx, const char* name, void** ptr, long* nfloats);
 int var_debug_ithor_gru_drop_workgroup(var_ctx* ctx);
 int var_debug_armnet_drop_workgroup(var_ctx* ctx);
+int var_debug_adam_guard(var_ctx* ctx, const unsigned* guard_dev, long n);
 int var_debug_ithor_dense(var_ctx* ctx, void* stream, int a_kfast, int b_kfast, const float* a, const float* b,
                           float* c, int M, int N, int K, int nsplit, int add);
 
diff --git a/voicecontrolledrobot-var_amd/_lib.py b/voicecontrolledrobot-var_amd/_lib.py
--- a/voicecontrolledrobot-var_amd/_lib.py
+++ b/voicecontrolledrobot-var_amd/_lib.py
@@ -50,6 +50,9 @@
     "var_mfcc": (_i, [_vp, _vp, _vp, _vp, _vp, _i, _i, _i, _vp]),
     "var_mfcc_ex": (_i, [_vp, _vp, _vp, _vp, _vp, _i, _i, _i, _i, _i, _i, _vp]),
     "var_arm_loss_grad_pcm": (_i, [_vp, _vp, _vp, _vp, _i, _l, _vp, _vp, _i, _vp, _vp, _i, _i, _f, _f, _vp, _vp, _vp]),
+    "var_arm_train_step_pcm": (_i, [_vp, _vp, _vp, _vp, _i, _l, _vp, _vp, _i, _vp, _vp, _i, _i, _f, _f, _vp, _vp, _vp, _vp, _l,
+                                    _vp, _f, _f, _f, _f, _vp, _vp, _i, _i, _vp, _vp, _i]),
+    "var_debug_adam_guard": (_i, [_vp, _vp, _l]),
     "var_arm_loss_grad_gather": (_i, [_vp, _vp, _vp, _vp, _i, _l, _vp, _vp, _vp, _i, _i, _f, _f, _vp, _vp, _vp]),
     "var_inbatch_loss_fwd_bwd": (_i, [_vp, _vp, _vp, _vp, _vp, _i, _i, _f, _f, _vp, _vp, _vp, _vp]),
     "var_comm_unique_id": (_i, [_vp, _vp]),
diff --git a/voicecontrolledrobot-var_amd/csrc/api.hip b/voicecontrolledrobot-var_amd/csrc/api.hip
--- a/voicecontrolledrobot-var_amd/csrc/api.hip
+++ b/voicecontrolledrobot-var_amd/csrc/api.hip
@@ -62,7 +62,7 @@
         delete c;
         return VAR_ERR_HIP;
     }
-    if (mfcc_build_tables(c) != VAR_OK || pack_table_upload(c) != VAR_OK) {
+    if (mfcc_build_tables(c) != VAR_OK || pack_table_upload(c) != VAR_OK || fold_sched_upload(c) != VAR_OK) {
         snprintf(g_init_err, sizeof(g_init_err), "var_init: %s", c->err);
         delete c;
         return VAR_ERR_HIP;
@@ -88,6 +88,7 @@
     if (c->mfcc_tab) (void)hipFree(c->mfcc_tab);
     if (c->mfcc_psf_tab) (void)hipFree(c->mfcc_psf_tab);
     if (c->pack_segs_dev) (void)hipFree(c->pack_segs_dev);
+    if (c->fold_sched_dev) (void)hipFree(c->fold_sched_dev);
     for (int i = 0; i < 2; i++) {
         if (c->ev_fork[i]) (void)hipEventDestroy(c->ev_fork[i]);
         if (c->ev_join[i]) (void)hipEventDestroy(c->ev_join[i]);
@@ -403,7 +404,7 @@
 }
 
 static int encoder_bwd(var_ctx* c, hipStream_t s, const float* params, float* grads, bool fused = false,
-                       float margin = 0.f, float inv_count = 0.f, float* loss_out = nullptr) {
+                       float margin = 0.f, float inv_count = 0.f, float* loss_out = nullptr, bool fold = true) {
     const int B = c->saved_B;
     int rc;
     if (!c->saved_image || !c->saved_pos || !c->saved_neg) {
@@ -415,10 +416,10 @@
     if (!dev_join && (rc = fork_side(c, s, 1)) != VAR_OK) return rc;
     if (c->saved_image) {
         if ((rc = launch_heads_bwd(c, s, s, params, grads, B, true, 0, 0, dev_join, fused, margin, inv_count, fused ? loss_out : nullptr)) != VAR_OK) return rc;
-        if ((rc = launch_img_bwd(c, s, params, grads, B)) != VAR_OK) return rc;
+        if ((rc = launch_img_bwd(c, s, params, grads, B, fold)) != VAR_OK) return rc;
     }
     if ((rc = launch_heads_bwd(c, ss, ss, params, grads, B, false, snd_lo, snd_hi, dev_join, fused, margin, inv_count)) != VAR_OK) return rc;
-    if ((rc = launch_snd_bwd(c, ss, params, grads, B)) != VAR_OK) return rc;
+    if ((rc = launch_snd_bwd(c, ss, params, grads, B, fold)) != VAR_OK) return rc;
     return join_side(c, s, 1);
 }
 
@@ -447,17 +448,18 @@
 static int loss_grad_impl(var_ctx* c, hipStream_t s, const float* params, const void* image, int image_is_u8,
                           long image_bstride, const int* image_index, const float* mfcc_pos, const float* mfcc_neg,
                           const AudioIn* audio, int B, int H, float margin, float inv_count, float* grads,
-                          float* loss_out, float* feats_out, const char* who) {
+                          float* loss_out, float* feats_out, const char* who, bool defer_fold = false) {
     if (image_bstride < 3L * H * H) { VAR_SET_ERR(c, "%s: image stride %ld < 3*H*H", who, image_bstride); return VAR_ERR_ARG; }
     int rc = check_plan(c, B, H, who);
     if (rc != VAR_OK) return rc;
     if ((rc = check_weights(c, params, who)) != VAR_OK) return rc;
     SET_DEVICE(c);
     const bool fused = !feats_out && image && (mfcc_pos || (audio && audio->pcm)) && (mfcc_neg || (audio && audio->pcm));
+    if (defer_fold && !fused) { VAR_SET_ERR(c, "%s: needs the image and both sound branches", who); return VAR_ERR_ARG; }
     if ((rc = encoder_fwd(c, s, params, image, image_is_u8, image_bstride, image_index, mfcc_pos, mfcc_neg, audio, B, 1,
                           !fused, fused, false)) != VAR_OK) return rc;
     if (fused) {
-        rc = encoder_bwd(c, s, params, grads, true, margin, inv_count, loss_out);
+        rc = encoder_bwd(c, s, params, grads, true, margin, inv_count, loss_out, !defer_fold);
         c->fwd_plan.dev_join = false;
         return rc;
     }
@@ -548,6 +550,47 @@
     return launch_adam_dev(c, (hipStream_t)stream, params, grads, exp_avg, exp_avg_sq, n, lr_dev, beta1, beta2, eps,
                            weight_decay, step_dev, n == VAR_N_PARAMS && c->bound->params == params, index_table, row_ints, n_rows, cursor_dev, index_row,
                            ahead_from);
+}
+
+int var_arm_train_step_pcm(var_ctx* c, void* stream, float* params, const void* image, int image_is_u8, long image_bstride,
+                           const int* image_index, const int16_t* pcm, int pcm_stride, const int* clip_index, const int* lens,
+                           int B, int H, float margin, float inv_count, float* grads, float* loss_out, float* exp_avg,
+                           float* exp_avg_sq, long n, const float* lr_dev, float beta1, float beta2, float eps,
+                           float weight_decay, int* step_dev, const int* index_table, int row_ints, int n_rows,
+                           int* cursor_dev, int* index_row, int ahead) {
+    CHECK_CTX(c);
+    if (!params || !image || !pcm || !lens || !grads || !loss_out || pcm_stride <= 0 || !exp_avg || !exp_avg_sq || !lr_dev || !step_dev) {
+        VAR_SET_ERR(c, "var_arm_train_step_pcm: null argument");
+        return VAR_ERR_ARG;
+    }
+    if (n != VAR_N_PARAMS) { VAR_SET_ERR(c, "var_arm_train_step_pcm: %ld parameters, the model has %d", n, VAR_N_PARAMS); return VAR_ERR_ARG; }
+    if (c->bound->params != params) {
+        VAR_SET_ERR(c, "var_arm_train_step_pcm: params is not the arena the bound weight image was packed from");
+        return VAR_ERR_ARG;
+    }
+    if (index_table && (!cursor_dev || !index_row || row_ints <= 0 || n_rows <= 0)) {
+        VAR_SET_ERR(c, "var_arm_train_step_pcm: index table without cursor / row buffer / sizes");
+        return VAR_ERR_ARG;
+    }
+    AudioIn a;
+    a.pcm = pcm; a.lens = lens; a.clip_index = clip_index; a.pcm_stride = pcm_stride;
+    int rc = loss_grad_impl(c, (hipStream_t)stream, params, image, image_is_u8, image_bstride, image_index, nullptr, nullptr, &a, B, H,
+                            margin, inv_count, grads, loss_out, nullptr, "var_arm_train_step_pcm", true);
+    if (rc != VAR_OK) return rc;
+    if (c->snd_groups <= 0) { VAR_SET_ERR(c, "var_arm_train_step_pcm: the sound backward left no slabs"); return VAR_ERR_STATE; }
+    return launch_fold_adam_dev(c, (hipStream_t)stream, params, grads, exp_avg, exp_avg_sq, lr_dev, beta1, beta2, eps, weight_decay,
+                                step_dev, index_table, row_ints, n_rows, cursor_dev, index_row, ahead);
+}
+
+int var_debug_adam_guard(var_ctx* c, const unsigned* guard_dev, long n) {
+    CHECK_CTX(c);
+    if (guard_dev) {
+        if (!c->adam_guard_dbg) { c->adam_guard_kept = c->adam_guard; c->adam_guard_kept_n = c->adam_guard_n; }
+        c->adam_guard = guard_dev; c->adam_guard_n = n; c->adam_guard_dbg = true;
+    } else if (c->adam_guard_dbg) {
+        c->adam_guard = c->adam_guard_kept; c->adam_guard_n = c->adam_guard_kept_n; c->adam_guard_dbg = false;
+    }
+    return VAR_OK;
 }
 
 int var_mfcc(var_ctx* c, void* stream, const int16_t* pcm, const int* lens, const int* clip_index, int nclips,
diff --git a/voicecontrolledrobot-var_amd/csrc/img_conv_bwd.hip b/voicecontrolledrobot-var_amd/csrc/img_conv_bwd.hip
--- a/voicecontrolledrobot-var_amd/csrc/img_conv_bwd.hip
+++ b/voicecontrolledrobot-var_amd/csrc/img_conv_bwd.hip
@@ -45,7 +45,7 @@
     return VAR_OK;
 }
 
-int launch_img_bwd(var_ctx* c, hipStream_t s, const float* params, float* grads, int B) {
+int launch_img_bwd(var_ctx* c, hipStream_t s, const float* params, float* grads, int B, bool fold) {
     int rc;
     const int H = c->H;
     if (H != 84 && H != 96) { VAR_SET_ERR(c, "unsupported image size %d (84 or 96)", H); return VAR_ERR_ARG; }
@@ -55,5 +55,6 @@
     rc = launch_img_bwd_tail2(c, s, B);
     if (rc != VAR_OK) return rc;
     (void)params;
+    if (!fold) return VAR_OK;
     return launch_img_wgrad_reduce(c, s, grads, 0, 4);
 }
diff --git a/voicecontrolledrobot-var_amd/csrc/img_wgrad.hip b/voicecontrolledrobot-var_amd/csrc/img_wgrad.hip
--- a/voicecontrolledrobot-var_amd/csrc/img_wgrad.hip
+++ b/voicecontrolledrobot-var_amd/csrc/img_wgrad.hip
@@ -332,6 +332,13 @@
     return VAR_OK;
 }
 
+void img_fold_segs(var_ctx* c, FoldSeg* out, bool nominal) {
+    const ParamLayout& L = c->pl;
+    for (int i = 0; i < 5; i++)
+        out[i] = FoldSeg{(int)slab_offset(i), kSlabSz[i], nominal ? kWgG[i] : c->wg_groups[i], kCombo[i], i < 3 ? 1 : 2, kImgCh[i],
+                         i == 0 ? 0 : 1, L.img_w[i], L.img_b[i], kCombo[i] * kSlabSz[i], 0u};
+}
+
 int img_wgrad_groups(int layer) { return kWgG[layer]; }
 size_t img_slab_offset(int layer) { return slab_offset(layer); }
 #endif
diff --git a/voicecontrolledrobot-var_amd/csrc/pack_adam.hip b/voicecontrolledrobot-var_amd/csrc/pack_adam.hip
--- a/voicecontrolledrobot-var_amd/csrc/pack_adam.hip
+++ b/voicecontrolledrobot-var_amd/csrc/pack_adam.hip
@@ -1,4 +1,7 @@
 #include <stdlib.h>
+
+#include <algorithm>
+#include <vector>
 
 #include "var_common.h"
 
@@ -123,6 +126,88 @@
 }
 
 constexpr int kAdamT = 1024;
+
+struct AdamCoef { float b1, b2, eps, wd, step_size, bc2_sqrt; };
+
+__device__ __forceinline__ void adam_step_scalars(const float* lr_dev, float b1, float b2, int t, float* sh_step) {
+    auto ipow = [](double b, int e) { double r = 1.0; while (e > 0) { if (e & 1) r *= b; b *= b; e >>= 1; } return r; };
+    const double bc1 = 1.0 - ipow((double)b1, t);
+    const double bc2 = 1.0 - ipow((double)b2, t);
+    sh_step[0] = (float)((double)lr_dev[0] / bc1);
+    sh_step[1] = (float)sqrt(bc2);
+}
+
+__device__ __forceinline__ float adam_elem(float pi, float g, float mo, float vo, const AdamCoef& A, float& mi, float& vi) {
+    const float gi = g + A.wd * pi;
+    mi = mo + (gi - mo) * (1.f - A.b1);
+    vi = vo * A.b2 + (1.f - A.b2) * gi * gi;
+    const float denom = sqrtf(vi) / A.bc2_sqrt + A.eps;
+    return pi - A.step_size * (mi / denom);
+}
+
+__device__ __forceinline__ void pack_scatter_elem(const PackSeg& S, int e, float pn, float* __restrict__ wpack) {
+    auto divmod = [](int a, int d, int& qq, int& r) {
+        qq = (int)((float)a * __frcp_rn((float)d));
+        r = a - qq * d;
+        if (r < 0) { --qq; r += d; } else if (r >= d) { ++qq; r -= d; }
+    };
+    int c, tap, nn, rest;
+    if (S.type == 2) { divmod(e, S.cin, rest, c); divmod(rest, S.taps, nn, tap); }
+    else { divmod(e, S.taps, rest, tap); divmod(rest, S.cin, nn, c); }
+    int d;
+    if (S.type == 3)
+        d = ((((tap * (S.cin / 16) + (c >> 4)) * (S.cout / 16) + (nn >> 4)) * 64 + 16 * (nn & 3) + (c & 15)) << 2) + ((nn >> 2) & 3);
+    else if (S.type >= 4) {
+        const int G = S.type == 4 ? tap * (S.cin / 16) + (c >> 4) : (c >> 4) * 9 + tap;
+        d = (((G * (S.cout / 16) + (nn >> 4)) * 64 + 16 * (c & 3) + (nn & 15)) << 2) + ((c >> 2) & 3);
+    } else d = S.type == 1 ? (tap * S.cout + nn) * S.cin + c : (tap * S.cin + c) * S.cout + nn;
+    wpack[S.dst + d] = pn;
+}
+
+__device__ __forceinline__ void adam_pack_span(long w0, int lane, long n, float* __restrict__ p, const float* g, float* __restrict__ m,
+                                               float* __restrict__ v, const AdamCoef& A, const PackSeg* ssegs, int nseg,
+                                               float* __restrict__ wpack) {
+    const long i = w0 + lane;
+    float pn = 0.f;
+    if (i < n) {
+        float mi, vi;
+        pn = adam_elem(p[i], g[i], m[i], v[i], A, mi, vi);
+        m[i] = mi;
+        v[i] = vi;
+        p[i] = pn;
+    }
+    if (wpack) {
+        bool hit = false;
+        if (lane < nseg) {
+            const int src = ssegs[lane].src, cnt = ssegs[lane].cin * ssegs[lane].cout * ssegs[lane].taps;
+            hit = src < w0 + 64 && src + cnt > w0;
+        }
+        unsigned long long mask = __ballot(hit);
+        while (mask) {
+            const int q = __ffsll((long long)mask) - 1;
+            mask &= mask - 1;
+            const PackSeg S = ssegs[q];
+            const int e = (int)i - S.src;
+            if (i >= n || e < 0 || e >= S.cin * S.cout * S.taps) continue;
+            pack_scatter_elem(S, e, pn, wpack);
+        }
+    }
+}
+
+__device__ __forceinline__ void fetch_index_row(const int* __restrict__ idx_table, int row_ints, int n_rows, int* __restrict__ cursor,
+                                                int* __restrict__ idx_row, int ahead_from) {
+    int next = cursor[0] + 1;
+    if (next >= n_rows) next = 0;
+    int next2 = next + 1;
+    if (next2 >= n_rows) next2 = 0;
+    for (int e = threadIdx.x; e < row_ints; e += kAdamT) {
+        idx_row[e] = idx_table[(size_t)next * row_ints + e];
+        if (ahead_from > 0) idx_row[row_ints + e] = idx_table[(size_t)next2 * row_ints + e];
+    }
+    __syncthreads();
+    if (threadIdx.x == 0) cursor[0] = next;
+}
+
 __global__ void __launch_bounds__(kAdamT)
 adam_pack_dev_kernel(const PackSeg* __restrict__ segs, int nseg, float* __restrict__ p, const float* __restrict__ g, float* __restrict__ m,
                      float* __restrict__ v, long n, const float* __restrict__ lr_dev, float b1, float b2, float eps,
@@ -133,80 +218,117 @@
     if (gloss && !(fabsf(*gloss) <= 3.4e38f)) return;
     __shared__ float sh_step[2];
     const int t = step_dev[0] + 1;
-    if (threadIdx.x == 0) {
-        auto ipow = [](double b, int e) { double r = 1.0; while (e > 0) { if (e & 1) r *= b; b *= b; e >>= 1; } return r; };
-        const double bc1 = 1.0 - ipow((double)b1, t);
-        const double bc2 = 1.0 - ipow((double)b2, t);
-        sh_step[0] = (float)((double)lr_dev[0] / bc1);
-        sh_step[1] = (float)sqrt(bc2);
-    }
+    if (threadIdx.x == 0) adam_step_scalars(lr_dev, b1, b2, t, sh_step);
     __syncthreads();
-    const float step_size = sh_step[0], bc2_sqrt = sh_step[1];
-    if (blockIdx.x == 0 && idx_table) {
-        int next = cursor[0] + 1;
-        if (next >= n_rows) next = 0;
-        int next2 = next + 1;
-        if (next2 >= n_rows) next2 = 0;
-        for (int e = threadIdx.x; e < row_ints; e += kAdamT) {
-            idx_row[e] = idx_table[(size_t)next * row_ints + e];
-            if (ahead_from > 0) idx_row[row_ints + e] = idx_table[(size_t)next2 * row_ints + e];
-        }
-        __syncthreads();
-        if (threadIdx.x == 0) cursor[0] = next;
-    }
+    const AdamCoef A{b1, b2, eps, wd, sh_step[0], sh_step[1]};
+    if (blockIdx.x == 0 && idx_table) fetch_index_row(idx_table, row_ints, n_rows, cursor, idx_row, ahead_from);
     __shared__ PackSeg ssegs[24];
     if (wpack) {
         for (int e = threadIdx.x; e < nseg * (int)(sizeof(PackSeg) / 4); e += kAdamT) ((int*)ssegs)[e] = ((const int*)segs)[e];
         __syncthreads();
     }
     const int lane = threadIdx.x & 63;
-    for (long w0 = (long)blockIdx.x * kAdamT + (threadIdx.x - lane); w0 < n; w0 += (long)gridDim.x * kAdamT) {
-        const long i = w0 + lane;
-        float pn = 0.f;
-        if (i < n) {
-            const float pi = p[i];
-            const float gi = g[i] + wd * pi;
-            const float mi = m[i] + (gi - m[i]) * (1.f - b1);
-            const float vi = v[i] * b2 + (1.f - b2) * gi * gi;
-            m[i] = mi;
-            v[i] = vi;
-            const float denom = sqrtf(vi) / bc2_sqrt + eps;
-            pn = pi - step_size * (mi / denom);
-            p[i] = pn;
-        }
-        if (wpack) {
-            bool hit = false;
-            if (lane < nseg) {
-                const int src = ssegs[lane].src, cnt = ssegs[lane].cin * ssegs[lane].cout * ssegs[lane].taps;
-                hit = src < w0 + 64 && src + cnt > w0;
+    for (long w0 = (long)blockIdx.x * kAdamT + (threadIdx.x - lane); w0 < n; w0 += (long)gridDim.x * kAdamT)
+        adam_pack_span(w0, lane, n, p, g, m, v, A, ssegs, nseg, wpack);
+    if (threadIdx.x == 0) {
+        if (atomicAdd(done_ctr, (unsigned)(t != (int)0x80000000)) == gridDim.x - 1) { step_dev[0] = t; done_ctr[0] = 0; }
+    }
+}
+
+constexpr int kFoldGrid = 256;
+constexpr int kFoldTileE = 128;
+__global__ void __launch_bounds__(kAdamT)
+fold_adam_pack_kernel(FoldTable Targ, const float* __restrict__ slabs, const int* __restrict__ sched, int n_fold_tiles, int plain_lo,
+                      const PackSeg* __restrict__ segs, int nseg, float* __restrict__ p, float* g, float* __restrict__ m,
+                      float* __restrict__ v, long n, const float* __restrict__ lr_dev, float b1, float b2, float eps,
+                      float wd, int* __restrict__ step_dev, unsigned* __restrict__ done_ctr, float* __restrict__ wpack,
+                      const int* __restrict__ idx_table, int row_ints, int n_rows, int* __restrict__ cursor,
+                      int* __restrict__ idx_row, int ahead_from, const unsigned* __restrict__ guard, const float* __restrict__ gloss) {
+    const bool skip = (guard && *guard) || (gloss && !(fabsf(*gloss) <= 3.4e38f));
+    __shared__ float sh_step[2];
+    __shared__ PackSeg ssegs[24];
+    __shared__ float part[2][kAdamT / 256][8][33];
+    __shared__ FoldTable T;
+    const int t = step_dev[0] + 1;
+    if (threadIdx.x == 0) { adam_step_scalars(lr_dev, b1, b2, t, sh_step); T = Targ; }
+    for (int e = threadIdx.x; e < nseg * (int)(sizeof(PackSeg) / 4); e += kAdamT) ((int*)ssegs)[e] = ((const int*)segs)[e];
+    __syncthreads();
+    const AdamCoef A{b1, b2, eps, wd, sh_step[0], sh_step[1]};
+    if (!skip && blockIdx.x == 0 && idx_table) fetch_index_row(idx_table, row_ints, n_rows, cursor, idx_row, ahead_from);
+    const int lane = threadIdx.x & 63;
+    const int quarter = threadIdx.x >> 8, l32 = threadIdx.x & 31, gs = (threadIdx.x >> 5) & 7;
+    int buf = 0;
+    for (int k = sched[blockIdx.x], k1 = sched[blockIdx.x + 1]; k < k1; ++k) {
+        const int tile = sched[kFoldGrid + 1 + k];
+        if (tile >= n_fold_tiles) {
+            const long w0 = (long)plain_lo + (long)(tile - n_fold_tiles) * kAdamT + (threadIdx.x - lane);
+            if (!skip && w0 < n) adam_pack_span(w0, lane, n, p, g, m, v, A, ssegs, nseg, wpack);
+            continue;
+        }
+        const int j = tile * kFoldTileE + quarter * 32 + l32;
+        const bool live = j < T.start[6];
+        int l = 0;
+#pragma unroll
+        for (int i = 1; i < 6; ++i) if (j >= T.start[i] && T.start[i + 1] > T.start[i]) l = i;
+        const FoldSeg S = T.seg[l];
+        const int e = live ? j - T.start[l] : 0;
+        int idx = -1;
+        if (live && gs == 0) {
+            const int combo = e / S.slab_sz, i = e - combo * S.slab_sz;
+            if (S.kind == 2) idx = S.gw + e;
+            else if (S.kind == 0) {
+                if (i >= 1024) idx = S.gb + (i - 1024);
+                else {
+                    const int nn = i / 32, col = i % 32;
+                    if (col < S.cin * 9) { const int tap = col / S.cin, c = col - tap * S.cin; idx = S.gw + (nn * S.cin + c) * 9 + tap; }
+                }
+            } else {
+                const int nb = combo / S.cblk, cb = combo - nb * S.cblk;
+                if (i >= 9216) { if (cb == 0) idx = S.gb + nb * 32 + (i - 9216); }
+                else { const int c = i % 32, tap = (i / 32) % 9, nn = i / 288; idx = S.gw + ((nb * 32 + nn) * S.cin + cb * 32 + c) * 9 + tap; }
             }
-            unsigned long long mask = __ballot(hit);
-            while (mask) {
-                const int q = __ffsll((long long)mask) - 1;
-                mask &= mask - 1;
-                const PackSeg S = ssegs[q];
-                const int e = (int)i - S.src;
-                if (i >= n || e < 0 || e >= S.cin * S.cout * S.taps) continue;
-                auto divmod = [](int a, int d, int& qq, int& r) {
-                    qq = (int)((float)a * __frcp_rn((float)d));
-                    r = a - qq * d;
-                    if (r < 0) { --qq; r += d; } else if (r >= d) { ++qq; r -= d; }
-                };
-                int c, tap, nn, rest;
-                if (S.type == 2) { divmod(e, S.cin, rest, c); divmod(rest, S.taps, nn, tap); }
-                else { divmod(e, S.taps, rest, tap); divmod(rest, S.cin, nn, c); }
-                int d;
-                if (S.type == 3)
-                    d = ((((tap * (S.cin / 16) + (c >> 4)) * (S.cout / 16) + (nn >> 4)) * 64 + 16 * (nn & 3) + (c & 15)) << 2) + ((nn >> 2) & 3);
-                else if (S.type >= 4) {
-                    const int G = S.type == 4 ? tap * (S.cin / 16) + (c >> 4) : (c >> 4) * 9 + tap;
-                    d = (((G * (S.cout / 16) + (nn >> 4)) * 64 + 16 * (c & 3) + (nn & 15)) << 2) + ((c >> 2) & 3);
-                } else d = S.type == 1 ? (tap * S.cout + nn) * S.cin + c : (tap * S.cin + c) * S.cout + nn;
-                wpack[S.dst + d] = pn;
+        }
+        float pi = 0.f, mo = 0.f, vo = 0.f;
+        if (idx >= 0 && !skip) { pi = p[idx]; mo = m[idx]; vo = v[idx]; }
+        const float* sp = slabs + S.slab_off + e;
+        float s = 0.f;
+        if (live) {
+            for (int g0 = gs; g0 < S.G; g0 += 128) {
+                float x[16];
+#pragma unroll
+                for (int u = 0; u < 16; ++u) x[u] = g0 + 8 * u < S.G ? sp[(size_t)(g0 + 8 * u) * S.gstride] : 0.f;
+#pragma unroll
+                for (int u = 0; u < 16; ++u) if (g0 + 8 * u < S.G) s += x[u];
             }
         }
-    }
-    if (threadIdx.x == 0) {
+        part[buf][quarter][gs][l32] = s;
+        __syncthreads();
+        if (idx >= 0) {
+            const float (*P)[33] = part[buf][quarter];
+            s = ((P[0][l32] + P[1][l32]) + (P[2][l32] + P[3][l32])) + ((P[4][l32] + P[5][l32]) + (P[6][l32] + P[7][l32]));
+            g[idx] = s;
+            if (!skip) {
+                float mi, vi;
+                const float pn = adam_elem(pi, s, mo, vo, A, mi, vi);
+                m[idx] = mi;
+                v[idx] = vi;
+                p[idx] = pn;
+                if (wpack) {
+                    unsigned mask = S.segmask;
+                    while (mask) {
+                        const int q = __ffs((int)mask) - 1;
+                        mask &= mask - 1;
+                        const PackSeg PS = ssegs[q];
+                        const int pe = idx - PS.src;
+                        if (pe < 0 || pe >= PS.cin * PS.cout * PS.taps) continue;
+                        pack_scatter_elem(PS, pe, pn, wpack);
+                    }
+                }
+            }
+        }
+        buf ^= 1;
+    }
+    if (!skip && threadIdx.x == 0) {
         if (atomicAdd(done_ctr, (unsigned)(t != (int)0x80000000)) == gridDim.x - 1) { step_dev[0] = t; done_ctr[0] = 0; }
     }
 }
@@ -228,6 +350,81 @@
     hipLaunchKernelGGL(adam_pack_dev_kernel, dim3(grid), dim3(kAdamT), 0, s, (const PackSeg*)c->pack_segs_dev, c->pack_nseg, p, g, m, v, n, lr_dev,
                        b1, b2, eps, wd, step_dev, c->done_ctr, repack ? c->wpack : nullptr, idx_table, row_ints, n_rows,
                        cursor, idx_row, ahead_from, (c->adam_guard && n == c->adam_guard_n) ? c->adam_guard : nullptr,
+                       n == c->adam_guard_n ? c->adam_guard_loss : nullptr);
+    VAR_HIP_CHECK(c, hipGetLastError());
+    return VAR_OK;
+}
+
+static int make_fold_table(var_ctx* c, bool nominal, FoldTable& T) {
+    const ParamLayout& L = c->pl;
+    const PackTable P = make_pack_table(c);
+    img_fold_segs(c, T.seg, nominal);
+    T.seg[5] = snd_fold_seg(c, nominal);
+    int st = 0;
+    for (int i = 0; i < 6; i++) {
+        FoldSeg& S = T.seg[i];
+        T.start[i] = st;
+        st += S.ncombo * S.slab_sz;
+        const int lo = S.gw, hi = i < 5 ? L.img_b[i] + kImgCh[i + 1] : S.gw + S.slab_sz;
+        S.segmask = 0;
+        for (int q = 0; q < P.nseg; q++) {
+            const PackSeg& K = P.seg[q];
+            if (K.src < hi && K.src + K.cin * K.cout * K.taps > lo) S.segmask |= 1u << q;
+        }
+    }
+    T.start[6] = st;
+    if (st % kFoldTileE || T.seg[5].gw + T.seg[5].slab_sz != L.ih_w0 || L.img_b[4] + kImgCh[5] != L.snd_w[0] || P.nseg > 24) {
+        VAR_SET_ERR(c, "fold + Adam: the slab element space does not tile the parameter arena");
+        return VAR_ERR_ARG;
+    }
+    return VAR_OK;
+}
+
+int fold_sched_upload(var_ctx* c) {
+    FoldTable T{};
+    int rc = make_fold_table(c, true, T);
+    if (rc != VAR_OK) return rc;
+    const int n_fold = T.start[6] / kFoldTileE;
+    const int n_plain = (c->pl.total - c->pl.ih_w0 + kAdamT - 1) / kAdamT;
+    const int nt = n_fold + n_plain;
+    std::vector<int> cost(nt, 4), order(nt), load(kFoldGrid, 0), sched(kFoldGrid + 1 + nt);
+    for (int t = 0; t < n_fold; t++) {
+        int l = 0;
+        for (int i = 1; i < 6; i++) if (t * kFoldTileE >= T.start[i]) l = i;
+        cost[t] = (T.seg[l].G + 7) / 8;
+    }
+    for (int t = 0; t < nt; t++) order[t] = t;
+    std::stable_sort(order.begin(), order.end(), [&](int a, int b) { return cost[a] > cost[b]; });
+    std::vector<std::vector<int>> mine(kFoldGrid);
+    for (int t : order) {
+        int b = 0;
+        for (int i = 1; i < kFoldGrid; i++) if (load[i] < load[b]) b = i;
+        load[b] += cost[t];
+        mine[b].push_back(t);
+    }
+    int k = 0;
+    for (int b = 0; b < kFoldGrid; b++) {
+        sched[b] = k;
+        for (int t : mine[b]) sched[kFoldGrid + 1 + k++] = t;
+    }
+    sched[kFoldGrid] = k;
+    VAR_HIP_CHECK(c, hipMalloc((void**)&c->fold_sched_dev, sizeof(int) * sched.size()));
+    VAR_HIP_CHECK(c, hipMemcpy(c->fold_sched_dev, sched.data(), sizeof(int) * sched.size(), hipMemcpyHostToDevice));
+    return VAR_OK;
+}
+
+int launch_fold_adam_dev(var_ctx* c, hipStream_t s, float* p, float* g, float* m, float* v, const float* lr_dev, float b1,
+                         float b2, float eps, float wd, int* step_dev, const int* idx_table, int row_ints, int n_rows,
+                         int* cursor, int* idx_row, int ahead_from) {
+    FoldTable T{};
+    int rc = make_fold_table(c, false, T);
+    if (rc != VAR_OK) return rc;
+    const long n = c->pl.total;
+    ProfScope prof(c, s, TAG_ADAM);
+    hipLaunchKernelGGL(fold_adam_pack_kernel, dim3(kFoldGrid), dim3(kAdamT), 0, s, T, (const float*)c->slabs, (const int*)c->fold_sched_dev,
+                       T.start[6] / kFoldTileE, c->pl.ih_w0, (const PackSeg*)c->pack_segs_dev, c->pack_nseg, p, g, m, v, n, lr_dev,
+                       b1, b2, eps, wd, step_dev, c->done_ctr, c->wpack, idx_table, row_ints, n_rows, cursor, idx_row, ahead_from,
+                       (c->adam_guard && n == c->adam_guard_n) ? c->adam_guard : nullptr,
                        n == c->adam_guard_n ? c->adam_guard_loss : nullptr);
     VAR_HIP_CHECK(c, hipGetLastError());
     return VAR_OK;
diff --git a/voicecontrolledrobot-var_amd/csrc/snd_mfma.hip b/voicecontrolledrobot-var_amd/csrc/snd_mfma.hip
--- a/voicecontrolledrobot-var_amd/csrc/snd_mfma.hip
+++ b/voicecontrolledrobot-var_amd/csrc/snd_mfma.hip
@@ -404,6 +404,10 @@
 
 static const int kSndG = 128;
 size_t snd_slab_floats() { return (size_t)kSndG * SND_SLICE; }
+FoldSeg snd_fold_seg(var_ctx* c, bool nominal) {
+    return FoldSeg{(int)c->snd_slab_off, SND_SLICE, nominal ? kSndG : c->snd_groups, 1, 1, 0, 2, c->pl.snd_w[0], c->pl.snd_b[0],
+                   SND_SLICE, 0u};
+}
 
 int launch_snd_fwd(var_ctx* c, hipStream_t s, const float* params, const float* pos, const float* neg, int B) {
     const ParamLayout& L = c->pl;
@@ -425,10 +429,11 @@
     return VAR_OK;
 }
 
-int launch_snd_bwd(var_ctx* c, hipStream_t s, const float* params, float* grads, int B) {
+int launch_snd_bwd(var_ctx* c, hipStream_t s, const float* params, float* grads, int B, bool fold) {
     const ParamLayout& L = c->pl;
     const PackLayout& K = c->kl;
     const int lo = c->saved_pos ? 0 : B, hi = c->saved_neg ? 2 * B : B;
+    c->snd_groups = 0;
     if (hi <= lo) {
         { const int rz = var_zero_async(c, s, grads + L.snd_w[0], sizeof(float) * SND_SLICE); if (rz != VAR_OK) return rz; }
         return VAR_OK;
@@ -441,11 +446,13 @@
     }
     const int G = hi - lo < kSndG ? hi - lo : kSndG;
     float* slabs = c->slabs + c->snd_slab_off;
+    c->snd_groups = G;
     {
         ProfScope prof(c, s, TAG_SND_WGRAD);
         hipLaunchKernelGGL(snd_wgrad_kernel, dim3(G), dim3(WNT), 0, s, lo, hi, B, c->saved_pos, c->saved_neg,
                            c->sact[1], c->sact[2], c->sact[3], c->gsact[1], c->gsact[2], c->gsact[3], c->gsact[4], slabs);
     }
+    if (!fold) { VAR_HIP_CHECK(c, hipGetLastError()); return VAR_OK; }
     ProfScope prof(c, s, TAG_SND_REDUCE);
     hipLaunchKernelGGL(snd_reduce_kernel, dim3((SND_SLICE + 31) / 32), dim3(256), 0, s, slabs, G,
                        grads + L.snd_w[0]);
diff --git a/voicecontrolledrobot-var_amd/csrc/var_common.h b/voicecontrolledrobot-var_amd/csrc/var_common.h
--- a/voicecontrolledrobot-var_amd/csrc/var_common.h
+++ b/voicecontrolledrobot-var_amd/csrc/var_common.h
@@ -153,6 +153,8 @@
     size_t slab_floats = 0;
     size_t snd_slab_off = 0;
     int wg_groups[5] = {0};
+    int snd_groups = 0;
+    int* fold_sched_dev = nullptr;
     float* loss_buf = nullptr;
     float* mfcc_tab = nullptr;
     int prof_tag = -1;
@@ -178,6 +180,7 @@
     void* irew = nullptr;
     const unsigned* adam_guard = nullptr;
     long adam_guard_n = 0;
+    const unsigned* adam_guard_kept = nullptr; long adam_guard_kept_n = 0; bool adam_guard_dbg = false;
     const float* adam_guard_loss = nullptr;
 };
 
@@ -265,6 +268,11 @@
 void ithor_reward_free(var_ctx* c);
 void comm_free(var_ctx* c);
 int pack_table_upload(var_ctx* c);
+int fold_sched_upload(var_ctx* c);
+struct FoldSeg { int slab_off, slab_sz, G, ncombo, cblk, cin, kind, gw, gb, gstride; unsigned segmask; };
+struct FoldTable { FoldSeg seg[6]; int start[7]; };
+void img_fold_segs(var_ctx* c, FoldSeg* out, bool nominal);
+FoldSeg snd_fold_seg(var_ctx* c, bool nominal);
 size_t img_slab_floats();
 int img_wgrad_groups(int layer);
 size_t img_slab_offset(int layer);
@@ -295,9 +303,9 @@
 int launch_img_bwd_chain(var_ctx* c, hipStream_t s, int B);
 static constexpr int kTail2G = 256;
 int launch_img_bwd_tail2(var_ctx* c, hipStream_t s, int B);
-int launch_img_bwd(var_ctx* c, hipStream_t s, const float* params, float* grads, int B);
+int launch_img_bwd(var_ctx* c, hipStream_t s, const float* params, float* grads, int B, bool fold = true);
 int launch_snd_fwd(var_ctx* c, hipStream_t s, const float* params, const float* pos, const float* neg, int B);
-int launch_snd_bwd(var_ctx* c, hipStream_t s, const float* params, float* grads, int B);
+int launch_snd_bwd(var_ctx* c, hipStream_t s, const float* params, float* grads, int B, bool fold = true);
 int launch_heads_fwd(var_ctx* c, hipStream_t s, hipStream_t ss, const FwdPlan& p, const float* params, int B, bool has_img,
                      bool has_pos, bool has_neg, bool finish);
 int launch_heads_bwd(var_ctx* c, hipStream_t s, hipStream_t ss, const float* params, float* grads, int B, bool has_img,
@@ -312,6 +320,9 @@
 int launch_adam_dev(var_ctx* c, hipStream_t s, float* p, const float* g, float* m, float* v, long n,
                     const float* lr_dev, float b1, float b2, float eps, float wd, int* step_dev, bool repack,
                     const int* idx_table, int row_ints, int n_rows, int* cursor, int* idx_row, int ahead_from);
+int launch_fold_adam_dev(var_ctx* c, hipStream_t s, float* p, float* g, float* m, float* v, const float* lr_dev, float b1,
+                         float b2, float eps, float wd, int* step_dev, const int* idx_table, int row_ints, int n_rows,
+                         int* cursor, int* idx_row, int ahead_from);
 int launch_mfcc(var_ctx* c, hipStream_t s, const int16_t* pcm, const int* lens, const int* clip_index, int nclips,
                 int pcm_stride, int out_frames, float* out);
 
diff --git a/voicecontrolledrobot-var_amd/trainer.py b/voicecontrolledrobot-var_amd/trainer.py
--- a/voicecontrolledrobot-var_amd/trainer.py
+++ b/voicecontrolledrobot-var_amd/trainer.py
@@ -156,17 +156,41 @@
                     "var_adam_step_graph")
         return body
 
+    def _body_step_pcm(self, images, pcm, idx, Bs, gb, table=None, rows=0, row_ints=0):
+        c, flat = self.ctx, self.model.flat_parameters()
+        fn = getattr(c.lib, "var_arm_train_step_pcm", None) if getattr(self, "fused_step", True) else None
+        if fn is None:
+            grad, adam = self._body_grad_pcm(images, pcm, idx, Bs, gb), self._body_adam(table, rows, row_ints, 0)
+
+            def two_calls():
+                grad()
+                adam()
+            return two_calls
+        img_idx, clip_idx, lens = idx[:Bs], idx[Bs:3 * Bs], idx[3 * Bs:5 * Bs]
+
+        def body():
+            self._bind()
+            c.check(fn(c.handle, c.stream(), ptr(flat), ptr(images), int(images.dtype == torch.uint8),
+                       images.stride(0), ptr(img_idx), ptr(pcm), pcm.stride(0), ptr(clip_idx), ptr(lens), Bs, self.hw,
+                       float(self.margin), 1.0 / gb, ptr(self.gbuf), self._loss_ptr(), ptr(self.exp_avg),
+                       ptr(self.exp_avg_sq), N_PARAMS, ptr(self._g_lr), float(self.betas[0]), float(self.betas[1]),
+                       float(self.eps), float(self.wd), ptr(self._g_step),
+                       ptr(table) if table is not None else None, row_ints, rows,
+                       ptr(self._g_cursor) if table is not None else None,
+                       ptr(self._g_idx) if table is not None else None, 0), "var_arm_train_step_pcm")
+        return body
+
     def capture_dataset_step(self, images, pcm, batch, global_batch=None):
         B = batch
         self._g_idx = torch.zeros(5 * B, dtype=torch.int32, device=self.dev)
         self._device_scalars(B)
         self.ctx.ensure_plan(B, self.hw)
-        grad = self._body_grad_pcm(images, pcm, self._g_idx, B, self._gb(B, global_batch))
-        adam = self._body_adam()
         if self._collective():
-            g_grad, g_adam = self.ctx.capture([[grad], [adam]])
+            grad = self._body_grad_pcm(images, pcm, self._g_idx, B, self._gb(B, global_batch))
+            g_grad, g_adam = self.ctx.capture([[grad], [self._body_adam()]])
         else:
-            (g_grad,), g_adam = self.ctx.capture([[grad, adam]]), None
+            step = self._body_step_pcm(images, pcm, self._g_idx, B, self._gb(B, global_batch))
+            (g_grad,), g_adam = self.ctx.capture([[step]]), None
 
         def replay(idx_row):
             self._bind()
@@ -207,7 +231,8 @@
             return bool(tail_batch) and row % steps_per_epoch == steps_per_epoch - 1
 
         if not dp:
-            graphs = [c.capture([[self._body_grad_pcm(images, pcm, self._g_idx, Bs, gb), adam]])[0] for Bs, gb in sizes]
+            graphs = [c.capture([[self._body_step_pcm(images, pcm, self._g_idx, Bs, gb, self._g_table, rows, row_ints)]])[0]
+                      for Bs, gb in sizes]
 
             def load_table(t):
                 assert t.shape == self._g_table.shape
```

After: 875,400 triplets/s. 0.955x the previous value.
